# xxlong0/NeuralUDF

Hardware: AMD Instinct MI355X
Metric: ray-samples/sec (train step) (higher is better)
Workload: dtype f32 emulated on the 16-bit matrix pipe, f32 accumulate, f32 state / epilogues / optimizer.  Forward-order sweeps (UDF value, input gradient, colour / NeRF forward): f16x2 (x = hi + 2^-11 lo in fp16, 3 fp16 MFMA products, correction terms in their own accumulator).  Backward sweeps (tangent, adjoint

## Files before the change

include/nudf.h:

```cpp
#ifndef NUDF_H
#define NUDF_H
#include <stdint.h>

#ifdef __cplusplus
extern "C" {
#endif

#define NUDF_ABI_VERSION 111
int nudf_version(void);
#define NUDF_ABI_STRUCTS(X) \
  X(NudfGemmNN) X(NudfGemmTN) X(NudfGemmTNProblem) X(NudfGemmTNGroup) X(NudfComposite) X(NudfCompositeGrad) \
  X(NudfUpsample) X(NudfPixelBlend) X(NudfPixelComposite) X(NudfPatchBlend) X(NudfPatchWarp) X(NudfBlendLoss) \
  X(NudfAdamTensor) X(NudfAdamGroup) X(NudfAdam) X(NudfChainStep) X(NudfChain) X(NudfPackFrag) X(NudfPackLayer) \
  X(NudfPackMulti) X(NudfUnpackLayer) X(NudfUnpackMulti) X(NudfRayBatch) X(NudfMeshUDF) X(NudfMeshUDFSparse) \
  X(NudfIsoSurface) X(NudfIsoSurfaceSparse) X(NudfPointCloud) X(NudfMeshTopo) X(NudfMeshOrient) X(NudfMeshRaster)
int nudf_abi_struct(int i, const char** name);
const char* nudf_last_error(void);

enum {
  NUDF_STATUS_NONFINITE_RENDER = 1,
  NUDF_STATUS_NONFINITE_SAMPLES = 2,
  NUDF_STATUS_NONFINITE_LOSS = 4
};
int nudf_set_status_flag(int32_t* device_word);
// ... 154 lines not shown
  const float* add_z; const float* add_udf;
  float* z_merged; float* udf_merged;
  int32_t merge_K;
} NudfUpsample;
#define NUDF_UP_DBG_ROWS 7
#define NUDF_UP_THEORICAL 256
#define NUDF_UP_SERIAL 512
#define NUDF_UP_NOCONTRACT 1024
#define NUDF_UP_SLEEF 2048
#define NUDF_UP_EXPCR 4096
int nudf_upsample(const NudfUpsample* args, void* stream);
int nudf_merge(const float* z, const float* udf, const float* z_new, const float* udf_new, int N, int M,
               int K, float* z_out, float* udf_out, void* stream);
int nudf_merge_points(const float* z, const float* z_new, int N, int M, int K, float* z_out, const float* rays_o,
                      const float* rays_d, const float* sample_dist, float* pts, float* xrows, int ldx, int xcols,
                      void* stream);

typedef struct NudfPixelBlend {
  const float* pts;
  const float* logits; int32_t nl;
  const float* proj;
  const float* imgs;
  int32_t P, V, H, W;
  float* pix;
  int32_t img_layout;
} NudfPixelBlend;
int nudf_pixel_blend_fwd(const NudfPixelBlend* a, void* stream);
int nudf_pixel_blend_bwd(const NudfPixelBlend* a, const float* d_pix, float* d_logits, void* stream);

typedef struct NudfPixelComposite {
  const float* w;
  const float* pix;
  const float* pts;
  const float* bg_in;
  const float* bg_tail;
  int32_t N, S, n_out;
  float* out;
} NudfPixelComposite;
int nudf_pixel_composite_fwd(const NudfPixelComposite* a, void* stream);
int nudf_pixel_composite_bwd(const NudfPixelComposite* a, const float* d_out, float* d_w, float* d_pix,
                             float* d_bg_in, float* d_bg_tail, void* stream);

typedef struct NudfPatchBlend {
  const float* pts;
  const float* grad;
  const float* rays_d;
  const float* uv;
  const float* logits; int32_t nl;
  const float* w; int32_t ldw;
  const float* ref_cam;
  const float* src_cam;
  const float* imgs;
  int32_t N, S, V, H, W, hps;
  float* patch_colors;
  float* patch_mask;
  int32_t img_layout;
} NudfPatchBlend;
int nudf_patch_blend_fwd(const NudfPatchBlend* a, void* stream);
int nudf_patch_blend_bwd(const NudfPatchBlend* a, const float* d_patch, float* d_logits, float* d_w, void* stream);

int nudf_pixel_warp(const NudfPixelBlend* a , float* colors ,
                    float* mask , void* stream);
typedef struct NudfPatchWarp {
  const float* pts;
  const float* normals;
  const float* uv;
  const float* ref_cam;
  const float* src_cam;
  const float* imgs;
  int32_t N, S, V, H, W, hps, img_layout;
  float* colors;
  float* mask;
} NudfPatchWarp;
int nudf_patch_warp(const NudfPatchWarp* a, void* stream);

int nudf_ssim_patch(const float* pred, const float* gt, const float* window, int N, int Npx, float* out,
                    const float* d_out, float* d_pred, void* stream);
int nudf_patch_metric(int type, const float* pred, const float* gt, const float* window, int N, int Npx, float* out,
                      const float* d_out, float* d_pred, void* stream);

typedef struct NudfBlendLoss {
  const float* cb; const float* c; const float* pix; const float* gt;
  const float* err;
  const float* patch_mask;
  const float* weight_sum;
  const float* err_sorted;
  const int64_t* order;
  float* m;
  float* err_masked;
  float* sums;
  const float* sums_ws;
  const float* w_dev;
  float* out;
  const float* d_total;
  float* d_cb; float* d_c; float* d_pix;
  float* d_err;
  float* d_sums;
  int32_t N, sums_nblk;
  float n_rays, trim_ratio;
} NudfBlendLoss;
int nudf_blend_loss_prepare(const NudfBlendLoss* args, void* stream);
int nudf_blend_loss_fwd(const NudfBlendLoss* args, void* stream);
int nudf_blend_loss_bwd(const NudfBlendLoss* args, void* stream);

int nudf_coarse_z(const float* near, const float* far, int nf_stride, const float* t_rand, int N, int S,
                  float* z, float* sample_dist, void* stream);
int nudf_coarse_start(const float* near, const float* far, int nf_stride, const float* t_rand, int center, int N, int S,
                      float* z, float* sample_dist, const float* rays_o, const float* rays_d, float* pts, void* stream);
int nudf_outside_z(const float* far, int f_stride, const float* lin, int N, int n_out, int n_samples,
                   float* z_out, void* stream);
int nudf_ray_points(const float* rays_o, const float* rays_d, const float* z, const float* sample_dist, int N,
                    int S, int mode, float* pts, void* stream);

int nudf_posenc(const float* x, int xld, int xdiv, const float* tangent, int D, int L, float in_scale, int P,
                float* dst1, int ld1, float scale1, float* dst2, int ld2, float scale2, void* stream);
int nudf_posenc_vjp(const float* x, int xld, int D, int L, float in_scale, int P, const float* src1, int ld1,
                    float scale1, const float* src2, int ld2, float scale2, float* g, void* stream);
int nudf_copy_cols(const float* src, int lds, int sdiv, float* dst, int ldd, int ncols, int P, float scale,
                   void* stream);

int nudf_udf_grad_seed(const float* sign, const float* w_row0, const float* h, int ldh, float hscale, int P, int C,
                       float inv_scale, float* out, int ldo, void* stream);
int nudf_udf_head_bwd(const float* sign, const float* dudf, const float* dfeat, int ldf, int P, int F,
                      float scale, float* out, int ldo, void* stream);
int nudf_signed_colsum(const float* sign, const float* R, int ldr, int P, int C, float scale, float* out,
                       void* stream);
int nudf_sigmoid_head_bwd(const float* y, const float* dy, const float* dy_extra, int ldx, int nsig,
                          const float* draw, int ldr, int nraw, int P, float* out, int ldo, void* stream);

int nudf_weightnorm_pack(const float* v, const float* g, int out, int in, const int* perm, float* W, int ldw,
                         float* Wt, int ldwt, float* inv_norm, void* stream);
int nudf_weightnorm_unpack_grad(const float* dW, int ldw, const float* v, const float* g, const float* inv_norm,
                                int out, int in, const int* perm, float* dv, float* dg, void* stream);

#define NUDF_ADAM_MAX_TENSORS 64
#define NUDF_ADAM_MAX_GROUPS 4
typedef struct NudfAdamTensor {
  float* p; const float* g; float* m; float* v;
  int32_t n;
  int32_t group;
  float neg_step_size;
  float bc2_sqrt;
} NudfAdamTensor;
typedef struct NudfAdamGroup {
  float one_minus_beta1, beta2, one_minus_beta2, eps;
} NudfAdamGroup;
typedef struct NudfAdam {
  int32_t n_tensors; int32_t pad_;
  NudfAdamTensor t[NUDF_ADAM_MAX_TENSORS];
  int32_t block_start[NUDF_ADAM_MAX_TENSORS + 1];
  int32_t pad2_;
  NudfAdamGroup group[NUDF_ADAM_MAX_GROUPS];
  const float* dyn;
} NudfAdam;
int nudf_adam_step(const NudfAdam* args, void* stream);
int nudf_adam_chunk(void);

enum {
  NUDF_CH_NONE = 0,
  NUDF_CH_SOFTPLUS = 1,
  NUDF_CH_MULSP = 2,
  NUDF_CH_TANGENT = 3,
  NUDF_CH_BWD = 4,
  NUDF_CH_UDFHEAD = 5,
  NUDF_CH_RELU = 6,
  NUDF_CH_SIGMOIDN = 7,
  NUDF_CH_MULMASK = 8,
  NUDF_CH_ADDMASK = 9,
  NUDF_CH_RELUADD = 10,
  NUDF_CH_SEED = 11
};
enum {
  NUDF_CH_INIT_LOAD = 0,
  NUDF_CH_INIT_POSENC = 1,
  NUDF_CH_INIT_SEED = 2
};
#define NUDF_CH_MAX_STEPS 20
typedef struct NudfChainStep {
  const float* Bp;
  const float* bias;
  const float* X1; const float* X2;
  float* C1; float* C2;
  const float* r1_row;
  const float* r1_col;
  int32_t K, N;
  int32_t epi;
  int32_t iparam;
  int32_t ldx1, ldx2, ldc1, ldc2;
  int32_t ldr1;
  int32_t prec;
  int32_t act_write;
  int32_t act_col0;
  int32_t pe_tail_col;
  int32_t ld_pe;
  float* pe_dst;
  float pe_tail_scale;
  float scale, xscale;
  int32_t layout;
  const float* row_w;
  float* row_sums;
  const float* X3;
  int32_t ldx3;
} NudfChainStep;
#define NUDF_CH_BLK_X1 1
#define NUDF_CH_BLK_X2 2
#define NUDF_CH_BLK_C1 4
#define NUDF_CH_BLK_C2 8
#define NUDF_CH_BLK_PE 16
#define NUDF_CH_STATE16 32
#define NUDF_CH_P4_X1 64
#define NUDF_CH_P4_C1 128
typedef struct NudfChain {
  int32_t P, n_steps;
  int32_t init;
  int32_t k0;
  int32_t x_div;
  int32_t tile_rows;
  int32_t lda0, ldg0;
  int32_t pe_L, pe_jvp;
  int32_t init_state16;
  float pe_in_scale;
  float seed_scale, seed_xscale;
  const float* A0;
  float* G0;
  const float* x;
  const float* v;
  const float* seed_sign;
  const float* seed_wrow;
  unsigned long long* dbg;
  float* absmax_out;
  const float* tile_amax_in;
  float* tile_amax_out;
  int32_t tile_scale;
  int32_t reserved0;
  NudfChainStep step[NUDF_CH_MAX_STEPS];
} NudfChain;
#define NUDF_CH_TILE_TQ 66
#define NUDF_CH_TILE_ROWS 128
#if defined(__cplusplus)
static_assert(sizeof(NudfChain) <= 4096, "NudfChain travels by value: the kernel-argument segment holds 4 KB");
#endif
int nudf_mlp_chain(const NudfChain* args, void* stream);
int nudf_mlp_chain_plan(const NudfChain* args, char* name, int capacity, int32_t* out);
int nudf_set_chain_t16(int on);
int nudf_pack_frag(const float* B, int ldb, int K, int N, float* out, void* stream);

#define NUDF_PACK_MAX_LAYERS 16
#define NUDF_PACK_MAX_FRAGS 4
typedef struct NudfPackFrag {
  float* dst;
  int32_t transpose;
  int32_t o0, i0;
  int32_t K, N;
  int32_t dtype;
} NudfPackFrag;
typedef struct NudfPackLayer {
  const float* v; const float* g;
  const int32_t* perm;
  float* W; float* Wt;
  float* inv_norm;
  int32_t out, in, ldw, ldwt;
  int32_t nfrag, row_start;
  NudfPackFrag frag[NUDF_PACK_MAX_FRAGS];
} NudfPackLayer;
typedef struct NudfPackMulti {
  int32_t n_layers, total_rows;
  NudfPackLayer layer[NUDF_PACK_MAX_LAYERS];
} NudfPackMulti;
int nudf_weightnorm_pack_multi(const NudfPackMulti* args, void* stream);

typedef struct NudfUnpackLayer {
  const float* dW;
  const float* v; const float* g; const float* inv_norm;
  const int32_t* perm;
  float* dv; float* dg;
  const float* db_in; float* db_out;
  int32_t out, in, ldw, row_start;
} NudfUnpackLayer;
typedef struct NudfUnpackMulti {
  int32_t n_layers, total_rows;
  NudfUnpackLayer layer[NUDF_PACK_MAX_LAYERS];
} NudfUnpackMulti;
int nudf_weightnorm_unpack_grad_multi(const NudfUnpackMulti* args, void* stream);

int nudf_scalars_fwd(const float* variance, const float* beta, const float* gamma, float beta_hi, float* scal,
                     float* recip, void* stream);
int nudf_scalars_bwd(const float* variance, const float* beta, const float* gamma, float beta_hi, const float* d_scal,
                     float* d_param, void* stream);

int nudf_l1_sum_fwd(const float* pred, const float* gt, int n, float* out, void* stream);
int nudf_l1_sum_bwd(const float* pred, const float* gt, int n, const float* d_out, float* d_pred, void* stream);

int nudf_sums_errors_fwd(const float* sums, float n_rays, float* err, void* stream);
int nudf_sums_errors_bwd(const float* sums, float n_rays, const float* d_err, float* d_sums, void* stream);

enum { NUDF_LW_COLOR_BASE = 0, NUDF_LW_COLOR = 1, NUDF_LW_COLOR_PIXEL = 2, NUDF_LW_COLOR_PATCH = 3, NUDF_LW_IGR = 4,
       NUDF_LW_IGR_NS = 5, NUDF_LW_SPARSE = 6, NUDF_LW_MASK = 7,
       NUDF_LW_COLOR_SUM = 8,
       NUDF_LW_COUNT = 16 };

int nudf_color_loss_fwd(const float* cb, const float* c, const float* gt, int n, const float* mask, int n_mask,
                        float w_b, float w_c, float w_px, const float* w_dev, float* out, float* den_out, void* stream);
int nudf_color_loss_bwd(const float* cb, const float* c, const float* gt, int n, const float* den, float w_b, float w_c,
                        float w_px, const float* w_dev, const float* d_out, float* d_cb, float* d_c, void* stream);
int nudf_color_loss_sums(const float* cb, const float* c, const float* gt, int n, const float* mask, int n_mask,
                         float* sums, void* stream);
int nudf_color_loss_finish(const float* sums, int has_mask, float w_b, float w_c, float w_px, const float* w_dev,
                           float* out, float* den_out, void* stream);
// ... 414 lines not shown
```

neuraludf_amd/_lib.py:

```python
from __future__ import annotations

import ctypes as C
import os

import torch

_HERE = os.path.dirname(os.path.abspath(__file__))
LIB_PATH = os.environ.get("NUDF_LIB") or os.path.join(_HERE, "libnudf.so")
ABI_VERSION = 111

c_fp = C.c_void_p
i32 = C.c_int32
f32 = C.c_float


class NudfError(RuntimeError):
    pass


class GemmNN(C.Structure):
    _fields_ = [("A", c_fp), ("lda", i32), ("B", c_fp), ("ldb", i32), ("bias", c_fp),
                ("C1", c_fp), ("ldc1", i32), ("C2", c_fp), ("ldc2", i32), ("C3", c_fp), ("ldc3", i32),
                ("X1", c_fp), ("ldx1", i32), ("X2", c_fp), ("ldx2", i32),
                ("M", i32), ("N", i32), ("K", i32), ("epi", i32), ("iparam", i32), ("scale", f32), ("xscale", f32)]


class GemmTN(C.Structure):
    _fields_ = [("A1", c_fp), ("lda1", i32), ("na1", i32), ("B1", c_fp), ("ldb1", i32),
                ("A2", c_fp), ("lda2", i32), ("na2", i32), ("B2", c_fp), ("ldb2", i32),
                ("C", c_fp), ("ldc", i32), ("dbias", c_fp), ("M", i32), ("NA", i32), ("NB", i32),
                ("rows_per_block", i32), ("prec", i32)]


TN_MAX_PROBLEMS = 12


class GemmTNProblem(C.Structure):
    _fields_ = [("A1", c_fp), ("B1", c_fp), ("C", c_fp), ("dbias", c_fp), ("lda1", i32), ("ldb1", i32), ("ldc", i32),
                ("NA", i32), ("NB", i32), ("tile_start", i32), ("flags", i32)]


class GemmTNGroup(C.Structure):
    _fields_ = [("n_problems", i32), ("M", i32), ("rows_per_block", i32), ("total_tiles", i32), ("prec", i32),
                ("prob", GemmTNProblem * TN_MAX_PROBLEMS), ("workspace", c_fp), ("workspace_floats", C.c_int64),
                ("assign", i32), ("amax_a", c_fp), ("amax_b", c_fp)]


class BlendLoss(C.Structure):
    _fields_ = [("cb", c_fp), ("c", c_fp), ("pix", c_fp), ("gt", c_fp), ("err", c_fp), ("patch_mask", c_fp),
                ("weight_sum", c_fp), ("err_sorted", c_fp), ("order", c_fp), ("m", c_fp), ("err_masked", c_fp), ("sums", c_fp),
                ("sums_ws", c_fp), ("w_dev", c_fp), ("out", c_fp), ("d_total", c_fp), ("d_cb", c_fp), ("d_c", c_fp),
                ("d_pix", c_fp), ("d_err", c_fp), ("d_sums", c_fp), ("N", i32), ("sums_nblk", i32), ("n_rays", f32),
                ("trim_ratio", f32)]


class RayBatch(C.Structure):
    _fields_ = [("image", c_fp), ("mask", c_fp), ("intrinsics_inv", c_fp), ("pose", c_fp), ("pixels_x", c_fp),
                ("pixels_y", c_fp), ("N", i32), ("H", i32), ("W", i32), ("h_patch_size", i32), ("rays", c_fp),
                ("ndc_uv", c_fp), ("xyz_cam", c_fp), ("near", c_fp), ("far", c_fp), ("patch_color", c_fp),
                ("patch_mask", c_fp)]


class Composite(C.Structure):
    _fields_ = [("rays_o", c_fp), ("rays_d", c_fp), ("z", c_fp), ("udf", c_fp), ("grad", c_fp),
                ("color", c_fp), ("color_base", c_fp), ("bg_z", c_fp), ("bg_sigma", c_fp), ("bg_color", c_fp),
                ("scal", c_fp), ("sample_dist", c_fp), ("background_rgb", c_fp),
                ("N", i32), ("S", i32), ("n_out", i32), ("s_nominal", i32),
                ("has_anneal", i32), ("cos_anneal", f32), ("flip_saturation", f32),
                ("use_norm_grad", i32), ("sparse_scale", f32), ("alpha_type", i32),
                ("weights", c_fp), ("out_color", c_fp), ("out_color_base", c_fp), ("out_depth", c_fp),
                ("out_normals", c_fp), ("out_wsum", c_fp), ("out_wsum_all", c_fp), ("sums", c_fp), ("ws", c_fp),
                ("o_alpha", c_fp), ("o_alpha_plus", c_fp), ("o_alpha_minus", c_fp), ("o_vis_prob", c_fp),
                ("o_alpha_occ", c_fp), ("o_raw_occ", c_fp), ("o_true_cos", c_fp), ("o_grad_mag", c_fp),
                ("o_mid_z", c_fp), ("o_dists", c_fp), ("o_inside", c_fp), ("o_flip", c_fp), ("sched", c_fp),
                ("p_variance", c_fp), ("p_beta", c_fp), ("p_gamma", c_fp), ("beta_hi", f32), ("defer_sums", i32),
                ("scal_out", c_fp), ("recip_out", c_fp)]


class CompositeGrad(C.Structure):
    _fields_ = [("d_color", c_fp), ("d_color_base", c_fp), ("d_weights", c_fp), ("d_depth", c_fp),
                ("d_normals", c_fp), ("d_wsum", c_fp), ("d_wsum_all", c_fp), ("d_sums", c_fp),
                ("o_d_udf", c_fp), ("o_d_grad", c_fp), ("o_d_color", c_fp), ("o_d_color_base", c_fp),
                ("o_d_bg_sigma", c_fp), ("o_d_bg_color", c_fp), ("o_d_scal", c_fp), ("ws", c_fp), ("o_d_param", c_fp)]


class Upsample(C.Structure):
    _fields_ = [("rays_o", c_fp), ("rays_d", c_fp), ("z", c_fp), ("udf", c_fp), ("u", c_fp),
                ("sample_dist", c_fp), ("gamma_dev", c_fp),
                ("N", i32), ("M", i32), ("K", i32), ("mode", i32),
                ("inv_s", f32), ("beta", f32), ("gamma", f32),
                ("z_new", c_fp), ("pts_new", c_fp), ("dbg", c_fp),
                ("prev_z", c_fp), ("prev_udf", c_fp), ("add_z", c_fp), ("add_udf", c_fp),
                ("z_merged", c_fp), ("udf_merged", c_fp), ("merge_K", i32)]


class PixelBlend(C.Structure):
    _fields_ = [("pts", c_fp), ("logits", c_fp), ("nl", i32), ("proj", c_fp), ("imgs", c_fp),
                ("P", i32), ("V", i32), ("H", i32), ("W", i32), ("pix", c_fp), ("img_layout", i32)]


class PixelComposite(C.Structure):
    _fields_ = [("w", c_fp), ("pix", c_fp), ("pts", c_fp), ("bg_in", c_fp), ("bg_tail", c_fp),
                ("N", i32), ("S", i32), ("n_out", i32), ("out", c_fp)]


class PatchBlend(C.Structure):
    _fields_ = [("pts", c_fp), ("grad", c_fp), ("rays_d", c_fp), ("uv", c_fp), ("logits", c_fp), ("nl", i32),
                ("w", c_fp), ("ldw", i32), ("ref_cam", c_fp), ("src_cam", c_fp), ("imgs", c_fp),
                ("N", i32), ("S", i32), ("V", i32), ("H", i32), ("W", i32), ("hps", i32),
                ("patch_colors", c_fp), ("patch_mask", c_fp), ("img_layout", i32)]


class PatchWarp(C.Structure):
    _fields_ = [("pts", c_fp), ("normals", c_fp), ("uv", c_fp), ("ref_cam", c_fp), ("src_cam", c_fp), ("imgs", c_fp),
                ("N", i32), ("S", i32), ("V", i32), ("H", i32), ("W", i32), ("hps", i32), ("img_layout", i32),
                ("colors", c_fp), ("mask", c_fp)]


ADAM_MAX_TENSORS = 64
ADAM_MAX_GROUPS = 4


class AdamTensor(C.Structure):
    _fields_ = [("p", c_fp), ("g", c_fp), ("m", c_fp), ("v", c_fp), ("n", i32), ("group", i32), ("neg_step_size", f32), ("bc2_sqrt", f32)]


class AdamGroup(C.Structure):
    _fields_ = [("one_minus_beta1", f32), ("beta2", f32), ("one_minus_beta2", f32), ("eps", f32)]


class Adam(C.Structure):
    _fields_ = [("n_tensors", i32), ("pad_", i32), ("t", AdamTensor * ADAM_MAX_TENSORS),
                ("block_start", i32 * (ADAM_MAX_TENSORS + 1)), ("pad2_", i32), ("group", AdamGroup * ADAM_MAX_GROUPS),
                ("dyn", c_fp)]


CH_MAX_STEPS = 20
CH_STATE16 = 32
CH_P4_X1, CH_P4_C1 = 64, 128
CH = dict(NONE=0, SOFTPLUS=1, MULSP=2, TANGENT=3, BWD=4, UDFHEAD=5, RELU=6, SIGMOIDN=7, MULMASK=8, ADDMASK=9, RELUADD=10,
          SEED=11)
CH_INIT = dict(LOAD=0, POSENC=1, SEED=2)


class ChainStep(C.Structure):
    _fields_ = [("Bp", c_fp), ("bias", c_fp), ("X1", c_fp), ("X2", c_fp), ("C1", c_fp), ("C2", c_fp),
                ("r1_row", c_fp), ("r1_col", c_fp), ("K", i32), ("N", i32), ("epi", i32), ("iparam", i32),
                ("ldx1", i32), ("ldx2", i32), ("ldc1", i32), ("ldc2", i32), ("ldr1", i32), ("prec", i32), ("act_write", i32),
                ("act_col0", i32), ("pe_tail_col", i32), ("ld_pe", i32), ("pe_dst", c_fp), ("pe_tail_scale", f32),
                ("scale", f32), ("xscale", f32), ("layout", i32), ("row_w", c_fp), ("row_sums", c_fp), ("X3", c_fp),
                ("ldx3", i32)]


class Chain(C.Structure):
    _fields_ = [("P", i32), ("n_steps", i32), ("init", i32), ("k0", i32), ("x_div", i32), ("tile_rows", i32), ("lda0", i32),
                ("ldg0", i32), ("pe_L", i32), ("pe_jvp", i32), ("init_state16", i32), ("pe_in_scale", f32), ("seed_scale", f32),
                ("seed_xscale", f32), ("A0", c_fp), ("G0", c_fp), ("x", c_fp), ("v", c_fp), ("seed_sign", c_fp),
                ("seed_wrow", c_fp), ("dbg", c_fp), ("absmax_out", c_fp), ("tile_amax_in", c_fp),
                ("tile_amax_out", c_fp), ("tile_scale", C.c_int32), ("reserved0", C.c_int32), ("step", ChainStep * CH_MAX_STEPS)]


PACK_MAX_LAYERS = 16
PACK_MAX_FRAGS = 4


class PackFrag(C.Structure):
    _fields_ = [("dst", c_fp), ("transpose", i32), ("o0", i32), ("i0", i32), ("K", i32), ("N", i32), ("dtype", i32)]


class PackLayer(C.Structure):
    _fields_ = [("v", c_fp), ("g", c_fp), ("perm", c_fp), ("W", c_fp), ("Wt", c_fp), ("inv_norm", c_fp),
                ("out", i32), ("in_", i32), ("ldw", i32), ("ldwt", i32), ("nfrag", i32), ("row_start", i32),
                ("frag", PackFrag * PACK_MAX_FRAGS)]


class PackMulti(C.Structure):
    _fields_ = [("n_layers", i32), ("total_rows", i32), ("layer", PackLayer * PACK_MAX_LAYERS)]


class UnpackLayer(C.Structure):
    _fields_ = [("dW", c_fp), ("v", c_fp), ("g", c_fp), ("inv_norm", c_fp), ("perm", c_fp), ("dv", c_fp),
                ("dg", c_fp), ("db_in", c_fp), ("db_out", c_fp), ("out", i32), ("in_", i32), ("ldw", i32), ("row_start", i32)]


class UnpackMulti(C.Structure):
    _fields_ = [("n_layers", i32), ("total_rows", i32), ("layer", UnpackLayer * PACK_MAX_LAYERS)]


class MeshUDF(C.Structure):
    _fields_ = [("U", c_fp), ("G", c_fp), ("axes", c_fp), ("cell_case", c_fp), ("cell_ntri", c_fp), ("edge_flag", c_fp),
                ("cells", c_fp), ("face_off", c_fp), ("edge_scan", c_fp), ("faces", c_fp), ("edges", c_fp), ("verts", c_fp),
                ("n_cells", C.c_int64), ("n_edges", C.c_int64), ("n_faces", C.c_int64), ("N", i32), ("mean_thr", f32),
                ("max_thr", f32), ("pad_", i32)]


class MeshUDFSparse(C.Structure):
    _fields_ = [("U", c_fp), ("G", c_fp), ("axes", c_fp), ("blocks", c_fp), ("block_slot", c_fp), ("cell_case", c_fp),
                ("cell_ntri", c_fp), ("cells", c_fp), ("face_off", c_fp), ("edge_keys", c_fp), ("edges", c_fp),
                ("faces", c_fp), ("verts", c_fp), ("n_blocks", C.c_int64), ("n_cells", C.c_int64), ("n_edges", C.c_int64),
                ("n_faces", C.c_int64), ("N", i32), ("B", i32), ("nb", i32), ("mean_thr", f32), ("max_thr", f32),
                ("pad_", i32)]


class IsoSurface(C.Structure):
    _fields_ = [("F", c_fp), ("axes", c_fp), ("cell_case", c_fp), ("cell_ntri", c_fp), ("edge_flag", c_fp), ("cells", c_fp),
                ("face_off", c_fp), ("edge_scan", c_fp), ("faces", c_fp), ("edges", c_fp), ("verts", c_fp),
                ("n_cells", C.c_int64), ("n_edges", C.c_int64), ("n_faces", C.c_int64), ("N", i32), ("level", f32)]


class IsoSurfaceSparse(C.Structure):
    _fields_ = [("F", c_fp), ("axes", c_fp), ("blocks", c_fp), ("block_slot", c_fp), ("cell_case", c_fp), ("cell_ntri", c_fp),
                ("cells", c_fp), ("face_off", c_fp), ("edge_keys", c_fp), ("edges", c_fp), ("faces", c_fp), ("verts", c_fp),
                ("n_blocks", C.c_int64), ("n_cells", C.c_int64), ("n_edges", C.c_int64), ("n_faces", C.c_int64), ("N", i32),
                ("B", i32), ("nb", i32), ("level", f32)]


class PointCloud(C.Structure):
    _fields_ = [("verts", c_fp), ("faces", c_fp), ("tri_n", c_fp), ("tri_off", c_fp), ("out", c_fp),
                ("n_verts", C.c_int64), ("n_faces", C.c_int64), ("n_out", C.c_int64), ("out_base", C.c_int64),
                ("cap", C.c_int64), ("density", C.c_double),
                ("pts", c_fp), ("n", C.c_int64), ("origin", C.c_double * 3), ("cell", C.c_double), ("grid", i32 * 3),
                ("pad_", i32), ("keys", c_fp), ("cell_key", c_fp), ("cell_start", c_fp), ("cell_count", c_fp),
                ("n_cells", C.c_int64), ("hash_key", c_fp), ("hash_row", c_fp), ("hash_cap", C.c_int64),
                ("rank", c_fp), ("state", c_fp), ("undecided", c_fp), ("r2", C.c_double),
                ("query", c_fp), ("query_idx", c_fp), ("n_query", C.c_int64), ("bound", C.c_double),
                ("box_bound2", C.c_double), ("box_lo", C.c_double * 3), ("box_hi", C.c_double * 3),
                ("dist", c_fp), ("idx", c_fp),
                ("md_ref_n", c_fp), ("md_ref_off", c_fp), ("md_ref_key", c_fp), ("md_ref_face", c_fp),
                ("md_n_refs", C.c_int64), ("md_cell_face", c_fp), ("md_point", c_fp), ("md_bary", c_fp),
                ("md_ray_o", c_fp), ("md_ray_d", c_fp), ("md_t_min", C.c_double), ("md_t_max", C.c_double),
                ("md_ray_window", c_fp), ("md_mode", i32), ("md_pad_", i32), ("md_count", c_fp)]


class MeshTopo(C.Structure):
    _fields_ = [("faces", c_fp), ("he_key", c_fp), ("he_id", c_fp), ("edge_start", c_fp), ("edges", c_fp), ("he_edge", c_fp),
                ("edge_key", c_fp), ("nbr_off", c_fp), ("nbr", c_fp), ("bverts", c_fp), ("new_count", c_fp), ("new_off", c_fp),
                ("new_faces", c_fp), ("pos", c_fp), ("pos_out", c_fp), ("labels", c_fp), ("changed", c_fp), ("proj", c_fp),
                ("masks", c_fp), ("vis_count", c_fp), ("n_faces", C.c_int64), ("n_verts", C.c_int64), ("n_edges", C.c_int64),
                ("n_bverts", C.c_int64), ("n_new", C.c_int64), ("lam", C.c_double), ("max_loop", i32), ("n_views", i32),
                ("H", i32), ("W", i32), ("border", i32), ("pad_", i32),
                ("sp_key", c_fp), ("sp_cluster_key", c_fp), ("sp_vcluster", c_fp), ("sp_member_off", c_fp),
                ("sp_member", c_fp), ("sp_corner_off", c_fp), ("sp_corner", c_fp), ("sp_attr", c_fp), ("sp_rep", c_fp),
                ("sp_accepted", c_fp), ("sp_quadric", c_fp), ("sp_attr_out", c_fp), ("sp_faces", c_fp),
                ("sp_triple", c_fp), ("sp_degenerate", c_fp), ("n_clusters", C.c_int64), ("sp_grid", C.c_int64 * 3),
                ("sp_origin", C.c_double * 3), ("sp_cell", C.c_double), ("sp_lambda", C.c_double),
                ("sp_boundary_weight", C.c_double), ("sp_attr_width", i32), ("sp_placement", i32),
                ("sp_sd_mark", c_fp), ("sp_sd_edge_vertex", c_fp), ("sp_sd_marked", c_fp), ("sp_sd_ring_off", c_fp),
                ("sp_sd_ring", c_fp), ("sp_sd_vclass", c_fp), ("sp_sd_pos_out", c_fp), ("sp_sd_attr_out", c_fp),
                ("sp_sd_fcount", c_fp), ("sp_sd_foff", c_fp), ("sp_sd_faces_out", c_fp), ("sp_sd_parent", c_fp),
                ("sp_sd_n_ring", C.c_int64), ("sp_sd_n_border", C.c_int64), ("sp_sd_n_marked", C.c_int64),
                ("sp_sd_n_out", C.c_int64), ("sp_sd_max_edge", C.c_double), ("sp_sd_scheme", i32),
                ("sp_sd_mark_all", i32),
                ("sp_sd_hf_bedge", c_fp), ("sp_sd_hf_brank", c_fp), ("sp_sd_hf_link", c_fp), ("sp_sd_hf_rank_in", c_fp),
                ("sp_sd_hf_rank_out", c_fp), ("sp_sd_hf_loop_off", c_fp), ("sp_sd_hf_loop_vertex", c_fp),
                ("sp_sd_hf_loop_edge", c_fp), ("sp_sd_hf_closed", c_fp), ("sp_sd_hf_perimeter", c_fp),
                ("sp_sd_hf_status", c_fp), ("sp_sd_hf_n_border", C.c_int64), ("sp_sd_hf_n_loops", C.c_int64),
                ("sp_sd_hf_n_items", C.c_int64), ("sp_sd_hf_max_perimeter", C.c_double), ("sp_sd_hf_round", i32),
                ("sp_sd_hf_pad_", i32)]


class MeshOrient(C.Structure):
    _fields_ = [("faces", c_fp), ("me_a", c_fp), ("me_b", c_fp), ("word", c_fp), ("changed", c_fp), ("nonorient", c_fp),
                ("comp_off", c_fp), ("comp_face", c_fp), ("comp_sum", c_fp), ("pos", c_fp), ("corner_off", c_fp),
                ("corner", c_fp), ("normals", c_fp), ("origin", C.c_double * 3), ("n_faces", C.c_int64),
                ("n_verts", C.c_int64), ("n_medges", C.c_int64), ("n_comps", C.c_int64),
                ("sm_nbr_off", c_fp), ("sm_nbr", c_fp), ("sm_fixed", c_fp), ("sm_pos_out", c_fp), ("sm_fnormal", c_fp),
                ("sm_fnormal_out", c_fp), ("sm_farea", c_fp), ("sm_fcentre", c_fp), ("sm_n_nbr", C.c_int64),
                ("sm_step", C.c_double), ("sm_inv2sc", C.c_double), ("sm_inv2ss", C.c_double), ("sm_weights", i32),
                ("sm_pad_", i32)]


class MeshRaster(C.Structure):
    _fields_ = [("pos", c_fp), ("faces", c_fp), ("proj", c_fp), ("scr", c_fp), ("npix", c_fp), ("entries", c_fp),
                ("zbuf", c_fp), ("depth", c_fp), ("face", c_fp), ("bary", c_fp), ("vis", c_fp), ("images", c_fp),
                ("normals", c_fp), ("cam_pos", c_fp), ("colors", c_fp), ("n_seen", c_fp), ("n_faces", C.c_int64),
                ("n_verts", C.c_int64), ("n_entries", C.c_int64), ("power", C.c_double), ("fill", f32 * 3),
                ("min_gap", f32), ("n_views", i32), ("H", i32), ("W", i32), ("image_f32", i32)]


LW = dict(color_base=0, color=1, color_pixel=2, color_patch=3, igr=4, igr_ns=5, sparse=6, mask=7, color_sum=8)
LW_COUNT = 16

EPI = dict(NONE=0, SOFTPLUS=1, RELU=2, MUL=3, MULMASK=4, TANGENT=5, BWD=6, SIGMOID=7, UDFHEAD=8,
           SKIPSPLIT=9, RELU_DUAL=10, ADDMASK=11, MULSP=12)

HOLE = dict(FILLED=0, OPEN_CHAIN=1, TOO_MANY_EDGES=2, PERIMETER=3, NONFINITE=4, DUPLICATE=5, REPEATED_VERTEX=6)
HOLE_MAX_EDGES = 64
HOLE_FAN_CAP = 4096

MIRRORS = {"Nudf" + c.__name__: c for c in C.Structure.__subclasses__() if c.__module__ == __name__}

_P, _I, _F = C.c_void_p, C.c_int, C.c_float
SIGNATURES = {
    "nudf_version": (_I, []),
    "nudf_abi_struct": (_I, [_I, C.POINTER(C.c_char_p)]),
    "nudf_last_error": (C.c_char_p, []),
    "nudf_set_status_flag": (_I, [_P]),
    "nudf_status_flag": (_P, []),
    "nudf_gemm_nn": (_I, [C.POINTER(GemmNN), _P]),
    "nudf_gemm_tn": (_I, [C.POINTER(GemmTN), _P]),
    "nudf_gemm_tn_grouped": (_I, [C.POINTER(GemmTNGroup), _P]),
    "nudf_gemm_tn_grouped_workspace": (C.c_int64, [C.POINTER(GemmTNGroup)]),
    "nudf_gemm_tn_grouped_plan": (_I, [C.POINTER(GemmTNGroup), C.POINTER(C.c_int32), i32]),
    "nudf_gemm_tn_grouped_kernel": (_I, [C.POINTER(GemmTNGroup), C.c_char_p, i32, C.POINTER(C.c_int32)]),
    "nudf_set_tn_flags": (_I, [i32]),
    "nudf_set_tn_debug": (_I, [_P]),
    "nudf_composite_fwd": (_I, [C.POINTER(Composite), _P]),
    "nudf_composite_bwd": (_I, [C.POINTER(Composite), C.POINTER(CompositeGrad), _P]),
    "nudf_partial_sums": (_I, [_P, _I, _I, _P, _P]),
    "nudf_composite_colour_finish": (_I, [_P, _P, _I, _I, _P, _P, _P, _P, _P]),
    "nudf_upsample": (_I, [C.POINTER(Upsample), _P]),
    "nudf_merge": (_I, [_P, _P, _P, _P, _I, _I, _I, _P, _P, _P]),
    "nudf_coarse_z": (_I, [_P, _P, _I, _P, _I, _I, _P, _P, _P]),
    "nudf_coarse_start": (_I, [_P, _P, _I, _P, _I, _I, _I, _P, _P, _P, _P, _P, _P]),
    "nudf_merge_points": (_I, [_P, _P, _I, _I, _I, _P, _P, _P, _P, _P, _P, _I, _I, _P]),
    "nudf_outside_z": (_I, [_P, _I, _P, _I, _I, _I, _P, _P]),
    "nudf_ray_points": (_I, [_P, _P, _P, _P, _I, _I, _I, _P, _P]),
    "nudf_posenc": (_I, [_P, _I, _I, _P, _I, _I, _F, _I, _P, _I, _F, _P, _I, _F, _P]),
    "nudf_posenc_vjp": (_I, [_P, _I, _I, _I, _F, _I, _P, _I, _F, _P, _I, _F, _P, _P]),
    "nudf_copy_cols": (_I, [_P, _I, _I, _P, _I, _I, _I, _F, _P]),
    "nudf_udf_grad_seed": (_I, [_P, _P, _P, _I, _F, _I, _I, _F, _P, _I, _P]),
    "nudf_udf_head_bwd": (_I, [_P, _P, _P, _I, _I, _I, _F, _P, _I, _P]),
    "nudf_signed_colsum": (_I, [_P, _P, _I, _I, _I, _F, _P, _P]),
    "nudf_sigmoid_head_bwd": (_I, [_P, _P, _P, _I, _I, _P, _I, _I, _I, _P, _I, _P]),
    "nudf_weightnorm_pack": (_I, [_P, _P, _I, _I, _P, _P, _I, _P, _I, _P, _P]),
    "nudf_weightnorm_unpack_grad": (_I, [_P, _I, _P, _P, _P, _I, _I, _P, _P, _P, _P]),
    "nudf_pixel_blend_fwd": (_I, [C.POINTER(PixelBlend), _P]),
    "nudf_pixel_blend_bwd": (_I, [C.POINTER(PixelBlend), _P, _P, _P]),
    "nudf_pixel_composite_fwd": (_I, [C.POINTER(PixelComposite), _P]),
    "nudf_pixel_composite_bwd": (_I, [C.POINTER(PixelComposite), _P, _P, _P, _P, _P, _P]),
    "nudf_patch_blend_fwd": (_I, [C.POINTER(PatchBlend), _P]),
    "nudf_patch_blend_bwd": (_I, [C.POINTER(PatchBlend), _P, _P, _P, _P]),
    "nudf_pixel_warp": (_I, [C.POINTER(PixelBlend), _P, _P, _P]),
    "nudf_patch_warp": (_I, [C.POINTER(PatchWarp), _P]),
    "nudf_ssim_patch": (_I, [_P, _P, _P, _I, _I, _P, _P, _P, _P]),
    "nudf_patch_metric": (_I, [_I] + [_P, _P, _P, _I, _I, _P, _P, _P, _P]),
    "nudf_adam_step": (_I, [C.POINTER(Adam), _P]),
    "nudf_adam_chunk": (_I, []),
    "nudf_mlp_chain": (_I, [C.POINTER(Chain), _P]),
    "nudf_mlp_chain_plan": (_I, [C.POINTER(Chain), C.c_char_p, i32, C.POINTER(C.c_int32)]),
    "nudf_set_chain_t16": (_I, [_I]),
    "nudf_pack_frag": (_I, [_P, _I, _I, _I, _P, _P]),
    "nudf_weightnorm_pack_multi": (_I, [C.POINTER(PackMulti), _P]),
    "nudf_weightnorm_unpack_grad_multi": (_I, [C.POINTER(UnpackMulti), _P]),
    "nudf_scalars_fwd": (_I, [_P, _P, _P, _F, _P, _P, _P]),
    "nudf_scalars_bwd": (_I, [_P, _P, _P, _F, _P, _P, _P]),
    "nudf_l1_sum_fwd": (_I, [_P, _P, _I, _P, _P]),
    "nudf_l1_sum_bwd": (_I, [_P, _P, _I, _P, _P, _P]),
    "nudf_sums_errors_fwd": (_I, [_P, _F, _P, _P]),
    "nudf_sums_errors_bwd": (_I, [_P, _F, _P, _P, _P]),
    "nudf_color_loss_fwd": (_I, [_P, _P, _P, _I, _P, _I, _F, _F, _F, _P, _P, _P, _P]),
    "nudf_color_loss_bwd": (_I, [_P, _P, _P, _I, _P, _F, _F, _F, _P, _P, _P, _P, _P]),
    "nudf_gen_ray_batch": (_I, [C.POINTER(RayBatch), _P]),
    "nudf_color_loss_sums": (_I, [_P, _P, _P, _I, _P, _I, _P, _P]),
    "nudf_color_loss_finish": (_I, [_P, _I, _F, _F, _F, _P, _P, _P, _P]),
    "nudf_step_loss_fwd": (_I, [_P, _P, _P, _I, _P, _I, _P, _F, _F, _F, _F, _F, _F, _F, _P, _P, _P, _P, _I, _P]),
    "nudf_step_loss_bwd": (_I, [_P, _P, _P, _I, _P, _P, _F, _F, _F, _F, _F, _F, _F, _P, _P, _P, _P, _P, _P, _P]),
    "nudf_col0_seed4": (_I, [_P, _P, _F, _I, _I, _P, _P, _P]),
    **{"nudf_" + n: (_I, [C.POINTER(st), _P]) for st, names in (
        (BlendLoss, ("blend_loss_prepare", "blend_loss_fwd", "blend_loss_bwd")),
        (MeshUDF, ("meshudf_classify", "meshudf_emit", "meshudf_vertices")),
        (MeshUDFSparse, ("meshudf_sparse_classify", "meshudf_sparse_edges", "meshudf_sparse_emit",
                         "meshudf_sparse_vertices")),
        (IsoSurface, ("isosurface_classify", "isosurface_emit", "isosurface_vertices")),
        (IsoSurfaceSparse, ("isosurface_sparse_classify", "isosurface_sparse_edges", "isosurface_sparse_emit",
                            "isosurface_sparse_vertices")),
        (PointCloud, ("pc_tri_count", "pc_tri_emit", "pc_keys", "pc_cells", "pc_thin_round", "pc_nearest",
                      "pc_tribin_count", "pc_tribin_emit", "pc_closest", "pc_raycast")),
        (MeshTopo, ("meshtopo_edges", "meshtopo_fill_count", "meshtopo_fill_emit", "meshtopo_smooth", "meshtopo_cc_hook",
                    "meshtopo_cc_jump", "meshtopo_views", "meshsimplify_keys", "meshsimplify_place",
                    "meshsimplify_faces", "meshsubdiv_mark", "meshsubdiv_odd", "meshsubdiv_even", "meshsubdiv_count",
                    "meshsubdiv_emit", "meshhole_link", "meshhole_rank", "meshhole_count", "meshhole_triangulate")),
        (MeshOrient, ("meshorient_hook", "meshorient_jump", "meshorient_check", "meshorient_outward", "meshorient_normals",
                      "meshsmooth_laplace", "meshsmooth_frames", "meshsmooth_normals", "meshsmooth_update")),
        (MeshRaster, ("meshraster_project", "meshraster_bounds", "meshraster_draw_small", "meshraster_draw_large",
                      "meshraster_resolve", "meshraster_visible", "meshraster_colour")),
    ) for n in names},
}
SYMBOLS = list(SIGNATURES)

_lib = None


def _abi_mismatch(version, table):
    if version != ABI_VERSION:
        return f"is ABI version {version}, this package binds {ABI_VERSION}"
    for name, size in table.items():
        if name not in MIRRORS:
            return f"has an argument struct {name} that this package does not bind"
        if size != C.sizeof(MIRRORS[name]):
            return f"has a {name} of {size} bytes, this package binds {C.sizeof(MIRRORS[name])}"
    missing = [name for name in MIRRORS if name not in table]
    if missing:
        return f"does not report {', '.join(missing)}, which this package binds"
    return None


def _abi_report(l):
    version, table, name, i = int(l.nudf_version()), {}, C.c_char_p(), 0
    if version == ABI_VERSION:
        while (size := l.nudf_abi_struct(i, C.byref(name))) >= 0:
            table[name.value.decode()], i = size, i + 1
    return version, table


def lib():
    global _lib
    if _lib is None:
        if not os.path.exists(LIB_PATH):
            raise NudfError(
                f"{LIB_PATH} not found: build it with `python -m neuraludf_amd.build` "
                "(the NeuralUDF hot path has no CPU/PyTorch fallback)")
        try:
            l = C.CDLL(LIB_PATH)
        except OSError as e:
            raise NudfError(f"cannot load {LIB_PATH}: {e}") from e
        try:
            why = _abi_mismatch(*_abi_report(l))
            if why is None:
                for name, (restype, argtypes) in SIGNATURES.items():
                    fn = getattr(l, name)
                    fn.restype, fn.argtypes = restype, argtypes
        except AttributeError as e:
            why = f"does not export every symbol of include/nudf.h ({e})"
        if why is not None:
            raise NudfError(f"{LIB_PATH} {why}: rebuild with `python -m neuraludf_amd.build --force`")
        _lib = l
    return _lib


STATUS_NONFINITE_RENDER, STATUS_NONFINITE_SAMPLES, STATUS_NONFINITE_LOSS = 1, 2, 4
_STATUS_WORDS = {}
_STATUS_BOUND = None


def bind_status(dev):
    global _STATUS_BOUND
    if dev.type != "cuda":
        raise NudfError("libnudf kernels need device tensors (got a CPU tensor): run on an MI355X")
    idx = dev.index if dev.index is not None else torch.cuda.current_device()
    if _STATUS_BOUND == idx:
        return _STATUS_WORDS[idx]
    w = _STATUS_WORDS.get(idx)
    if w is None:
        w = torch.zeros(1, dtype=torch.int32, device=torch.device("cuda", idx))
        _STATUS_WORDS[idx] = w
    check(lib().nudf_set_status_flag(C.c_void_p(w.data_ptr())), "nudf_set_status_flag")
    _STATUS_BOUND = idx
    return w


def read_status(dev, clear=False):
    w = bind_status(dev)
    v = int(w.item())
    if clear and v:
        w.zero_()
    return v


def status_text(bits):
    names = [(STATUS_NONFINITE_SAMPLES, "non-finite new samples in the hierarchical re-sampling (nudf_upsample)"),
             (STATUS_NONFINITE_RENDER, "non-finite composited ray outputs or renderer scalars (nudf_composite_fwd)"),
             (STATUS_NONFINITE_LOSS, "non-finite loss (nudf_step_loss_fwd)")]
    return "; ".join(t for b, t in names if bits & b) or "finite"


def ptr(t):
    if t is None:
        return None
    if not t.is_cuda:
        raise NudfError("libnudf kernels need device tensors (got a CPU tensor): run on an MI355X")
    if not t.is_contiguous():
        raise NudfError("libnudf kernels need contiguous tensors")
    return t.data_ptr()


HOST_FAST = os.environ.get("NUDF_HOST_FAST", "1") != "0"
_raw_stream = getattr(torch._C, "_cuda_getCurrentRawStream", None)
_raw_device = getattr(torch._C, "_cuda_getDevice", None)


def stream():
    if HOST_FAST and _raw_stream is not None and _raw_device is not None:
        return C.c_void_p(_raw_stream(_raw_device()))
    return C.c_void_p(torch.cuda.current_stream().cuda_stream)


def check(rc, what=""):
    if rc != 0:
        msg = lib().nudf_last_error()
        raise NudfError(f"{what} failed (hipError {rc}): {msg.decode() if msg else ''}")
# ... 19 lines not shown
```

neuraludf_amd/csrc/optim.hip:

```cpp
#include "nudf_common.h"
#include "../../include/nudf.h"

#define ADAM_BLOCK 256
#define ADAM_PER_THREAD 4
#define ADAM_CHUNK (ADAM_BLOCK * ADAM_PER_THREAD)

__global__ __launch_bounds__(ADAM_BLOCK) void adam_kernel(NudfAdam a) {
  int lo = 0, hi = a.n_tensors;
  const int b = blockIdx.x;
  while (hi - lo > 1) {
    const int mid = (lo + hi) >> 1;
    if (a.block_start[mid] <= b) lo = mid; else hi = mid;
  }
  NudfAdamTensor t = a.t[lo];
  const NudfAdamGroup g = a.group[t.group];
  if (a.dyn) {
    t.neg_step_size = a.dyn[2 * lo];
    t.bc2_sqrt = a.dyn[2 * lo + 1];
  }
  const int base = (b - a.block_start[lo]) * ADAM_CHUNK;
#pragma unroll
  for (int k = 0; k < ADAM_PER_THREAD; ++k) {
    const int i = base + k * ADAM_BLOCK + threadIdx.x;
    if (i < t.n) {
      const float gr = t.g[i];
      float m = t.m[i], v = t.v[i];
      m = m + (gr - m) * g.one_minus_beta1;
      v = v * g.beta2 + g.one_minus_beta2 * gr * gr;
      const float denom = sqrtf(v) / t.bc2_sqrt + g.eps;
      t.p[i] = t.p[i] + t.neg_step_size * (m / denom);
      t.m[i] = m;
      t.v[i] = v;
    }
  }
}

extern "C" int nudf_adam_step(const NudfAdam* args, void* stream) {
  const NudfAdam& a = *args;
  if (a.n_tensors <= 0) return 0;
  if (a.n_tensors > NUDF_ADAM_MAX_TENSORS) {
    nudf_set_error("nudf_adam_step: too many tensors in one call", hipErrorInvalidValue);
    return (int)hipErrorInvalidValue;
  }
  const int nblk = a.block_start[a.n_tensors];
  if (nblk <= 0) return 0;
  hipLaunchKernelGGL(adam_kernel, dim3(nblk), dim3(ADAM_BLOCK), 0, (hipStream_t)stream, a);
  NUDF_CHECK_LAUNCH("nudf_adam_step");
  return 0;
}

extern "C" int nudf_adam_chunk(void) { return ADAM_CHUNK; }
```

neuraludf_amd/csrc/rays_embed.hip:

```cpp
#include "nudf_common.h"
#include "../../include/nudf.h"

static inline int nblocks(long long n, int bs) { return (int)((n + bs - 1) / bs); }

__global__ void coarse_z_kernel(const float* near, const float* far, int nf_stride, const float* t_rand,
                                int N, int S, float* z) {
  int idx = blockIdx.x * blockDim.x + threadIdx.x;
  if (idx >= N * S) return;
  int r = idx / S, s = idx - r * S;
  float nr = near[r * nf_stride], fr = far[r * nf_stride];
  float step = 1.0f / (float)(S - 1);
  float t = (s < S / 2) ? s * step : 1.0f - (S - 1 - s) * step;
  float v = nr + (fr - nr) * t;
  if (t_rand) v = v + t_rand[r] * 2.0f / (float)S;
  z[idx] = v;
}

__global__ void sample_dist_kernel(const float* near, const float* far, int n, int S, float* out) {
  __shared__ float red[256];
  float acc = 0.f;
  for (int i = threadIdx.x; i < n; i += blockDim.x) acc += (far[i] - near[i]) / (float)S;
  red[threadIdx.x] = acc;
  __syncthreads();
  for (int s = 128; s > 0; s >>= 1) {
    if (threadIdx.x < s) red[threadIdx.x] += red[threadIdx.x + s];
    __syncthreads();
  }
  if (threadIdx.x == 0) out[0] = red[0] / (float)n;
}

extern "C" int nudf_coarse_z(const float* near, const float* far, int nf_stride, const float* t_rand, int N, int S,
                             float* z, float* sample_dist, void* stream) {
  hipStream_t st = (hipStream_t)stream;
  hipLaunchKernelGGL(coarse_z_kernel, dim3(nblocks((long long)N * S, 256)), dim3(256), 0, st, near, far, nf_stride,
                     t_rand, N, S, z);
  if (sample_dist)
    hipLaunchKernelGGL(sample_dist_kernel, dim3(1), dim3(256), 0, st, near, far, nf_stride ? N : 1, S, sample_dist);
  NUDF_CHECK_LAUNCH("nudf_coarse_z");
  return 0;
}

__global__ __launch_bounds__(256) void coarse_start_kernel(const float* near, const float* far, int nf_stride,
                                                           const float* t_rand, int center, int N, int S, float* z,
                                                           float* sample_dist, const float* __restrict__ o,
                                                           const float* __restrict__ d, float* __restrict__ pts) {
  const int idx = blockIdx.x * blockDim.x + threadIdx.x;
  if (idx < N * S) {
    const int r = idx / S, s = idx - r * S;
    const float nr = near[r * nf_stride], fr = far[r * nf_stride];
    const float step = 1.0f / (float)(S - 1);
    const float t = (s < S / 2) ? s * step : 1.0f - (S - 1 - s) * step;
    float v = nr + (fr - nr) * t;
    if (t_rand) {
      const float tr = center ? __fsub_rn(t_rand[r], 0.5f) : t_rand[r];
      v = v + tr * 2.0f / (float)S;
    }
    z[idx] = v;
    if (pts) {
      pts[(size_t)idx * 3 + 0] = o[r * 3 + 0] + d[r * 3 + 0] * v;
      pts[(size_t)idx * 3 + 1] = o[r * 3 + 1] + d[r * 3 + 1] * v;
      pts[(size_t)idx * 3 + 2] = o[r * 3 + 2] + d[r * 3 + 2] * v;
    }
  }
  if (blockIdx.x == 0 && sample_dist) {
    __shared__ float red[256];
    const int n = nf_stride ? N : 1;
    float acc = 0.f;
    for (int i = threadIdx.x; i < n; i += 256) acc += (far[i] - near[i]) / (float)S;
    red[threadIdx.x] = acc;
    __syncthreads();
    for (int s = 128; s > 0; s >>= 1) {
      if (threadIdx.x < s) red[threadIdx.x] += red[threadIdx.x + s];
      __syncthreads();
    }
    if (threadIdx.x == 0) sample_dist[0] = red[0] / (float)n;
  }
}
extern "C" int nudf_coarse_start(const float* near, const float* far, int nf_stride, const float* t_rand, int center, int N,
                                 int S, float* z, float* sample_dist, const float* rays_o, const float* rays_d, float* pts,
                                 void* stream) {
  if (N <= 0 || S < 2) {
    nudf_set_error("nudf_coarse_start: N >= 1 and S >= 2 required", hipErrorInvalidValue);
    return (int)hipErrorInvalidValue;
  }
  hipLaunchKernelGGL(coarse_start_kernel, dim3(nblocks((long long)N * S, 256)), dim3(256), 0, (hipStream_t)stream, near, far,
                     nf_stride, t_rand, center, N, S, z, sample_dist, rays_o, rays_d, pts);
  NUDF_CHECK_LAUNCH("nudf_coarse_start");
  return 0;
}

__global__ void outside_z_kernel(const float* far, int f_stride, const float* lin, int N, int n_out, float inv_ns,
                                 float* z_out) {
  int idx = blockIdx.x * blockDim.x + threadIdx.x;
  if (idx >= N * n_out) return;
  int r = idx / n_out, j = idx - r * n_out;
  z_out[idx] = far[r * f_stride] / lin[n_out - 1 - j] + inv_ns;
}
extern "C" int nudf_outside_z(const float* far, int f_stride, const float* lin, int N, int n_out, int n_samples,
                              float* z_out, void* stream) {
  hipLaunchKernelGGL(outside_z_kernel, dim3(nblocks((long long)N * n_out, 256)), dim3(256), 0, (hipStream_t)stream,
                     far, f_stride, lin, N, n_out, 1.0f / (float)n_samples, z_out);
  NUDF_CHECK_LAUNCH("nudf_outside_z");
  return 0;
}

__global__ void ray_points_kernel(const float* __restrict__ o, const float* __restrict__ d, const float* __restrict__ z,
                                  const float* sample_dist, int N, int S, int mode, float* __restrict__ pts) {
  int idx = blockIdx.x * blockDim.x + threadIdx.x;
  if (idx >= N * S) return;
  int r = idx / S, s = idx - r * S;
  float t = z[idx];
  if (mode >= 1) {
    float dist = (s < S - 1) ? (z[idx + 1] - t) : sample_dist[0];
    t = t + dist * 0.5f;
  }
  float px = o[r * 3 + 0] + d[r * 3 + 0] * t;
  float py = o[r * 3 + 1] + d[r * 3 + 1] * t;
  float pz = o[r * 3 + 2] + d[r * 3 + 2] * t;
  if (mode == 2) {
    float rr = sqrtf(px * px + py * py + pz * pz);
    rr = fminf(fmaxf(rr, 1.0f), 1e10f);
    pts[(size_t)idx * 4 + 0] = px / rr;
    pts[(size_t)idx * 4 + 1] = py / rr;
    pts[(size_t)idx * 4 + 2] = pz / rr;
    pts[(size_t)idx * 4 + 3] = 1.0f / rr;
  } else {
    pts[(size_t)idx * 3 + 0] = px;
    pts[(size_t)idx * 3 + 1] = py;
    pts[(size_t)idx * 3 + 2] = pz;
  }
}
extern "C" int nudf_ray_points(const float* rays_o, const float* rays_d, const float* z, const float* sample_dist, int N,
                               int S, int mode, float* pts, void* stream) {
  if (N * S == 0) return 0;
  hipLaunchKernelGGL(ray_points_kernel, dim3(nblocks((long long)N * S, 256)), dim3(256), 0, (hipStream_t)stream, rays_o,
                     rays_d, z, sample_dist, N, S, mode, pts);
  NUDF_CHECK_LAUNCH("nudf_ray_points");
  return 0;
}

__global__ void posenc_kernel(const float* __restrict__ x, int xld, int xdiv, const float* __restrict__ v, int D, int L,
                              float in_scale, int P, float* d1, int ld1, float s1, float* d2, int ld2, float s2,
                              int mode) {
  const int E = D * (2 * L + 1);
  long long idx = (long long)blockIdx.x * blockDim.x + threadIdx.x;
  if (idx >= (long long)P * E) return;
  int p = (int)(idx / E), e = (int)(idx - (long long)p * E);
  int blk = e / D, j = e - blk * D;
  float xv = x[(size_t)(p / xdiv) * xld + j] * in_scale;
  float val;
  if (blk == 0) {
    val = (mode == 0) ? xv : v[(size_t)p * D + j] * in_scale;
  } else {
    int k = (blk - 1) >> 1;
// ... 168 lines not shown
  out[idx] = v;
}
extern "C" int nudf_sigmoid_head_bwd(const float* y, const float* dy, const float* dy_extra, int ldx, int nsig,
                                     const float* draw, int ldr, int nraw, int P, float* out, int ldo, void* stream) {
  if (P == 0) return 0;
  hipLaunchKernelGGL(sigmoid_head_bwd_kernel, dim3(nblocks((long long)P * ldo, 256)), dim3(256), 0,
                     (hipStream_t)stream, y, dy, dy_extra, ldx, nsig, draw, ldr, nraw, P, out, ldo);
  NUDF_CHECK_LAUNCH("nudf_sigmoid_head_bwd");
  return 0;
}

__global__ void wn_pack_kernel(const float* __restrict__ v, const float* __restrict__ g, int out, int in,
                               const int* __restrict__ perm, float* __restrict__ W, int ldw, float* __restrict__ Wt,
                               int ldwt, float* __restrict__ inv_norm) {
  const int row = blockIdx.x * (blockDim.x >> 6) + (threadIdx.x >> 6);
  if (row >= out) return;
  const int l = threadIdx.x & 63;
  float sc = 1.0f;
  if (g) {
    float ss = 0.f;
    for (int i = l; i < in; i += 64) {
      float t = v[(size_t)row * in + i];
      ss += t * t;
    }
    ss = wave_sum(ss);
    float inv = 1.0f / sqrtf(ss);
    if (l == 0 && inv_norm) inv_norm[row] = inv;
    sc = g[row] * inv;
  }
  for (int i = l; i < in; i += 64) {
    int c = perm ? perm[i] : i;
    float w = v[(size_t)row * in + i] * sc;
    if (W) W[(size_t)row * ldw + c] = w;
    if (Wt) Wt[(size_t)c * ldwt + row] = w;
  }
}
extern "C" int nudf_weightnorm_pack(const float* v, const float* g, int out, int in, const int* perm, float* W, int ldw,
                                    float* Wt, int ldwt, float* inv_norm, void* stream) {
  hipLaunchKernelGGL(wn_pack_kernel, dim3((out + 3) / 4), dim3(256), 0, (hipStream_t)stream, v, g, out, in, perm, W, ldw,
                     Wt, ldwt, inv_norm);
  NUDF_CHECK_LAUNCH("nudf_weightnorm_pack");
  return 0;
}

__global__ void wn_unpack_grad_kernel(const float* __restrict__ dW, int ldw, const float* __restrict__ v,
                                      const float* __restrict__ g, const float* __restrict__ inv_norm, int out, int in,
                                      const int* __restrict__ perm, float* __restrict__ dv, float* __restrict__ dg) {
  const int row = blockIdx.x * (blockDim.x >> 6) + (threadIdx.x >> 6);
  if (row >= out) return;
  const int l = threadIdx.x & 63;
  if (!g) {
    for (int i = l; i < in; i += 64) dv[(size_t)row * in + i] = dW[(size_t)row * ldw + (perm ? perm[i] : i)];
    return;
  }
  float dot = 0.f;
  for (int i = l; i < in; i += 64) dot += dW[(size_t)row * ldw + (perm ? perm[i] : i)] * v[(size_t)row * in + i];
  dot = wave_sum(dot);
  const float inv = inv_norm[row];
  const float gg = g[row];
  if (l == 0) dg[row] = dot * inv;
  const float c1 = gg * inv, c2 = gg * inv * inv * inv * dot;
  for (int i = l; i < in; i += 64)
    dv[(size_t)row * in + i] = c1 * dW[(size_t)row * ldw + (perm ? perm[i] : i)] - c2 * v[(size_t)row * in + i];
}
extern "C" int nudf_weightnorm_unpack_grad(const float* dW, int ldw, const float* v, const float* g,
                                           const float* inv_norm, int out, int in, const int* perm, float* dv, float* dg,
                                           void* stream) {
  hipLaunchKernelGGL(wn_unpack_grad_kernel, dim3((out + 3) / 4), dim3(256), 0, (hipStream_t)stream, dW, ldw, v, g,
                     inv_norm, out, in, perm, dv, dg);
  NUDF_CHECK_LAUNCH("nudf_weightnorm_unpack_grad");
  return 0;
}

__device__ __forceinline__ void frag_store(const NudfPackFrag& f, int o, int c, float w) {
  const int k = f.transpose ? (c - f.i0) : (o - f.o0);
  const int n = f.transpose ? (o - f.o0) : (c - f.i0);
  if (k < 0 || n < 0 || k >= f.K || n >= f.N) return;
  const int NT = (f.N + 31) >> 5;
  if (f.dtype == 0) {
    const int g = k >> 3, r = k & 7;
    const int lane = 32 * (r >> 2) + (n & 31);
    f.dst[((size_t)(g * NT + (n >> 5)) * 64 + lane) * 4 + (r & 3)] = w;
  } else if (f.dtype == 3) {
    const int g = k >> 4, r = k & 15;
    const int lane = 32 * (r >> 3) + (n & 31);
    const __bf16 hi = (__bf16)w;
    const float r1 = w - (float)hi;
    const __bf16 mid = (__bf16)r1;
    const __bf16 lo = (__bf16)(r1 - (float)mid);
    unsigned short* d16 = reinterpret_cast<unsigned short*>(f.dst) + ((size_t)(g * NT + (n >> 5)) * 3 * 64 + lane) * 8 + (r & 7);
    d16[0] = __builtin_bit_cast(unsigned short, hi);
    d16[512] = __builtin_bit_cast(unsigned short, mid);
    d16[1024] = __builtin_bit_cast(unsigned short, lo);
  } else if (f.dtype == 4) {
    const int g = k >> 4, r = k & 15;
    const int lane = 32 * (r >> 3) + (n & 31);
    const _Float16 hi = (_Float16)w;
    const _Float16 lo = (_Float16)((w - (float)hi) * 2048.0f);
    unsigned short* d16 = reinterpret_cast<unsigned short*>(f.dst) + ((size_t)(g * NT + (n >> 5)) * 2 * 64 + lane) * 8 + (r & 7);
    d16[0] = __builtin_bit_cast(unsigned short, hi);
    d16[512] = __builtin_bit_cast(unsigned short, lo);
  } else {
    const int g = k >> 4, r = k & 15;
    const int lane = 32 * (r >> 3) + (n & 31);
    unsigned short bits;
    if (f.dtype == 1) {
      const _Float16 hv = (_Float16)w;
      bits = __builtin_bit_cast(unsigned short, hv);
    } else {
      const __bf16 bv = (__bf16)w;
      bits = __builtin_bit_cast(unsigned short, bv);
    }
    reinterpret_cast<unsigned short*>(f.dst)[((size_t)(g * NT + (n >> 5)) * 64 + lane) * 8 + (r & 7)] = bits;
  }
}

#define WNP_ROWS 32
#define WNP_THREADS 1024
__device__ __forceinline__ void wnp_split8(const float (&w)[8], uint4& hi, uint4& mid, uint4& lo) {
  unsigned short h[8], m[8], q[8];
#pragma unroll
  for (int j = 0; j < 8; ++j) {
    const __bf16 a = (__bf16)w[j];
    const float r1 = w[j] - (float)a;
    const __bf16 b = (__bf16)r1;
    const __bf16 c = (__bf16)(r1 - (float)b);
    h[j] = __builtin_bit_cast(unsigned short, a);
    m[j] = __builtin_bit_cast(unsigned short, b);
    q[j] = __builtin_bit_cast(unsigned short, c);
  }
  hi = uint4{(unsigned)h[0] | ((unsigned)h[1] << 16), (unsigned)h[2] | ((unsigned)h[3] << 16),
             (unsigned)h[4] | ((unsigned)h[5] << 16), (unsigned)h[6] | ((unsigned)h[7] << 16)};
  mid = uint4{(unsigned)m[0] | ((unsigned)m[1] << 16), (unsigned)m[2] | ((unsigned)m[3] << 16),
              (unsigned)m[4] | ((unsigned)m[5] << 16), (unsigned)m[6] | ((unsigned)m[7] << 16)};
  lo = uint4{(unsigned)q[0] | ((unsigned)q[1] << 16), (unsigned)q[2] | ((unsigned)q[3] << 16),
             (unsigned)q[4] | ((unsigned)q[5] << 16), (unsigned)q[6] | ((unsigned)q[7] << 16)};
}

__device__ __forceinline__ void wnp_split8_f16(const float (&w)[8], uint4& hi, uint4& lo) {
  unsigned short h[8], q[8];
#pragma unroll
  for (int j = 0; j < 8; ++j) {
    const _Float16 a = (_Float16)w[j];
    const _Float16 b = (_Float16)((w[j] - (float)a) * 2048.0f);
    h[j] = __builtin_bit_cast(unsigned short, a);
    q[j] = __builtin_bit_cast(unsigned short, b);
  }
  hi = uint4{(unsigned)h[0] | ((unsigned)h[1] << 16), (unsigned)h[2] | ((unsigned)h[3] << 16),
             (unsigned)h[4] | ((unsigned)h[5] << 16), (unsigned)h[6] | ((unsigned)h[7] << 16)};
  lo = uint4{(unsigned)q[0] | ((unsigned)q[1] << 16), (unsigned)q[2] | ((unsigned)q[3] << 16),
             (unsigned)q[4] | ((unsigned)q[5] << 16), (unsigned)q[6] | ((unsigned)q[7] << 16)};
}

__global__ __launch_bounds__(WNP_THREADS) void wn_pack_multi_kernel(NudfPackMulti a, int pw) {
  extern __shared__ float panel[];
  int li = 0, b = blockIdx.x;
  for (; li < a.n_layers; ++li) {
    const int nb = (a.layer[li].out + WNP_ROWS - 1) / WNP_ROWS;
    if (b < nb) break;
    b -= nb;
  }
  if (li >= a.n_layers) return;
  const NudfPackLayer& L = a.layer[li];
  const int row0 = b * WNP_ROWS;
  const int wave = threadIdx.x >> 6, l = threadIdx.x & 63, tid = threadIdx.x;
  for (int e = tid; e < WNP_ROWS * pw; e += WNP_THREADS) panel[e] = 0.0f;
  __syncthreads();
  for (int r = wave; r < WNP_ROWS; r += WNP_THREADS / 64) {
    const int row = row0 + r;
    if (row >= L.out) break;
    float sc = 1.0f;
    if (L.g) {
      float ss = 0.f;
      for (int i = l; i < L.in; i += 64) {
        const float t = L.v[(size_t)row * L.in + i];
        ss += t * t;
      }
      ss = wave_sum(ss);
      const float inv = 1.0f / sqrtf(ss);
      if (l == 0 && L.inv_norm) L.inv_norm[row] = inv;
      sc = L.g[row] * inv;
    }
    for (int i = l; i < L.in; i += 64) {
      const int c = L.perm ? L.perm[i] : i;
      const float w = L.v[(size_t)row * L.in + i] * sc;
      if (L.W) L.W[(size_t)row * L.ldw + c] = w;
      panel[r * pw + c] = w;
    }
  }
  __syncthreads();
  const int nrows = min(WNP_ROWS, L.out - row0);
  if (L.Wt) {
    for (int e = tid; e < L.in * WNP_ROWS; e += WNP_THREADS) {
      const int c = e >> 5, r = e & 31;
      if (r < nrows) L.Wt[(size_t)c * L.ldwt + row0 + r] = panel[r * pw + c];
    }
  }
  for (int fi = 0; fi < L.nfrag; ++fi) {
    const NudfPackFrag& f = L.frag[fi];
    const int NT = (f.N + 31) >> 5;
    uint4* d4 = reinterpret_cast<uint4*>(f.dst);
    const bool split16 = f.dtype == 3 || f.dtype == 4;
    const int np = (f.dtype == 3) ? 3 : 2;
    if (split16 && f.transpose) {
      const int Q = (f.K + 7) >> 3;
      for (int e = tid; e < WNP_ROWS * Q; e += WNP_THREADS) {
        const int r = e & 31, q = e >> 5;
        const int n = row0 + r - f.o0;
        if (r >= nrows || n < 0 || n >= f.N) continue;
        float w[8];
#pragma unroll
        for (int j = 0; j < 8; ++j) {
          const int k = 8 * q + j;
          w[j] = (k < f.K) ? panel[r * pw + f.i0 + k] : 0.0f;
        }
        uint4 hi, mid, lo;
        const size_t slot = ((size_t)((q >> 1) * NT + (n >> 5)) * np) * 64 + 32 * (q & 1) + (n & 31);
        if (np == 3) {
          wnp_split8(w, hi, mid, lo);
          d4[slot] = hi; d4[slot + 64] = mid; d4[slot + 128] = lo;
        } else {
          wnp_split8_f16(w, hi, lo);
          d4[slot] = hi; d4[slot + 64] = lo;
        }
      }
    } else if (split16 && (f.o0 & 7) == 0) {
      for (int e = tid; e < 4 * f.N; e += WNP_THREADS) {
        const int t = e / f.N, n = e - t * f.N;
        const int k0 = row0 - f.o0 + 8 * t;
        if (k0 < 0 || k0 >= f.K) continue;
        float w[8];
#pragma unroll
        for (int j = 0; j < 8; ++j) w[j] = (k0 + j < f.K) ? panel[(8 * t + j) * pw + f.i0 + n] : 0.0f;
        uint4 hi, mid, lo;
        const size_t slot = ((size_t)((k0 >> 4) * NT + (n >> 5)) * np) * 64 + 32 * ((k0 >> 3) & 1) + (n & 31);
        if (np == 3) {
          wnp_split8(w, hi, mid, lo);
          d4[slot] = hi; d4[slot + 64] = mid; d4[slot + 128] = lo;
        } else {
          wnp_split8_f16(w, hi, lo);
          d4[slot] = hi; d4[slot + 64] = lo;
        }
      }
    } else {
      for (int e = tid; e < nrows * L.in; e += WNP_THREADS) {
        const int r = e / L.in, c = e - r * L.in;
        frag_store(f, row0 + r, c, panel[r * pw + c]);
      }
    }
  }
}
extern "C" int nudf_weightnorm_pack_multi(const NudfPackMulti* args, void* stream) {
  if (args->n_layers <= 0 || args->total_rows <= 0) return 0;
  if (args->n_layers > NUDF_PACK_MAX_LAYERS) {
    nudf_set_error("nudf_weightnorm_pack_multi: too many layers", hipErrorInvalidValue);
    return (int)hipErrorInvalidValue;
  }
  int blocks = 0, in_max = 0;
  for (int i = 0; i < args->n_layers; ++i) {
    blocks += (args->layer[i].out + WNP_ROWS - 1) / WNP_ROWS;
    in_max = max(in_max, args->layer[i].in);
    for (int f = 0; f < args->layer[i].nfrag; ++f)
      if ((args->layer[i].frag[f].dtype == 3 || args->layer[i].frag[f].dtype == 4) && (((uintptr_t)args->layer[i].frag[f].dst) & 15)) {
        nudf_set_error("nudf_weightnorm_pack_multi: split (bf16x3 / f16x2) fragment buffers must be 16-byte aligned", hipErrorInvalidValue);
        return (int)hipErrorInvalidValue;
      }
  }
  const int pw = (in_max + 31) / 32 * 32 + 4;
  const size_t lds = (size_t)WNP_ROWS * pw * sizeof(float);
  if (lds > 64 * 1024) {
    nudf_set_error("nudf_weightnorm_pack_multi: layer wider than 508 inputs", hipErrorInvalidValue);
    return (int)hipErrorInvalidValue;
  }
  hipLaunchKernelGGL(wn_pack_multi_kernel, dim3(blocks), dim3(WNP_THREADS), lds, (hipStream_t)stream, *args, pw);
  NUDF_CHECK_LAUNCH("nudf_weightnorm_pack_multi");
  return 0;
}

__global__ __launch_bounds__(256) void wn_unpack_multi_kernel(NudfUnpackMulti a) {
  const int grow = blockIdx.x * 4 + (threadIdx.x >> 6);
  if (grow >= a.total_rows) return;
  int li = 0;
  while (li + 1 < a.n_layers && a.layer[li + 1].row_start <= grow) ++li;
  const NudfUnpackLayer& L = a.layer[li];
  const int row = grow - L.row_start;
  const int l = threadIdx.x & 63;
  if (l == 0 && L.db_out) L.db_out[row] = L.db_in[row];
  if (!L.g) {
    for (int i = l; i < L.in; i += 64)
      L.dv[(size_t)row * L.in + i] = L.dW[(size_t)row * L.ldw + (L.perm ? L.perm[i] : i)];
    return;
  }
  float dot = 0.f;
  for (int i = l; i < L.in; i += 64)
    dot += L.dW[(size_t)row * L.ldw + (L.perm ? L.perm[i] : i)] * L.v[(size_t)row * L.in + i];
  dot = wave_sum(dot);
  const float inv = L.inv_norm[row];
  const float gg = L.g[row];
  if (l == 0) L.dg[row] = dot * inv;
  const float c1 = gg * inv, c2 = gg * inv * inv * inv * dot;
  for (int i = l; i < L.in; i += 64)
    L.dv[(size_t)row * L.in + i] =
        c1 * L.dW[(size_t)row * L.ldw + (L.perm ? L.perm[i] : i)] - c2 * L.v[(size_t)row * L.in + i];
}
extern "C" int nudf_weightnorm_unpack_grad_multi(const NudfUnpackMulti* args, void* stream) {
  if (args->n_layers <= 0 || args->total_rows <= 0) return 0;
  if (args->n_layers > NUDF_PACK_MAX_LAYERS) {
    nudf_set_error("nudf_weightnorm_unpack_grad_multi: too many layers", hipErrorInvalidValue);
    return (int)hipErrorInvalidValue;
  }
  hipLaunchKernelGGL(wn_unpack_multi_kernel, dim3((args->total_rows + 3) / 4), dim3(256), 0, (hipStream_t)stream, *args);
  NUDF_CHECK_LAUNCH("nudf_weightnorm_unpack_grad_multi");
  return 0;
}

__global__ void scalars_fwd_kernel(const float* variance, const float* beta, const float* gamma, float beta_hi,
                                   float* scal, float* recip) {
  if (threadIdx.x != 0) return;
  const float s = fminf(fmaxf(expf(10.0f * variance[0]), 1e-6f), 1e6f);
  const float b = fminf(fmaxf(fminf(fmaxf(expf(10.0f * beta[0]), 0.0f), beta_hi), 1e-6f), 1e6f);
  const float g = fminf(fmaxf(expf(10.0f * gamma[0]), 1e-6f), 1e6f);
  scal[0] = s; scal[1] = b; scal[2] = g;
  if (recip) { recip[0] = 1.0f / s; recip[1] = 1.0f / b; }
}
extern "C" int nudf_scalars_fwd(const float* variance, const float* beta, const float* gamma, float beta_hi,
                                float* scal, float* recip, void* stream) {
  hipLaunchKernelGGL(scalars_fwd_kernel, dim3(1), dim3(64), 0, (hipStream_t)stream, variance, beta, gamma, beta_hi,
                     scal, recip);
  NUDF_CHECK_LAUNCH("nudf_scalars_fwd");
  return 0;
}
__global__ void scalars_bwd_kernel(const float* variance, const float* beta, const float* gamma, float beta_hi,
                                   const float* d_scal, float* d_param) {
  if (threadIdx.x != 0) return;
  const float s = expf(10.0f * variance[0]);
  d_param[0] = (s >= 1e-6f && s <= 1e6f) ? d_scal[0] * 10.0f * s : 0.0f;
  const float b = expf(10.0f * beta[0]);
  const float b1 = fminf(fmaxf(b, 0.0f), beta_hi);
  d_param[1] = (b >= 0.0f && b <= beta_hi && b1 >= 1e-6f && b1 <= 1e6f) ? d_scal[1] * 10.0f * b : 0.0f;
  const float g = expf(10.0f * gamma[0]);
  d_param[2] = (g >= 1e-6f && g <= 1e6f) ? d_scal[2] * 10.0f * g : 0.0f;
}
extern "C" int nudf_scalars_bwd(const float* variance, const float* beta, const float* gamma, float beta_hi,
                                const float* d_scal, float* d_param, void* stream) {
  hipLaunchKernelGGL(scalars_bwd_kernel, dim3(1), dim3(64), 0, (hipStream_t)stream, variance, beta, gamma, beta_hi,
                     d_scal, d_param);
  NUDF_CHECK_LAUNCH("nudf_scalars_bwd");
  return 0;
}

__global__ __launch_bounds__(1024) void l1_sum_fwd_kernel(const float* __restrict__ pred, const float* __restrict__ gt,
                                                          int n, float* out) {
  __shared__ float red[16];
  float acc = 0.f;
  for (int i = threadIdx.x; i < n; i += 1024) acc += fabsf(pred[i] - gt[i]);
  acc = wave_sum(acc);
  if ((threadIdx.x & 63) == 0) red[threadIdx.x >> 6] = acc;
  __syncthreads();
  if (threadIdx.x == 0) {
    float t = 0.f;
    for (int w = 0; w < 16; ++w) t += red[w];
    out[0] = t;
  }
}
extern "C" int nudf_l1_sum_fwd(const float* pred, const float* gt, int n, float* out, void* stream) {
  if (n <= 0) return 0;
  hipLaunchKernelGGL(l1_sum_fwd_kernel, dim3(1), dim3(1024), 0, (hipStream_t)stream, pred, gt, n, out);
  NUDF_CHECK_LAUNCH("nudf_l1_sum_fwd");
  return 0;
}
__global__ void l1_sum_bwd_kernel(const float* __restrict__ pred, const float* __restrict__ gt, int n,
                                  const float* d_out, float* __restrict__ d_pred) {
  const int i = blockIdx.x * blockDim.x + threadIdx.x;
  if (i >= n) return;
  const float d = pred[i] - gt[i];
  d_pred[i] = d_out[0] * ((d > 0.0f) ? 1.0f : ((d < 0.0f) ? -1.0f : 0.0f));
}
extern "C" int nudf_l1_sum_bwd(const float* pred, const float* gt, int n, const float* d_out, float* d_pred,
                               void* stream) {
  if (n <= 0) return 0;
  hipLaunchKernelGGL(l1_sum_bwd_kernel, dim3(nblocks(n, 256)), dim3(256), 0, (hipStream_t)stream, pred, gt, n, d_out,
                     d_pred);
  NUDF_CHECK_LAUNCH("nudf_l1_sum_bwd");
  return 0;
}

__global__ void sums_errors_fwd_kernel(const float* sums, float n_rays, float* err) {
  if (threadIdx.x != 0) return;
  err[0] = sums[0] / (sums[1] + 1e-5f);
  err[1] = sums[2] / (sums[3] + 1e-5f);
  err[2] = sums[4] / n_rays;
}
extern "C" int nudf_sums_errors_fwd(const float* sums, float n_rays, float* err, void* stream) {
  hipLaunchKernelGGL(sums_errors_fwd_kernel, dim3(1), dim3(64), 0, (hipStream_t)stream, sums, n_rays, err);
  NUDF_CHECK_LAUNCH("nudf_sums_errors_fwd");
  return 0;
}
__global__ void sums_errors_bwd_kernel(const float* sums, float n_rays, const float* d_err, float* d_sums) {
  if (threadIdx.x != 0) return;
  const float a = sums[1] + 1e-5f, b = sums[3] + 1e-5f;
  d_sums[0] = d_err[0] / a;
  d_sums[1] = -d_err[0] * sums[0] / (a * a);
  d_sums[2] = d_err[1] / b;
  d_sums[3] = -d_err[1] * sums[2] / (b * b);
// ... 402 lines not shown
```

neuraludf_amd/mlp.py:

```python
from __future__ import annotations

import math
from typing import List, Optional

import ctypes as C

import torch

from . import _lib
import os

from ._lib import CH, CH_INIT, CH_MAX_STEPS, EPI, Chain, GemmNN, GemmTN, call, ptr


def pad32(n: int) -> int:
    return (n + 31) // 32 * 32


def pad_rows(P: int) -> int:
    return (P + 63) // 64 * 64


def _buf(P, width, dev, zero=None, dtype=torch.float32, blocked=False):
    if blocked:
        assert zero is False and dtype == torch.float32
        t = torch.empty((pad_rows(P), pad32(width)), device=dev, dtype=dtype)
        t._nudf_blk = True
        return t
    ld = pad32(width)
    if dtype == torch.bfloat16:
        t = (torch.zeros if zero else torch.empty)((pad_rows(P), ld), device=dev, dtype=dtype)
        if zero is None and ld != width:
            t.view(pad_rows(P) // 4, ld, 4)[:, width:, :].zero_()
        t._nudf_p4 = True
        return t
    if zero is None:
        t = torch.empty((pad_rows(P), ld), device=dev, dtype=dtype)
        if ld != width:
            t[:, width:].zero_()
        return t
    return (torch.zeros if zero else torch.empty)((pad_rows(P), ld), device=dev, dtype=dtype)


def _is16(t):
    return t is not None and t.dtype == torch.bfloat16


def _isblk(t):
    return t is not None and getattr(t, "_nudf_blk", False)


def _isp4(t):
    return t is not None and getattr(t, "_nudf_p4", False)


def pack16(t):
    R, ld = t.shape
    assert R % 4 == 0
    b = t.to(torch.bfloat16).reshape(R // 4, 4, ld).permute(0, 2, 1).reshape(R, ld).contiguous()
    b._nudf_p4 = True
    return b


def unpack16(t):
    R, ld = t.shape
    assert _isp4(t) and R % 4 == 0
    return t.reshape(R // 4, ld, 4).permute(0, 2, 1).reshape(R, ld).float()


def block(t):
    R, ld = t.shape
    assert R % 32 == 0 and ld % 4 == 0 and t.dtype == torch.float32
    b = t.reshape(R // 32, 32, ld // 4, 4).permute(0, 2, 1, 3).reshape(R, ld).contiguous()
    b._nudf_blk = True
    return b


def unblock(t):
    if not _isblk(t):
        return t
    R, ld = t.shape
    return t.reshape(R // 32, ld // 4, 32, 4).permute(0, 2, 1, 3).reshape(R, ld).contiguous()


def _zero_cols(t, c0):
    if c0 < t.shape[1]:
        t[:, c0:].zero_()
    return t


def alloc_grads(layers, zero=True):
    sizes = [(pl.out_pad * pl.in_pad, pl.out_pad) for pl in layers]
    flat = (torch.zeros if zero else torch.empty)(sum(a + b for a, b in sizes), device=layers[0].W.device)
    out, off = [], 0
    for pl, (a, b) in zip(layers, sizes):
        dW = flat[off:off + a].view(pl.out_pad, pl.in_pad)
        db = flat[off + a:off + a + pl.out]
        out.append((dW, db))
        off += a + b
    return out


def gemm_nn(A, B, M, N, K, epi, C1=None, ldc1=0, C2=None, ldc2=0, C3=None, ldc3=0, X1=None, ldx1=0, X2=None, ldx2=0,
            bias=None, lda=None, ldb=None, iparam=0, scale=1.0, xscale=1.0, c1_off=0, c2_off=0, x1_off=0, x2_off=0):
    a = GemmNN()
    a.A, a.lda = ptr(A), (lda if lda is not None else A.shape[1])
    a.B, a.ldb = ptr(B), (ldb if ldb is not None else B.shape[1])
    a.bias = ptr(bias)
    a.C1 = (ptr(C1) + 4 * c1_off) if C1 is not None else None
    a.ldc1 = ldc1 or (C1.shape[1] if (C1 is not None and C1.dim() == 2) else 0)
    a.C2 = (ptr(C2) + 4 * c2_off) if C2 is not None else None
    a.ldc2 = ldc2 or (C2.shape[1] if (C2 is not None and C2.dim() == 2) else 0)
    a.C3 = ptr(C3)
    a.ldc3 = ldc3 or (C3.shape[1] if (C3 is not None and C3.dim() == 2) else 0)
    a.X1 = (ptr(X1) + 4 * x1_off) if X1 is not None else None
    a.ldx1 = ldx1 or (X1.shape[1] if (X1 is not None and X1.dim() == 2) else 0)
    a.X2 = (ptr(X2) + 4 * x2_off) if X2 is not None else None
    a.ldx2 = ldx2 or (X2.shape[1] if (X2 is not None and X2.dim() == 2) else 0)
    a.M, a.N, a.K, a.epi, a.iparam, a.scale, a.xscale = M, N, K, EPI[epi], iparam, scale, xscale
    if PROFILE is not None:
        _timed("gemm_nn", 2.0 * M * N * getattr(B, "k_true", K), lambda: call("nudf_gemm_nn", a))
        return
    call("nudf_gemm_nn", a)


MFMA_PRODUCTS = {0: 1, 1: 1, 2: 1, 3: 6, 4: 3}

PROFILE = None


def _timed(name, flops, fn, detail=None, nbytes=0.0, xflops=None):
    s = torch.cuda.Event(enable_timing=True)
    e = torch.cuda.Event(enable_timing=True)
    s.record()
    fn()
    e.record()
    PROFILE.append((name, flops, s, e, detail or name, nbytes, xflops))


def call_timed(cls, detail, nbytes, name, *args, units=0.0):
    if PROFILE is None:
        call(name, *args)
    else:
        _timed(cls, -float(units), lambda: call(name, *args), detail, float(nbytes))


def gemm_tn(A1, na1, B1, C, NA, NB, M, dbias=None, A2=None, na2=0, B2=None):
    for t in (A1, B1, A2, B2):
        if t is not None and (_is16(t) or _isblk(t)):
            raise _lib.NudfError("gemm_tn: bf16-stored / blocked-layout operands need gemm_tn_grouped (per-problem "
                                 "NUDF_TN_A16 / _B16 / _A_BLK / _B_BLK flags): the per-layer path (USE_CHAIN = False) "
                                 "stores row-major fp32 state")
    a = GemmTN()
    a.A1, a.lda1, a.na1 = ptr(A1), A1.shape[1], na1
    a.B1, a.ldb1 = ptr(B1), B1.shape[1]
    if A2 is not None:
        a.A2, a.lda2, a.na2 = ptr(A2), A2.shape[1], na2
        a.B2, a.ldb2 = ptr(B2), B2.shape[1]
# ... 273 lines not shown

TN_DETERMINISTIC = True
_TN_WS = {}


def _tn_workspace(g, dev):
    need = int(_lib.lib().nudf_gemm_tn_grouped_workspace(C.byref(g)))
    if need <= 0:
        return None, 0
    ws = _TN_WS.get(dev)
    if ws is None or ws.numel() < need:
        ws = _TN_WS[dev] = torch.empty(need, device=dev)
    return ws, ws.numel()


TN_ASSIGN = os.environ.get("NUDF_TN_ASSIGN", "1") == "1"
_TN_ATOMIC = bool(int(os.environ.get("NUDF_TN_FLAGS", "0")) & 8)


def tn_can_assign():
    return TN_ASSIGN and TN_DETERMINISTIC and not _TN_ATOMIC


def gemm_tn_grouped(jobs, M, assign=False, rows_per_block=0, f16x2=False, amax_a=None, amax_b=None):
    for base in range(0, len(jobs), _lib.TN_MAX_PROBLEMS):
        chunk = jobs[base:base + _lib.TN_MAX_PROBLEMS]
        g = _lib.GemmTNGroup()
        g.n_problems, g.M, g.rows_per_block = len(chunk), M, rows_per_block
        g.prec = _tn_prec()
        if f16x2 and g.prec == 3 and not any(_is16(t) or _isblk(t) for j in chunk for t in (j[0], j[2])):
            g.prec = 4
            g.amax_a, g.amax_b = ptr(amax_a), ptr(amax_b)
        flops = nbytes = 0.0
        for i, (A1, NA, B1, NB, Cm, db) in enumerate(chunk):
            q = g.prob[i]
            q.A1, q.B1, q.C, q.dbias = ptr(A1), ptr(B1), ptr(Cm), ptr(db)
            q.flags = ((1 if _is16(A1) else 0) | (2 if _is16(B1) else 0) | (4 if _isblk(A1) else 0) | (8 if _isblk(B1) else 0) |
                       (16 if _isp4(A1) else 0) | (32 if _isp4(B1) else 0))
            q.lda1, q.ldb1, q.ldc, q.NA, q.NB = A1.shape[1], B1.shape[1], Cm.shape[1], NA, NB
            flops += 2.0 * M * NA * NB
            nbytes += float(M) * (NA * A1.element_size() + NB * B1.element_size())
        if TN_DETERMINISTIC:
            ws, n = _tn_workspace(g, chunk[0][0].device)
            g.workspace, g.workspace_floats = ptr(ws), n
        g.assign = 1 if assign else 0
        if PROFILE is not None:
            _timed("gemm_tn", flops, lambda: call("nudf_gemm_tn_grouped", g),
                   "%s %d problems M=%d (%.1f GFLOP)" % (_lib.kernel_of("nudf_gemm_tn_grouped_kernel", g)[0], len(chunk), M, flops / 1e9),
                   nbytes, flops * MFMA_PRODUCTS.get(int(g.prec), 1))
        else:
            call("nudf_gemm_tn_grouped", g)


class PackedLinear:

    def __init__(self, lin: torch.nn.Module, perm: Optional[List[int]] = None):
        self.lin = lin
        self.weight_norm = hasattr(lin, "weight_v")
        v = lin.weight_v if self.weight_norm else lin.weight
        self.out, self.inp = v.shape
        self.out_pad, self.in_pad = pad32(self.out), pad32(self.inp)
        self._perm_list = perm
        self.perm = None
        self.W = self.Wt = self.inv_norm = None
        self._ver = None
        self._frags = {}
        self._plist = None

    def params(self):
        reg = self.lin._parameters
        pl = self._plist
        if self.weight_norm:
            if pl is None or reg.get("weight_v") is not pl[0] or reg.get("weight_g") is not pl[1] or reg.get("bias") is not pl[2]:
                pl = self._plist = [self.lin.weight_v, self.lin.weight_g, self.lin.bias]
        elif pl is None or reg.get("weight") is not pl[0] or reg.get("bias") is not pl[1]:
            pl = self._plist = [self.lin.weight, self.lin.bias]
        return list(pl)

    def _ensure_buffers(self, dev):
        if self.W is None or self.W.device != dev:
            self.W = torch.zeros(self.out_pad, self.in_pad, device=dev)
            self.Wt = torch.zeros(self.in_pad, self.out_pad, device=dev)
            self.inv_norm = torch.empty(self.out, device=dev)
            self.Wt.k_true, self.W.k_true = self.inp, self.out
            self._frags = {}
            if self._perm_list is not None:
                self.perm = torch.tensor(self._perm_list, dtype=torch.int32, device=dev)

    def invalidate(self):
        self._ver = None
        self._frags = {}

    def frag(self, kind):
        f = self._frags.get(kind)
        if f is None:
            if "@" in kind:
                raise _lib.NudfError("16-bit fragment %r was not packed (pack_group packs them)" % kind)
            if kind == "fwd":
                f = pack_frag(self.Wt, self.out_pad, self.inp, self.out)
            elif kind == "bwd":
                f = pack_frag(self.W, self.in_pad, self.out, self.inp)
            elif kind == "fwd_head0":
                f = pack_frag(self.Wt, self.out_pad, self.inp, 1)
            elif kind == "fwd_feat":
                f = pack_frag(self.Wt, self.out_pad, self.inp, self.out - 1, off=1)
            elif kind == "bwd_feat":
                f = pack_frag(self.W, self.in_pad, self.out - 1, self.inp, off=self.in_pad)
            elif kind.startswith("bwd_hid:"):
                f = pack_frag(self.W, self.in_pad, self.out, int(kind.split(":")[1]))
            elif kind.startswith("fwd_in:"):
                _, i0, K = kind.split(":")
                f = pack_frag(self.Wt, self.out_pad, int(K), self.out, off=int(i0) * self.out_pad)
            else:
                raise KeyError(kind)
            self._frags[kind] = f
        return f

    @property
    def bias(self):
        return self.lin.bias.detach()

    def new_grad_buffers(self):
        dev = self.W.device
        return torch.zeros(self.out_pad, self.in_pad, device=dev), torch.zeros(self.out, device=dev)


PRECISION = os.environ.get("NUDF_PRECISION", "bf16x3")
_PREC = {"f32": 0, "f16": 1, "bf16": 2, "bf16x3": 3, "f16x2": 4}
FWD_F16X2 = os.environ.get("NUDF_FWD_F16X2", "1")
BWD_F16X2 = os.environ.get("NUDF_BWD_F16X2", "1") != "0"
EX_FLY = os.environ.get("NUDF_EX_FLY", "1") != "0"
TN_F16X2 = True
TN_SPLIT = True
BLOCKED_STATE = True


FUSE_SWEEPS = os.environ.get("NUDF_FUSE_SWEEPS", "1") != "0"


def set_fuse_sweeps(on):
    global FUSE_SWEEPS
    old, FUSE_SWEEPS = FUSE_SWEEPS, bool(on)
    return old


def _shared_split(state=None, mixed16=False):
    return (PRECISION != "fp32" if mixed16 else PRECISION == "bf16x3") and CHAIN_TILE in (0, 32, 64) and not _isblk(state)


def _fuse():
    return FUSE_SWEEPS and _shared_split()


def _tn_prec():
    if PRECISION == "fp32":
        return 0
    return 3 if PRECISION == "bf16x3" else 2


HEAD16 = os.environ.get("NUDF_HEAD16", "1") != "0"


def _head_kind():
    return "fwd_head0@f16" if (PRECISION == "mixed16" and HEAD16) else "fwd_head0"


def _state_blocked(P):
    return PRECISION == "fp32" and USE_CHAIN and CHAIN_TILE in (0, 66) and P > 256 * 64


def _state_dtype():
    return torch.bfloat16 if PRECISION == "mixed16" else torch.float32


def set_precision(name):
    global PRECISION
    if name not in ("fp32", "mixed16", "bf16x3"):
        raise ValueError("precision must be 'fp32', 'bf16x3' or 'mixed16'")
    PRECISION = name


def set_fwd_split(name):
    global FWD_F16X2
    if str(name) not in ("0", "1", "grad"):
        raise ValueError("forward split must be '0', '1' or 'grad'")
    old, FWD_F16X2 = FWD_F16X2, str(name)
    return old


def _sweep_dtype(sweep):
    if PRECISION == "fp32":
        return "f32"
    if PRECISION == "bf16x3":
        if FWD_F16X2 != "0" and (sweep == "fwd" or (sweep == "grad" and FWD_F16X2 != "grad")):
            return "f16x2"
        if sweep == "bwd" and BWD_F16X2 and FWD_F16X2 != "0":
            return "f16x2"
        return "bf16x3"
    return "f16" if sweep in ("fwd", "grad") else "bf16"


def _kind(base, sweep):
    dt = _sweep_dtype(sweep)
    return base if dt == "f32" else base + "@" + dt


def _frag_spec(pl, kind):
    dtype = 0
    if "@" in kind:
        kind, dt = kind.split("@")
        dtype = _PREC[dt]
    return _frag_spec32(pl, kind) + (dtype,)


def _frag_spec32(pl, kind):
    if kind == "fwd":
        return (1, 0, 0, pl.inp, pl.out)
    if kind == "bwd":
        return (0, 0, 0, pl.out, pl.inp)
    if kind == "fwd_head0":
        return (1, 0, 0, pl.inp, 1)
    if kind == "fwd_feat":
        return (1, 1, 0, pl.inp, pl.out - 1)
    if kind == "bwd_feat":
        return (0, 1, 0, pl.out - 1, pl.inp)
    if kind.startswith("bwd_hid:"):
        return (0, 0, 0, pl.out, int(kind.split(":")[1]))
    if kind.startswith("fwd_in:"):
        _, i0, K = kind.split(":")
        return (1, 0, int(i0), int(K), pl.out)
    raise KeyError(kind)


def _mode_key():
    return (PRECISION, FWD_F16X2, BWD_F16X2, HEAD16)


def pack_group(layers, kinds=None):
    memo_key = (len(layers), tuple(kinds) if kinds is not None else None)
    memos = getattr(layers[0], "_group_memo", None) if _lib.HOST_FAST else None
    m = memos.get(memo_key) if memos is not None else None
    if m is not None:
        fresh = True
        for pl, ver_obj, p0, v0, d0, p1, v1, d1 in m:
            if (pl._ver is not ver_obj or p0._version != v0 or p0.data_ptr() != d0
                    or (p1 is not None and (p1._version != v1 or p1.data_ptr() != d1))):
                fresh = False
                break
        if fresh:
            return
    kinds = kinds or [()] * len(layers)
    dev = layers[0].params()[0].device
    stale = False
    kinds = [tuple(dict.fromkeys(ks)) for ks in kinds]
    for pl, ks in zip(layers, kinds):
        ps = pl.params()
        ver = tuple((p.data_ptr(), p._version) for p in ps[:-1])
        if ver != pl._ver or pl.W is None or pl.W.device != dev or any(k not in pl._frags for k in ks):
            stale = True
        pl._new_ver = ver
    if not stale:
        _remember_group(layers, memo_key)
        return
    psig = _pack_ptr_signature(layers, kinds, dev)
    if m is not None and psig is not None and getattr(layers[0], "_pack_descs", {}).get(memo_key, (None,))[0] == psig:
        for a in layers[0]._pack_descs[memo_key][1]:
            call("nudf_weightnorm_pack_multi", a)
        for pl in layers:
            pl._ver = pl._new_ver
        _remember_group(layers, memo_key)
        return
    descs = []
    for base in range(0, len(layers), _lib.PACK_MAX_LAYERS):
        chunk = layers[base:base + _lib.PACK_MAX_LAYERS]
        a = _lib.PackMulti()
        rows = 0
        keep = []
        for li, pl in enumerate(chunk):
            ks = kinds[base + li]
            if len(ks) > _lib.PACK_MAX_FRAGS:
                raise _lib.NudfError("too many fragment copies for one layer")
            pl._ensure_buffers(dev)
            ps = pl.params()
            v = ps[0].detach().contiguous()
            g = ps[1].detach().contiguous() if pl.weight_norm else None
            keep += [v, g]
            L = a.layer[li]
            L.v, L.g, L.perm = ptr(v), ptr(g), ptr(pl.perm)
            L.W, L.Wt, L.inv_norm = ptr(pl.W), ptr(pl.Wt), ptr(pl.inv_norm)
            L.out, L.in_, L.ldw, L.ldwt = pl.out, pl.inp, pl.in_pad, pl.out_pad
            L.nfrag, L.row_start = len(ks), rows
            for fi, kind in enumerate(ks):
                tr, o0, i0, K, N, dtype = _frag_spec(pl, kind)
                f = pl._frags.get(kind)
                if f is None:
                    nfl = k8(K) // 8 * ((N + 31) // 32) * 256
                    f = torch.zeros({0: nfl, 3: 3 * (nfl // 2), 4: nfl}.get(dtype, nfl // 2), device=dev, dtype=torch.float32)
                    f.k_true, f.n_true, f.prec = K, N, dtype
                    pl._frags[kind] = f
                F = L.frag[fi]
                F.dst, F.transpose, F.o0, F.i0, F.K, F.N, F.dtype = ptr(f), tr, o0, i0, K, N, dtype
            rows += pl.out
        a.n_layers, a.total_rows = len(chunk), rows
        call("nudf_weightnorm_pack_multi", a)
        descs.append(a)
        del keep
    for pl in layers:
        pl._ver = pl._new_ver
    _remember_group(layers, memo_key)
    psig = _pack_ptr_signature(layers, kinds, dev)
    if psig is not None:
        layers[0].__dict__.setdefault("_pack_descs", {})[memo_key] = (psig, descs)


def _pack_ptr_signature(layers, kinds, dev):
    sig = []
    for pl, ks in zip(layers, kinds):
        if pl.W is None or pl.W.device != dev:
            return None
        for p in pl.params()[:-1]:
            if not p.is_contiguous():
                return None
            sig.append(p.data_ptr())
        sig += [pl.W.data_ptr(), pl.Wt.data_ptr(), pl.inv_norm.data_ptr(), pl.perm.data_ptr() if pl.perm is not None else 0]
        for k in ks:
            f = pl._frags.get(k)
            if f is None:
                return None
            sig.append(f.data_ptr())
    return sig


def _remember_group(layers, memo_key):
    m = []
    for pl in layers:
        ps = pl.params()[:-1]
        p0 = ps[0]
        p1 = ps[1] if len(ps) > 1 else None
        m.append((pl, pl._ver, p0, p0._version, p0.data_ptr(), p1, p1._version if p1 is not None else 0,
                  p1.data_ptr() if p1 is not None else 0))
    memos = getattr(layers[0], "_group_memo", None)
    if memos is None or len(memos) > 8:
        memos = layers[0]._group_memo = {}
    memos[memo_key] = m


def claim_grad_slot(engine, layers):
    slot = getattr(engine, "grad_slot", None)
    if slot is None or getattr(engine, "_slot_inflight", False):
        return None
    lo, hi = slot.data_ptr(), slot.data_ptr() + 4 * slot.numel()
    for pl in layers:
        for p in pl.params():
            g = p.grad
            if g is not None and lo <= g.data_ptr() < hi:
                return None
    try:
        torch.autograd.Variable._execution_engine.queue_callback(lambda: setattr(engine, "_slot_inflight", False))
        engine._slot_inflight = True
    except RuntimeError:
        pass
    return slot


def unpack_group(layers, grads, slot=None):
    out_per_layer = []
    off = 0
    if slot is not None:
        need = sum(p.numel() for pl in layers for p in pl.params())
        if slot.numel() != need or slot.dtype != torch.float32 or not slot.is_contiguous():
            raise _lib.NudfError("gradient slot has %d elements, the layers need %d" % (slot.numel(), need))

    def take(shape_like):
        nonlocal off
        if slot is None:
            return torch.empty_like(shape_like)
        n = shape_like.numel()
        v = slot[off:off + n].view(shape_like.shape)
        off += n
        return v
    for base in range(0, len(layers), _lib.PACK_MAX_LAYERS):
        chunk = layers[base:base + _lib.PACK_MAX_LAYERS]
        a = _lib.UnpackMulti()
        rows = 0
        keep = []
        for li, pl in enumerate(chunk):
            dW, db = grads[base + li]
            ps = pl.params()
            v = ps[0].detach().contiguous()
            dv = take(v)
            L = a.layer[li]
            L.dW, L.v, L.perm, L.dv = ptr(dW), ptr(v), ptr(pl.perm), ptr(dv)
            L.out, L.in_, L.ldw, L.row_start = pl.out, pl.inp, pl.in_pad, rows
            dg = None
            if pl.weight_norm:
                g = ps[1].detach().contiguous()
                dg = take(g)
                L.g, L.inv_norm, L.dg = ptr(g), ptr(pl.inv_norm), ptr(dg)
                keep += [v, g]
            else:
                keep += [v]
            dbo = take(ps[-1].detach())
            L.db_in, L.db_out = ptr(db), ptr(dbo)
            keep.append(db)
            out_per_layer.append([dv, dg, dbo] if pl.weight_norm else [dv, dbo])
            rows += pl.out
        a.n_layers, a.total_rows = len(chunk), rows
        call("nudf_weightnorm_unpack_grad_multi", a)
        del keep
    return [t for lay in out_per_layer for t in lay]


def _tn_jobs(specs, layers, grads, bias=True):
    jobs = []
    for D, X, i, *rows in specs:
        pl, (dW, db) = layers[i], grads[i]
        r0, r1 = rows or (0, pl.out)
        if rows:
            dW, db = dW[r0:r1], db[r0:r1]
        jobs.append((D, r1 - r0, X, pl.in_pad, dW, db if bias else None))
    return jobs


class Engine:

    def __init__(self, net):
        self.net = net
        self._kinds_cache = {}
        self._site_token = object()

    def _all(self):
        return self.layers

    def params(self):
        out = []
        for pl in self._all():
            out += pl.params()
        return out

    def invalidate(self):
        for pl in self._all():
            pl.invalidate()

    def mark_stale(self):
        for pl in self._all():
            pl._ver = None

    def _frag_kinds(self):
        k = self._kinds_cache.get(_mode_key())
        if k is None:
            k = self._kinds_cache[_mode_key()] = tuple(tuple(dict.fromkeys(ks)) for ks in self._frag_kinds_build())
        return k

    def _site(self, name):
        return (name, self._site_token)

    def backward(self, st, *adjoints):
        return (self._backward_chain if "chain" in st else self._backward_layers)(st, *adjoints)

    def _weight_grads(self, P, first, second=(), f16x2=False, amax_a=None, amax_b=None):
        layers = self._all()
        assign = tn_can_assign()
        grads = alloc_grads(layers, zero=not assign)
        gemm_tn_grouped(_tn_jobs(first, layers, grads), P, assign=assign, f16x2=f16x2, amax_a=amax_a)
        if second:
            gemm_tn_grouped(_tn_jobs(second, layers, grads, bias=False), P, f16x2=f16x2, amax_b=amax_b)
        return unpack_group(layers, grads, claim_grad_slot(self, layers))


class UDFEngine(Engine):
    def __init__(self, net):
        super().__init__(net)
        self.L = net.num_layers - 2
        self.E = net.embed_dim
        self.layers = [PackedLinear(getattr(net, f"lin{l}")) for l in range(self.L + 1)]
        self.skip = set(net.skip_in)
        self.inv_sqrt2 = 1.0 / math.sqrt(2.0)
        self.head_type = {"abs": 0, "square": 1, "sdf": 2}[getattr(net, "udf_type", "abs")]

    def _embed(self, x, P, X, tangent=None):
        net = self.net
        skip_dst = [X[s] for s in sorted(self.skip)]
        d2 = skip_dst[0] if skip_dst else None
        off2 = (self.layers[sorted(self.skip)[0]].inp - self.E) if skip_dst else 0
        call("nudf_posenc", ptr(x), 3, 1, ptr(tangent), net.d_in, net.multires, float(net.scale), P,
             ptr(X[0]), X[0].shape[1], 1.0,
             (ptr(d2) + 4 * off2) if d2 is not None else None, d2.shape[1] if d2 is not None else 0, self.inv_sqrt2)
        for s, dst in zip(sorted(self.skip)[1:], skip_dst[1:]):
            off = self.layers[s].inp - self.E
            call("nudf_posenc", ptr(x), 3, 1, ptr(tangent), net.d_in, net.multires, float(net.scale), P,
                 ptr(dst) + 4 * off, dst.shape[1], self.inv_sqrt2, None, 0, 0.0)

    def _chain_ok(self):
        net = self.net
        widths_ok = all(pl.out <= 256 and pl.inp <= 256 for pl in self.layers[:-1]) and self.layers[-1].inp <= 256 \
            and self.layers[-1].out - 1 <= 256
        skip_ok = len(self.skip) <= 1 and all(0 < s < self.L for s in self.skip)
        return USE_CHAIN and net.multires > 0 and net.d_in == 3 and widths_ok and skip_ok and self.L + 2 <= CH_MAX_STEPS

    def forward(self, x, need_grad_state, feat_ld=0, udf_only=False, feat_buf=None):
        if self._chain_ok():
            return self._forward_chain(x, need_grad_state, feat_ld, udf_only, feat_buf)
        return self._forward_layers(x, need_grad_state, feat_ld, udf_only)

    def _gradient_guard(self):
        if len(self.skip) > 1:
            raise NotImplementedError("more than one skip layer")
        if self.E > PV_MAXE:
            raise _lib.NudfError("nudf_posenc_vjp: encoding wider than %d (multires %d gives %d columns)"
                                 % (PV_MAXE, self.net.multires, self.E))

    def gradient(self, x, st):
        self._gradient_guard()
        if self._chain_ok():
            return self._gradient_chain(x, st)
        return self._gradient_layers(x, st)

    def forward_gradient(self, x, feat_ld=0, feat_buf=None):
        self._gradient_guard()
        if self._chain_ok() and _fuse() and 2 * self.L + 3 <= CH_MAX_STEPS:
            st = self._forward_chain(x, True, feat_ld, False, feat_buf, with_grad=True)
            g, DA = st.pop("g"), st.pop("DA")
            return st, g, DA
        st = self.forward(x, need_grad_state=True, feat_ld=feat_ld, feat_buf=feat_buf)
        g, DA = self.gradient(x, st)
        return st, g, DA

    def backward(self, x, st, DA, d_udf, d_feat, d_feat_ld, d_g):
        if self._chain_ok():
            return self._backward_chain(x, st, DA, d_udf, d_feat, d_feat_ld, d_g)
        return self._backward_layers(x, st, DA, d_udf, d_feat, d_feat_ld, d_g)

    def _frag_kinds_build(self):
        kinds = []
        for l, pl in enumerate(self.layers):
            if l == self.L:
                ks = [_head_kind(), _kind("fwd_feat", "fwd"), _kind("bwd_feat", "bwd")]
            elif l in self.skip:
                ks = [_kind("fwd", "fwd"), _kind("bwd", "grad"), _kind("bwd_hid:%d" % self.layers[l - 1].out, "bwd")]
                if PRECISION != "fp32":
                    ks.append(_kind("fwd", "bwd"))
            else:
                ks = [_kind("fwd", "fwd"), _kind("bwd", "grad")]
                if PRECISION != "fp32":
                    ks += [_kind("fwd", "bwd"), _kind("bwd", "bwd")]
            kinds.append(tuple(ks))
        return kinds

    def _blocked(self, P):
        return _state_blocked(P) and k8(self.layers[self.L].inp) == self.layers[self.L].inp

    def _skip_col(self, l):
        return self.layers[l].inp - self.E

    def _forward_chain(self, x, need_grad_state, feat_ld=0, udf_only=False, feat_buf=None, with_grad=False):
        P, dev, L = x.shape[0], x.device, self.L
        net = self.net
        pack_group(self.layers, self._frag_kinds())
        sd = _state_dtype()
        blk = self._blocked(P)
        X = ([_buf(P, self.layers[0].inp, dev, zero=False)] +
             [_buf(P, pl.inp, dev, zero=False, dtype=sd, blocked=blk) for pl in self.layers[1:]]) if need_grad_state else None
        if need_grad_state and k8(self.layers[L].inp) != self.layers[L].inp:
            X[L] = _buf(P, self.layers[L].inp, dev, dtype=sd)
        cb = ChainBuilder(P, "POSENC", k8(self.E), site=self._site("udf_fwd_grad" if with_grad else "udf_fwd"))
        cb.posenc(x, net.multires, float(net.scale))
        if need_grad_state:
            cb.init_store(X[0])
        for l in range(L):
            pl = self.layers[l]
            nxt_skip = (l + 1) in self.skip
            cb.step("SOFTPLUS", pl.frag(_kind("fwd", "fwd")), k8(pl.inp), pl.out, bias=pl.bias,
                    C1=X[l + 1] if need_grad_state else None,
                    scale=self.inv_sqrt2 if nxt_skip else 1.0,
                    pe_tail_col=self._skip_col(l + 1) if nxt_skip else -1, pe_tail_scale=self.inv_sqrt2,
                    pe_dst=X[l + 1] if (need_grad_state and nxt_skip) else None)
        pl = self.layers[L]
        Pp = pad_rows(P)
        udf = torch.empty(Pp, device=dev)
        sign = torch.empty(Pp, device=dev) if need_grad_state else None
        F = pl.out - 1
        feat = None
        if not udf_only:
            ld = max(feat_ld, F)
            if feat_buf is not None and tuple(feat_buf.shape) == (Pp, ld) and ld >= F + 3 and feat_buf.is_contiguous():
                feat = feat_buf
            else:
                feat = torch.empty((Pp, ld), device=dev)
                if ld >= F + 3:
                    call("nudf_copy_cols", ptr(x), 3, 1, ptr(feat) + 4 * F, ld, 3, P, 1.0)
                    _zero_cols(feat, F + 3)
                else:
                    _zero_cols(feat, F)
            cb.step("NONE", pl.frag(_kind("fwd_feat", "fwd")), k8(pl.inp), F, bias=pl.bias, bias_off=1, C1=feat,
                    act_write=0)
        cb.step("UDFHEAD", pl.frag(_head_kind()), k8(pl.inp), 1, bias=pl.bias, C1=sign, C2=udf, ldc1=1, ldc2=1,
                act_write=0, scale=1.0 / float(net.scale), iparam=self.head_type)
        st = dict(udf=udf[:P], sign=(sign[:P] if sign is not None else None),
                  feat=(feat[:P] if feat is not None else None), X=X, P=P)
        if with_grad:
            DA = self._gradient_buffers(P, X, dev)
            n_top = self.layers[L - 1].out
            cb.step("SEED", None, k8(n_top), n_top, r1_col=pl.W, C1=DA[L - 1], scale=1.0 / float(net.scale),
                    xscale=self._xs(L - 1))
            demb0, demb_skip = self._gradient_steps(cb, P, X, DA, dev)
            cb.launch()
            st["g"], st["DA"] = self._gradient_finish(x, P, demb0, demb_skip), DA
            return st
        cb.launch()
        return st

    def _gradient_buffers(self, P, X, dev):
        L = self.L
        return [_buf(P, self.layers[l].out, dev, zero=False, dtype=X[L].dtype, blocked=_isblk(X[L])) for l in range(L)]

    def _gradient_steps(self, cb, P, X, DA, dev):
        Epad = pad32(self.E)
        demb_skip = None
        for l in range(self.L - 1, 0, -1):
            pl = self.layers[l]
            if l in self.skip:
                demb_skip = torch.empty(pad_rows(P), Epad, device=dev)
                cb.step("MULSP", pl.frag(_kind("bwd", "grad")), k8(pl.out), pl.inp, X1=X[l], C1=DA[l - 1], C2=demb_skip,
                        iparam=self.layers[l - 1].out, scale=self.inv_sqrt2, xscale=self._xs(l - 1))
            else:
                cb.step("MULSP", pl.frag(_kind("bwd", "grad")), k8(pl.out), pl.inp, X1=X[l], C1=DA[l - 1],
                        xscale=self._xs(l - 1))
        demb0 = torch.empty(pad_rows(P), Epad, device=dev)
        pl0 = self.layers[0]
        cb.step("NONE", pl0.frag(_kind("bwd", "grad")), k8(pl0.out), pl0.inp, C1=demb0, act_write=0)
        return demb0, demb_skip

    def _gradient_finish(self, x, P, demb0, demb_skip):
        net, Epad = self.net, pad32(self.E)
        g = torch.empty(P, 3, device=x.device)
        call("nudf_posenc_vjp", ptr(x), 3, net.d_in, net.multires, float(net.scale), P,
             ptr(demb0), Epad, 1.0, ptr(demb_skip), Epad, 1.0, ptr(g))
        return g

    def _gradient_chain(self, x, st):
        P, L, dev = st["P"], self.L, x.device
        X = st["X"]
        net = self.net
        DA = self._gradient_buffers(P, X, dev)
        plL = self.layers[L]
        cb = ChainBuilder(P, "SEED", k8(self.layers[L - 1].out), site=self._site("udf_grad"))
        cb.init_seed(X[L], X[L].shape[1], st["sign"], plL.W, 1.0 / float(net.scale), self._xs(L - 1))
        cb.init_store(DA[L - 1])
        demb0, demb_skip = self._gradient_steps(cb, P, X, DA, dev)
        cb.launch()
        return self._gradient_finish(x, P, demb0, demb_skip), DA

    def _backward_chain(self, x, st, DA, d_udf, d_feat, d_feat_ld, d_g):
        P, L, dev = st["P"], self.L, x.device
        X, sign = st["X"], st["sign"]
        layers = self.layers
        net = self.net
        second = d_g is not None and DA is not None
        R = EX = None
        ex_fly = second and EX_FLY and _shared_split(X[L], mixed16=True)
        tn2 = _shared_split(X[L]) and not _is16(X[L])
        amax = torch.zeros(2, device=dev) if tn2 else None
        bsc = _sweep_dtype("bwd") == "f16x2"
        TA = torch.empty(pad_rows(P) // 32, device=dev) if (bsc and second) else None
        if second:
            sd, blk = X[L].dtype, _isblk(X[L])
            R = ([_buf(P, layers[0].inp, dev, zero=False)] +
                 [_buf(P, pl.inp, dev, zero=False, dtype=sd, blocked=blk) for pl in layers[1:]])
            EX = None if ex_fly else [_buf(P, layers[l].out, dev, zero=False, dtype=sd, blocked=blk) for l in range(L)]
            cb = ChainBuilder(P, "POSENC", k8(self.E), site=self._site("udf_tangent"))
            cb.posenc(x, net.multires, float(net.scale), tangent=d_g.contiguous())
            cb.init_store(R[0])
            if tn2:
                cb.absmax(amax[1:2])
            if bsc:
                cb.tile_scale(amax_out=TA)
            for l in range(L):
                pl = layers[l]
                nxt_skip = (l + 1) in self.skip
                if ex_fly:
                    cb.step("MULSP", pl.frag(_kind("fwd", "bwd")), k8(pl.inp), pl.out, X1=X[l + 1], C1=R[l + 1],
                            scale=self.inv_sqrt2 if nxt_skip else 1.0, xscale=self._xs(l),
                            pe_tail_col=self._skip_col(l + 1) if nxt_skip else -1, pe_tail_scale=self.inv_sqrt2,
                            pe_dst=R[l + 1] if nxt_skip else None)
                else:
                    cb.step("TANGENT", pl.frag(_kind("fwd", "bwd")), k8(pl.inp), pl.out, X1=X[l + 1], X2=DA[l], C1=R[l + 1],
                            C2=EX[l],
                            scale=self.inv_sqrt2 if nxt_skip else 1.0, xscale=self._xs(l),
                            pe_tail_col=self._skip_col(l + 1) if nxt_skip else -1, pe_tail_scale=self.inv_sqrt2,
                            pe_dst=R[l + 1] if nxt_skip else None)
            cb.launch()
        inv_scale = 1.0 / float(net.scale)
        plL = layers[L]
        F = plL.out - 1
        head4 = torch.empty(pad_rows(P), 4, device=dev)
        sg4 = torch.empty(pad_rows(P), 4, device=dev) if second else None
        if d_udf is not None:
            call("nudf_col0_seed4", ptr(sign), ptr(d_udf.reshape(-1).contiguous()), float(inv_scale), P, pad_rows(P),
                 ptr(head4), ptr(sg4))
        else:
            head4.zero_()
            if second:
                call("nudf_col0_seed4", ptr(sign), None, float(inv_scale), P, pad_rows(P), ptr(sg4), None)
        ABAR = [_buf(P, layers[l].out, dev, zero=False, dtype=X[L].dtype, blocked=_isblk(X[L])) for l in range(L)]
        cb = ChainBuilder(P, "LOAD", k8(F), site=self._site("udf_adjoint"))
        if d_feat is None:
            d_feat, d_feat_ld = torch.zeros(P, k8(F), device=dev), k8(F)
        elif d_feat_ld < k8(F) or d_feat_ld % 4:
            padded = torch.zeros(P, pad32(F), device=dev)
            padded[:, :F] = d_feat[:, :F]
            d_feat, d_feat_ld = padded, pad32(F)
        cb.init_load(d_feat, d_feat_ld)
        if tn2:
            cb.absmax(amax[0:1])
        if bsc:
            cb.tile_scale(amax_in=TA)
        for l in range(L, 0, -1):
            pl = layers[l]
            sc = self.inv_sqrt2 if l in self.skip else 1.0
            x2 = (R[l] if ex_fly else EX[l - 1]) if second else None
            x3 = DA[l - 1] if ex_fly else None
            if l == L:
                cb.step("BWD", pl.frag(_kind("bwd_feat", "bwd")), k8(F), layers[l - 1].out, X1=X[l], X2=x2, X3=x3,
                        C1=ABAR[l - 1], r1_row=head4, ldr1=4, r1_col=pl.W, scale=sc,
                        xscale=self._xs(l - 1))
            else:
                n_hid = layers[l - 1].out
                cb.step("BWD", pl.frag(_kind("bwd" if n_hid == pl.inp else "bwd_hid:%d" % n_hid, "bwd")), k8(pl.out),
                        n_hid, X1=X[l], X2=x2, X3=x3, C1=ABAR[l - 1], scale=sc, xscale=self._xs(l - 1))
        cb.launch()
        assert d_feat.shape[1] == d_feat_ld and d_feat.is_contiguous()
        first = [(ABAR[l], X[l], l) for l in range(L)] + [(d_feat, X[L], L, 1, plL.out), (head4, X[L], L, 0, 1)]
        sec = [(DA[l], R[l], l) for l in range(L)] + [(sg4, R[L], L, 0, 1)] if second else ()
        return self._weight_grads(P, first, sec, f16x2=tn2, amax_a=amax[0:1] if tn2 else None,
                                  amax_b=amax[1:2] if tn2 else None)

    def _forward_layers(self, x, need_grad_state, feat_ld=0, udf_only=False):
        P = x.shape[0]
        dev = x.device
        L = self.L
        pack_group(self.layers)
        X = [_buf(P, pl.inp, dev) for pl in self.layers]
        self._embed(x, P, X)
        for l in range(L):
            pl = self.layers[l]
            sc = self.inv_sqrt2 if (l + 1) in self.skip else 1.0
            gemm_nn(X[l], pl.Wt, P, pl.out, pl.in_pad, "SOFTPLUS", C1=X[l + 1], bias=pl.bias, scale=sc)
        pl = self.layers[L]
        udf = torch.empty(P, device=dev)
        sign = torch.empty(P, device=dev) if need_grad_state else None
        F = pl.out - 1
        feat = None
        if not udf_only:
            ld = max(feat_ld, F)
            feat = (torch.zeros if ld > F else torch.empty)((P, ld), device=dev)
            if ld >= F + 3:
                call("nudf_copy_cols", ptr(x), 3, 1, ptr(feat) + 4 * F, ld, 3, P, 1.0)
        gemm_nn(X[L], pl.Wt, P, 1 if udf_only else pl.out, pl.in_pad, "UDFHEAD", C1=feat, C2=udf, ldc2=1, C3=sign,
                ldc3=1, bias=pl.bias, scale=1.0 / float(self.net.scale), iparam=self.head_type)
        return dict(udf=udf, sign=sign, feat=feat, X=X, P=P)

    def _xs(self, j):
        return math.sqrt(2.0) if (j + 1) in self.skip else 1.0

    def _gradient_layers(self, x, st):
        P, L, dev = st["P"], self.L, x.device
        X = st["X"]
        DA = [_buf(P, self.layers[l].out, dev) for l in range(L)]
        plL = self.layers[L]
        call("nudf_udf_grad_seed", ptr(st["sign"]), ptr(plL.W), ptr(X[L]), X[L].shape[1], self._xs(L - 1), P,
             self.layers[L - 1].out, 1.0 / float(self.net.scale), ptr(DA[L - 1]), DA[L - 1].shape[1])
        Epad = pad32(self.E)
        demb_skip = None
        for l in range(L - 1, 0, -1):
            pl = self.layers[l]
            if l in self.skip:
                if demb_skip is not None:
                    raise NotImplementedError("more than one skip layer")
                demb_skip = torch.zeros(P, Epad, device=dev)
                gemm_nn(DA[l], pl.W, P, pl.inp, pl.out_pad, "SKIPSPLIT", C1=DA[l - 1], C2=demb_skip, X1=X[l],
                        iparam=self.layers[l - 1].out, scale=self.inv_sqrt2, xscale=self._xs(l - 1))
            else:
                gemm_nn(DA[l], pl.W, P, pl.inp, pl.out_pad, "MULSP", C1=DA[l - 1], X1=X[l], xscale=self._xs(l - 1))
        demb0 = torch.zeros(P, Epad, device=dev)
        pl0 = self.layers[0]
        gemm_nn(DA[0], pl0.W, P, pl0.inp, pl0.out_pad, "NONE", C1=demb0)
        g = torch.empty(P, 3, device=dev)
        call("nudf_posenc_vjp", ptr(x), 3, self.net.d_in, self.net.multires, float(self.net.scale), P,
             ptr(demb0), Epad, 1.0, ptr(demb_skip), Epad, 1.0, ptr(g))
        return g, DA

    def _backward_layers(self, x, st, DA, d_udf, d_feat, d_feat_ld, d_g):
        P, L, dev = st["P"], self.L, x.device
        X, sign = st["X"], st["sign"]
        layers = self.layers
        grads = [pl.new_grad_buffers() for pl in layers]
        second = d_g is not None and DA is not None
        R = EX = None
        if second:
            R = [_buf(P, pl.inp, dev) for pl in layers]
            EX = [_buf(P, layers[l].out, dev) for l in range(L)]
            self._embed(x, P, R, tangent=d_g.contiguous())
            for l in range(L):
                pl = layers[l]
                sc = self.inv_sqrt2 if (l + 1) in self.skip else 1.0
                gemm_nn(R[l], pl.Wt, P, pl.out, pl.in_pad, "TANGENT", C1=R[l + 1], C2=EX[l], X1=X[l + 1], X2=DA[l],
                        scale=sc, xscale=self._xs(l))
            call("nudf_signed_colsum", ptr(sign), ptr(R[L]), R[L].shape[1], P, layers[L].inp,
                 1.0 / float(self.net.scale), ptr(grads[L][0]))
        plL = layers[L]
        ABAR = [None] * (L + 1)
        ABAR[L] = _buf(P, plL.out, dev)
        call("nudf_udf_head_bwd", ptr(sign), ptr(d_udf), ptr(d_feat), d_feat_ld, P, plL.out - 1,
             1.0 / float(self.net.scale), ptr(ABAR[L]), ABAR[L].shape[1])
        for l in range(L, 0, -1):
            pl = layers[l]
            ABAR[l - 1] = _buf(P, layers[l - 1].out, dev)
            sc = self.inv_sqrt2 if l in self.skip else 1.0
            gemm_nn(ABAR[l], pl.W, P, layers[l - 1].out, pl.out_pad, "BWD", C1=ABAR[l - 1], X1=X[l],
                    X2=EX[l - 1] if second else None, scale=sc, xscale=self._xs(l - 1))
        for l, pl in enumerate(layers):
            dW, db = grads[l]
            if second and l < L:
                gemm_tn(ABAR[l], pl.out, X[l], dW, pl.out, pl.in_pad, P, dbias=db, A2=DA[l], na2=pl.out, B2=R[l])
            else:
                gemm_tn(ABAR[l], pl.out, X[l], dW, pl.out, pl.in_pad, P, dbias=db)
        return unpack_group(layers, grads)


def relu_chain_bwd(layers, inputs, outs, D_last, P, first_needs_input_grad, add_at=None):
    n = len(layers)
    grads = alloc_grads(layers)
    D = D_last
    d_in0 = None
    tn_jobs = []
    for i in range(n - 1, -1, -1):
        pl = layers[i]
        tn_jobs.append((D, pl.out, inputs[i], pl.in_pad, grads[i][0], grads[i][1]))
        if i > 0:
            prev = layers[i - 1]
            Dn = _buf(P, prev.out, D.device)
            extra = add_at.get(i - 1) if add_at else None
            if extra is not None:
                gemm_nn(D, pl.W, P, prev.out, pl.out_pad, "ADDMASK", C1=Dn, X1=outs[i - 1], ldx1=outs[i - 1].shape[1],
                        X2=extra[0], ldx2=extra[1], x2_off=extra[2])
            else:
                gemm_nn(D, pl.W, P, prev.out, pl.out_pad, "MULMASK", C1=Dn, X1=outs[i - 1], ldx1=outs[i - 1].shape[1])
            D = Dn
        elif first_needs_input_grad:
            d_in0 = _buf(P, pl.inp, D.device, zero=False)
            gemm_nn(D, pl.W, P, pl.inp, pl.out_pad, "NONE", C1=d_in0)
    gemm_tn_grouped(tn_jobs, P)
    return grads, d_in0


class ColorEngine(Engine):

    def __init__(self, net):
        super().__init__(net)
        n = net.num_layers - 1
        self.n = n
        F, H, dout = net.d_feature, net.d_hidden, net.d_out
        self.F, self.H, self.dout = F, H, dout
        self.npe = net.view_dim
        self.nrm = 0 if net.mode == "no_normal" else 6
        perm_b0 = [F + i for i in range(3 + self.nrm)] + list(range(F))
        perm_v0 = [H + i for i in range(self.npe)] + [H + self.npe + j for j in range(dout)] + list(range(H))
        self.base = [PackedLinear(getattr(net, f"lin_base{l}"), perm_b0 if l == 0 else None) for l in range(n)]
        self.view = [PackedLinear(getattr(net, f"lin{l}"), perm_v0 if l == 0 else None) for l in range(n)]

    def _all(self):
        return self.view + self.base

    @property
    def cin_ld(self):
        return pad32(self.F + 3 + self.nrm)

    def _chain_ok(self):
        n = self.n
        ok = USE_CHAIN and n >= 2 and 2 * n <= CH_MAX_STEPS and self.H <= 256 and self.net.embedview_fn is not None
        ok = ok and k8(self.base[0].inp) <= 288 and k8(self.H + self.npe + self.dout) <= 288 and self.F % 4 == 0
        ok = ok and self.view[n - 1].out <= 32 and self.dout <= 32
        ok = ok and self.H + self.npe + pad32(self.dout) <= 288
        return ok

    def _frag_kinds_build(self):
        fw, bw = _kind("fwd", "fwd"), _kind("bwd", "bwd")
        kinds = [(fw, _kind("bwd_hid:%d" % self.F, "bwd"))]
        kinds += [(fw, bw)] * (self.n - 1)
        kinds += [(fw, bw)] * self.n
        return kinds

    def forward(self, CIN, rays_d, S, P, keep_state=True, row_w=None):
        if self._chain_ok():
            return self._forward_chain(CIN, rays_d, S, P, keep_state, row_w)
        if row_w is not None:
            raise _lib.NudfError("the compositing sum inside the colour heads needs the fused chain launch")
        return self._forward_layers(CIN, rays_d, S, P, keep_state)

    def _forward_chain(self, CIN, rays_d, S, P, keep_state=True, row_w=None):
        dev, n = CIN.device, self.n
        fused = row_w is not None
        assert not (fused and keep_state)
        H, npe, dout = self.H, self.npe, self.dout
        pack_group(self.base + self.view, self._frag_kinds())
        Pp = pad_rows(P)
        VIN = torch.empty(Pp, pad32(H + npe + dout), device=dev) if keep_state else None
        sd = _state_dtype()
        HB = [CIN] + [_buf(P, H, dev, zero=False, dtype=sd) for _ in range(n - 1)] if keep_state else None
        HV = [VIN] + [_buf(P, H, dev, zero=False, dtype=sd) for _ in range(n - 1)] if keep_state else None
        cb = ChainBuilder(P, "LOAD", k8(self.base[0].inp), site=self._site("col_fwd"))
        cb.init_load(CIN, CIN.shape[1])
        cb.posenc(rays_d, self.net.multires_view, 1.0, x_div=S)
        for l in range(n - 1):
            pl = self.base[l]
            tap = (l == n - 2)
            cb.step("RELU", pl.frag(_kind("fwd", "fwd")), k8(pl.inp), pl.out, bias=pl.bias, C1=HB[l + 1] if keep_state else None,
                    C2=VIN if (tap and keep_state) else None, pe_tail_col=H if tap else -1, pe_tail_scale=1.0,
                    pe_dst=VIN if (tap and keep_state) else None)
        color_base = None if fused else torch.empty(Pp, dout, device=dev)
        sums_b = torch.empty(Pp // 32, 4, device=dev) if fused else None
        sums_c = torch.empty(Pp // 32, 4, device=dev) if fused else None
        pl = self.base[n - 1]
        cb.step("SIGMOIDN", pl.frag(_kind("fwd", "fwd")), k8(pl.inp), pl.out, bias=pl.bias, C1=color_base, C2=VIN if keep_state else None,
                c2_off=H + npe, iparam=dout, act_write=1, act_col0=H + npe, row_w=row_w, row_sums=sums_b)
        for l in range(n - 1):
            pl = self.view[l]
            cb.step("RELU", pl.frag(_kind("fwd", "fwd")), k8(pl.inp), pl.out, bias=pl.bias, C1=HV[l + 1] if keep_state else None)
        pl = self.view[n - 1]
        nb = pl.out - dout
        color = None if fused else torch.empty(Pp, dout, device=dev)
        logits = torch.empty(Pp, max(nb, 1), device=dev)
        cb.step("SIGMOIDN", pl.frag(_kind("fwd", "fwd")), k8(pl.inp), pl.out, bias=pl.bias, C1=color, C2=logits if nb > 0 else None,
                iparam=dout, act_write=0, row_w=row_w, row_sums=sums_c)
        cb.launch()
        if fused:
            return sums_b, sums_c, (logits[:P] if nb > 0 else None), None
        st = dict(HB=HB, HV=HV, P=P, chain=True) if keep_state else None
        return color_base[:P], color[:P], (logits[:P] if nb > 0 else None), st

    def _backward_chain(self, st, color_base, color, d_cb, d_color, d_logits):
        P, n = st["P"], self.n
        HB, HV = st["HB"], st["HV"]
        dev = color.device
        H, npe, dout = self.H, self.npe, self.dout
        plv = self.view[n - 1]
        nb = plv.out - dout
        sd = HV[1].dtype
        Dv = [_buf(P, H, dev, zero=False, dtype=sd) for _ in range(n - 1)] + [_buf(P, plv.out, dev, zero=False)]
        call("nudf_sigmoid_head_bwd", ptr(color), ptr(d_color), None, 0, dout, ptr(d_logits), max(nb, 1), nb, P,
             ptr(Dv[n - 1]), Dv[n - 1].shape[1])
        dVIN = _buf(P, self.view[0].inp, dev, zero=False)
        tn2 = PRECISION == "bf16x3" and not _is16(HV[1])
        amax = torch.zeros(1, device=dev) if tn2 else None
        cb = ChainBuilder(P, "LOAD", k8(plv.out), site=self._site("col_bwd_view"))
        cb.init_load(Dv[n - 1], Dv[n - 1].shape[1])
        if tn2:
            cb.absmax(amax)
        bsc = _sweep_dtype("bwd") == "f16x2"
        TV = torch.empty(pad_rows(P) // 32, device=dev) if bsc else None
        if bsc:
            cb.tile_scale(amax_out=TV)
        for i in range(n - 1, 0, -1):
            pl = self.view[i]
            cb.step("MULMASK", pl.frag(_kind("bwd", "bwd")), k8(pl.out), pl.inp, X1=HV[i], C1=Dv[i - 1])
        pl0 = self.view[0]
        cb.step("NONE", pl0.frag(_kind("bwd", "bwd")), k8(pl0.out), pl0.inp, C1=dVIN, act_write=0)
        cb.launch()
        plb = self.base[n - 1]
        Db = [_buf(P, H, dev, zero=False, dtype=sd) for _ in range(n - 1)] + [_buf(P, plb.out, dev, zero=False)]
        call("nudf_sigmoid_head_bwd", ptr(color_base), ptr(d_cb), ptr(dVIN) + 4 * (H + npe), dVIN.shape[1],
             dout, None, 0, 0, P, ptr(Db[n - 1]), Db[n - 1].shape[1])
        dCIN = torch.empty(pad_rows(P), self.cin_ld, device=dev)
        if k8(self.F) != self.F:
            _zero_cols(dCIN, self.F)
        cb = ChainBuilder(P, "LOAD", k8(plb.out), site=self._site("col_bwd_base"))
        cb.init_load(Db[n - 1], Db[n - 1].shape[1])
        if tn2:
            cb.absmax(amax)
        if bsc:
            cb.tile_scale(amax_in=TV)
        for i in range(n - 1, 0, -1):
            pl = self.base[i]
            if i == n - 1:
                cb.step("ADDMASK", pl.frag(_kind("bwd", "bwd")), k8(pl.out), pl.inp, X1=HB[i], X2=dVIN, C1=Db[i - 1])
            else:
                cb.step("MULMASK", pl.frag(_kind("bwd", "bwd")), k8(pl.out), pl.inp, X1=HB[i], C1=Db[i - 1])
        pb0 = self.base[0]
        cb.step("NONE", pb0.frag(_kind("bwd_hid:%d" % self.F, "bwd")), k8(pb0.out), self.F, C1=dCIN, act_write=0)
        cb.launch()
        jobs = [(Dv[i], HV[i], i) for i in range(n)] + [(Db[i], HB[i], n + i) for i in range(n)]
        return self._weight_grads(P, jobs, f16x2=tn2, amax_a=amax), dCIN[:P]

    def _forward_layers(self, CIN, rays_d, S, P, keep_state=True):
        dev = CIN.device
        n = self.n
        pack_group(self.base + self.view)
        VIN = _zero_cols(torch.empty(P, pad32(self.H + self.npe + self.dout), device=dev), self.H + self.npe + self.dout)
        call("nudf_posenc", ptr(rays_d), 3, S, None, 3, self.net.multires_view, 1.0, P,
             ptr(VIN) + 4 * self.H, VIN.shape[1], 1.0, None, 0, 0.0)
        HB = [CIN]
        for l in range(n - 1):
            pl = self.base[l]
            h = _buf(P, pl.out, dev)
            if l == n - 2:
                gemm_nn(HB[l], pl.Wt, P, pl.out, pl.in_pad, "RELU_DUAL", C1=h, C2=VIN, bias=pl.bias)
            else:
                gemm_nn(HB[l], pl.Wt, P, pl.out, pl.in_pad, "RELU", C1=h, bias=pl.bias)
            HB.append(h)
        color_base = torch.empty(P, self.dout, device=dev)
        pl = self.base[n - 1]
        gemm_nn(HB[n - 1], pl.Wt, P, pl.out, pl.in_pad, "SIGMOID", C1=color_base, C2=VIN, c2_off=self.H + self.npe,
                bias=pl.bias, iparam=self.dout)
        HV = [VIN]
        for l in range(n - 1):
            pl = self.view[l]
            h = _buf(P, pl.out, dev)
            gemm_nn(HV[l], pl.Wt, P, pl.out, pl.in_pad, "RELU", C1=h, bias=pl.bias)
            HV.append(h)
        pl = self.view[n - 1]
        color = torch.empty(P, self.dout, device=dev)
        nb = pl.out - self.dout
        logits = torch.empty(P, max(nb, 1), device=dev)
        gemm_nn(HV[n - 1], pl.Wt, P, pl.out, pl.in_pad, "SIGMOID", C1=color, C3=logits, bias=pl.bias,
                iparam=self.dout)
        st = dict(HB=HB, HV=HV, P=P) if keep_state else None
        return color_base, color, (logits if nb > 0 else None), st

    def _backward_layers(self, st, color_base, color, d_cb, d_color, d_logits):
        P, n = st["P"], self.n
        HB, HV = st["HB"], st["HV"]
        dev = color.device
        plv = self.view[n - 1]
        nb = plv.out - self.dout
        D = _buf(P, plv.out, dev, zero=False)
        call("nudf_sigmoid_head_bwd", ptr(color), ptr(d_color), None, 0, self.dout, ptr(d_logits), max(nb, 1), nb, P,
             ptr(D), D.shape[1])
        gv, dVIN = relu_chain_bwd(self.view, HV, HV[1:], D, P, True)
        Db = _buf(P, self.dout, dev, zero=False)
        call("nudf_sigmoid_head_bwd", ptr(color_base), ptr(d_cb), ptr(dVIN) + 4 * (self.H + self.npe), dVIN.shape[1],
             self.dout, None, 0, 0, P, ptr(Db), Db.shape[1])
        gb, dCIN = relu_chain_bwd(self.base, HB, HB[1:], Db, P, True, add_at={n - 2: (dVIN, dVIN.shape[1], 0)})
        return unpack_group(self.view + self.base, gv + gb), dCIN[:P]


class PlainColorEngine(Engine):

    def __init__(self, net):
        super().__init__(net)
        self.layers = [PackedLinear(getattr(net, f"lin{l}")) for l in range(net.num_layers - 1)]
        self.dout = net.d_out

    def forward(self, Xin, P, keep_state=True):
        dev, n = Xin.device, len(self.layers)
        pack_group(self.layers)
        X = _buf(P, self.layers[0].inp, dev)
        X[:P, :Xin.shape[1]] = Xin
        H = [X]
        for l in range(n - 1):
            pl = self.layers[l]
            h = _buf(P, pl.out, dev)
            gemm_nn(H[l], pl.Wt, P, pl.out, pl.in_pad, "RELU", C1=h, bias=pl.bias)
            H.append(h)
        pl = self.layers[n - 1]
        nb = pl.out - self.dout
        color = torch.empty(P, self.dout, device=dev)
        logits = torch.empty(P, max(nb, 1), device=dev)
        if self.net.squeeze_out:
            gemm_nn(H[n - 1], pl.Wt, P, pl.out, pl.in_pad, "SIGMOID", C1=color, C3=logits, bias=pl.bias, iparam=self.dout)
        else:
            raw = _buf(P, pl.out, dev)
            gemm_nn(H[n - 1], pl.Wt, P, pl.out, pl.in_pad, "NONE", C1=raw, bias=pl.bias)
            color, logits = raw[:P, :self.dout].contiguous(), raw[:P, self.dout:pl.out].contiguous()
        st = dict(H=H, P=P) if keep_state else None
        return color, (logits if nb > 0 else None), st

    def backward(self, st, color, d_color, d_logits):
        P, H = st["P"], st["H"]
        dev = color.device
        pl = self.layers[-1]
        nb = pl.out - self.dout
        D = _buf(P, pl.out, dev, zero=True)
        if self.net.squeeze_out:
            if d_color is None:
                d_color = torch.zeros_like(color)
            if nb > 0 and d_logits is None:
                d_logits = torch.zeros(P, nb, device=dev)
            call("nudf_sigmoid_head_bwd", ptr(color), ptr(d_color.contiguous()), None, 0, self.dout,
                 ptr(d_logits.contiguous()) if nb > 0 else None, max(nb, 1), nb, P, ptr(D), D.shape[1])
        else:
            if d_color is not None:
                D[:P, :self.dout] = d_color
            if nb > 0 and d_logits is not None:
                D[:P, self.dout:pl.out] = d_logits
        grads, dX = relu_chain_bwd(self.layers, H, H[1:], D, P, True)
        return unpack_group(self.layers, grads), dX[:P, :self.layers[0].inp]


class NerfEngine(Engine):

    def __init__(self, net):
        super().__init__(net)
        assert net.use_viewdirs, "NeRF(use_viewdirs=False) has no forward in the reference (fields.py:629-630)"
        self.D, self.W = net.D, net.W
        self.e = net.input_ch
        self.ev = net.input_ch_view
        self.skips = set(net.skips)
        self.pts = []
        for i in range(self.D):
            lin = net.pts_linears[i]
            perm = None
            if (i - 1) in self.skips:
                perm = [self.W + j for j in range(self.e)] + list(range(self.W))
            self.pts.append(PackedLinear(lin, perm))
        self.alpha = PackedLinear(net.alpha_linear)
        self.feature = PackedLinear(net.feature_linear)
        self.views = PackedLinear(net.views_linears[0])
        self.rgb = PackedLinear(net.rgb_linear)
        if len(net.views_linears) != 1:
            raise NotImplementedError("NeRF with more than one views layer")

    def _all(self):
        return self.pts + [self.views, self.feature, self.alpha, self.rgb]

    def _skip_layer(self):
        sk = [i + 1 for i in sorted(self.skips) if i + 1 < self.D]
        return sk[0] if sk else -1

    def _chain_ok(self):
        net = self.net
        sk = [i for i in self.skips if 0 <= i < self.D]
        ok = USE_CHAIN and self.W <= 256 and self.W % 32 == 0 and self.D + 5 <= CH_MAX_STEPS and len(sk) <= 1
        ok = ok and (not sk or sk[0] < self.D - 1) and k8(self.e) <= 288 and k8(self.W + self.ev) <= 288
        ok = ok and net.d_in_view == 3 and self.ev == 3 * (2 * net.multires_view + 1) and self.views.out <= 256
        return ok

    def _frag_kinds_build(self):
        fw, bw = _kind("fwd", "fwd"), _kind("bwd", "bwd")
        W, e, j = self.W, self.e, self._skip_layer()
        kinds = []
        for i in range(self.D):
            if i == j:
                kinds.append((_kind("fwd_in:0:%d" % W, "fwd"), _kind("fwd_in:%d:%d" % (W, e), "fwd"),
                              _kind("bwd_hid:%d" % W, "bwd")))
            else:
                kinds.append((fw,) if i == 0 else (fw, bw))
        kinds += [(fw, _kind("bwd_hid:%d" % W, "bwd")), (fw, bw), (fw,), (fw, bw)]
        return kinds

    def forward(self, pts4, rays_d, S, P, keep_state=True):
        if self._chain_ok():
            return self._forward_chain(pts4, rays_d, S, P, keep_state)
        return self._forward_layers(pts4, rays_d, S, P, keep_state)

    def _forward_chain(self, pts4, rays_d, S, P, keep_state=True):
        dev, D, W, e, ev = pts4.device, self.D, self.W, self.e, self.ev
        net = self.net
        fw = _kind("fwd", "fwd")
        j = self._skip_layer()
        pack_group(self._all(), self._frag_kinds())
        Hin = [_buf(P, self.pts[0].inp, dev)]
        if keep_state:
            Hin += [_buf(P, pl.inp, dev) for pl in self.pts[1:]]
        d2 = Hin[j] if (j >= 0 and keep_state) else None
        call("nudf_posenc", ptr(pts4), net.d_in, 1, None, net.d_in, net.multires, 1.0, P,
             ptr(Hin[0]), Hin[0].shape[1], 1.0,
             (ptr(d2) + 4 * W) if d2 is not None else None, d2.shape[1] if d2 is not None else 0, 1.0)
        Pp = pad_rows(P)
        h_last = _buf(P, W, dev, zero=False) if keep_state else None
        VIN = _zero_cols(torch.empty(Pp, pad32(W + ev), device=dev), W + ev) if keep_state else None
        hv = _buf(P, self.views.out, dev, zero=False) if keep_state else None
        sigma = torch.empty(Pp, 1, device=dev)
        rgb = torch.empty(Pp, 3, device=dev)
        cb = ChainBuilder(P, "LOAD", k8(e), site=self._site("nerf_fwd"))
        cb.init_load(Hin[0], Hin[0].shape[1])
        cb.posenc(rays_d, net.multires_view, 1.0, x_div=S)
        SK = None
        if j >= 0:
            SK = _buf(P, W, dev, zero=False)
            cb.step("NONE", self.pts[j].frag(_kind("fwd_in:%d:%d" % (W, e), "fwd")), k8(e), W, C1=SK, act_write=0)
        for i in range(D):
            pl = self.pts[i]
            dst = None
            if keep_state:
                dst = Hin[i + 1] if i + 1 < D else h_last
            if i == j:
                cb.step("RELUADD", pl.frag(_kind("fwd_in:0:%d" % W, "fwd")), k8(W), W, bias=pl.bias, X2=SK, C1=dst)
            else:
                cb.step("RELU", pl.frag(fw), k8(pl.inp), pl.out, bias=pl.bias, C1=dst)
        cb.step("NONE", self.alpha.frag(fw), k8(W), 1, bias=self.alpha.bias, C1=sigma, act_write=0)
        cb.step("NONE", self.feature.frag(fw), k8(W), W, bias=self.feature.bias, C1=VIN, pe_tail_col=W, pe_tail_scale=1.0,
                pe_dst=VIN)
        cb.step("RELU", self.views.frag(fw), k8(W + ev), self.views.out, bias=self.views.bias, C1=hv)
        cb.step("NONE", self.rgb.frag(fw), k8(self.views.out), 3, bias=self.rgb.bias, C1=rgb, act_write=0)
        cb.launch()
        st = dict(Hin=Hin, h_last=h_last, VIN=VIN, hv=hv, P=P, chain=True) if keep_state else None
        return sigma[:P], rgb[:P], st

    def _backward_chain(self, st, d_sigma, d_rgb):
        P, D, W = st["P"], self.D, self.W
        Hin, h_last, VIN, hv = st["Hin"], st["h_last"], st["VIN"], st["hv"]
        dev = VIN.device
        bw = _kind("bwd", "bwd")
        j = self._skip_layer()
        Pp = pad_rows(P)
        Drgb = torch.zeros(Pp, 32, device=dev)
        call("nudf_copy_cols", ptr(d_rgb), 3, 1, ptr(Drgb), 32, 3, P, 1.0)
        Dsig = torch.zeros(Pp, 32, device=dev)
        call("nudf_copy_cols", ptr(d_sigma), 1, 1, ptr(Dsig), 32, 1, P, 1.0)
        Dv = _buf(P, self.views.out, dev, zero=False)
        dF = _buf(P, W, dev, zero=False)
        Dp = [_buf(P, W, dev, zero=False) for _ in range(D)]
        cb = ChainBuilder(P, "LOAD", k8(3), site=self._site("nerf_bwd"))
        cb.init_load(Drgb, Drgb.shape[1])
        if _sweep_dtype("bwd") == "f16x2":
            cb.tile_scale()
        cb.step("MULMASK", self.rgb.frag(bw), k8(3), self.views.out, X1=hv, C1=Dv)
        cb.step("NONE", self.views.frag(_kind("bwd_hid:%d" % W, "bwd")), k8(self.views.out), W, C1=dF)
        cb.step("MULMASK", self.feature.frag(bw), k8(W), W, X1=h_last, r1_row=Dsig, ldr1=Dsig.shape[1],
                r1_col=self.alpha.W, C1=Dp[D - 1])
        for i in range(D - 1, 0, -1):
            pl = self.pts[i]
            kind = _kind("bwd_hid:%d" % W, "bwd") if i == j else bw
            cb.step("MULMASK", pl.frag(kind), k8(pl.out), W, X1=Hin[i], C1=Dp[i - 1], act_write=1 if i > 1 else 0)
        cb.launch()
        jobs = [(Dp[i], Hin[i], i) for i in range(D)] + [(Dv, VIN, D), (dF, h_last, D + 1), (Dsig, h_last, D + 2), (Drgb, hv, D + 3)]
        return self._weight_grads(P, jobs)

    def _forward_layers(self, pts4, rays_d, S, P, keep_state=True):
        dev = pts4.device
        pack_group(self._all())
        Hin = [_buf(P, pl.inp, dev) for pl in self.pts]
        skip_layers = [i + 1 for i in sorted(self.skips) if i + 1 < self.D]
        d2 = Hin[skip_layers[0]] if skip_layers else None
        call("nudf_posenc", ptr(pts4), self.net.d_in, 1, None, self.net.d_in, self.net.multires, 1.0, P,
             ptr(Hin[0]), Hin[0].shape[1], 1.0,
             (ptr(d2) + 4 * self.W) if d2 is not None else None, d2.shape[1] if d2 is not None else 0, 1.0)
        if len(skip_layers) > 1:
            raise NotImplementedError("more than one NeRF skip")
        outs = []
        for i in range(self.D):
            pl = self.pts[i]
            dst = Hin[i + 1] if i + 1 < self.D else _buf(P, pl.out, dev)
            gemm_nn(Hin[i], pl.Wt, P, pl.out, pl.in_pad, "RELU", C1=dst, bias=pl.bias)
            outs.append(dst)
        h = outs[-1]
        if (self.D - 1) in self.skips:
            raise NotImplementedError("skip after the last NeRF layer")
        sigma = torch.empty(P, 1, device=dev)
        gemm_nn(h, self.alpha.Wt, P, 1, self.alpha.in_pad, "NONE", C1=sigma, bias=self.alpha.bias)
        VIN = torch.zeros(P, pad32(self.W + self.ev), device=dev)
        gemm_nn(h, self.feature.Wt, P, self.feature.out, self.feature.in_pad, "NONE", C1=VIN, bias=self.feature.bias)
        call("nudf_posenc", ptr(rays_d), 3, S, None, self.net.d_in_view, self.net.multires_view, 1.0, P,
             ptr(VIN) + 4 * self.W, VIN.shape[1], 1.0, None, 0, 0.0)
        hv = _buf(P, self.views.out, dev)
        gemm_nn(VIN, self.views.Wt, P, self.views.out, self.views.in_pad, "RELU", C1=hv, bias=self.views.bias)
        rgb = torch.empty(P, 3, device=dev)
        gemm_nn(hv, self.rgb.Wt, P, 3, self.rgb.in_pad, "NONE", C1=rgb, bias=self.rgb.bias)
        st = dict(Hin=Hin, outs=outs, VIN=VIN, hv=hv, P=P) if keep_state else None
        return sigma, rgb, st

    def _backward_layers(self, st, d_sigma, d_rgb):
        P = st["P"]
        Hin, outs, VIN, hv = st["Hin"], st["outs"], st["VIN"], st["hv"]
        dev = VIN.device
        Drgb = torch.zeros(P, 32, device=dev)
        call("nudf_copy_cols", ptr(d_rgb), 3, 1, ptr(Drgb), 32, 3, P, 1.0)
        g_rgb = self.rgb.new_grad_buffers()
        gemm_tn(Drgb, 3, hv, g_rgb[0], 3, self.rgb.in_pad, P, dbias=g_rgb[1])
        Dv = _buf(P, self.views.out, dev)
        gemm_nn(Drgb, self.rgb.W, P, self.views.out, self.rgb.out_pad, "MULMASK", C1=Dv, X1=hv)
        g_views = self.views.new_grad_buffers()
        gemm_tn(Dv, self.views.out, VIN, g_views[0], self.views.out, self.views.in_pad, P, dbias=g_views[1])
        dVIN = _buf(P, self.views.inp, dev)
        gemm_nn(Dv, self.views.W, P, self.views.inp, self.views.out_pad, "NONE", C1=dVIN)
        g_feat = self.feature.new_grad_buffers()
        gemm_tn(dVIN, self.feature.out, outs[-1], g_feat[0], self.feature.out, self.feature.in_pad, P, dbias=g_feat[1])
        Dsig = torch.zeros(P, 32, device=dev)
        call("nudf_copy_cols", ptr(d_sigma), 1, 1, ptr(Dsig), 32, 1, P, 1.0)
        g_alpha = self.alpha.new_grad_buffers()
        gemm_tn(Dsig, 1, outs[-1], g_alpha[0], 1, self.alpha.in_pad, P, dbias=g_alpha[1])
        T1 = _buf(P, self.W, dev)
        gemm_nn(Dsig, self.alpha.W, P, self.W, self.alpha.out_pad, "NONE", C1=T1)
        Dh = _buf(P, self.W, dev)
        gemm_nn(dVIN, self.feature.W, P, self.W, self.feature.out_pad, "ADDMASK", C1=Dh, X1=outs[-1],
                ldx1=outs[-1].shape[1], X2=T1)
        gp, _ = relu_chain_bwd(self.pts, Hin, outs, Dh, P, False)
        return unpack_group(self._all(), gp + [g_views, g_feat, g_alpha, g_rgb])
```

neuraludf_amd/optim.py:

```python
from __future__ import annotations

import math

import torch

from ._lib import ADAM_MAX_GROUPS, ADAM_MAX_TENSORS, Adam, call, lib, NudfError


class FusedAdam(torch.optim.Optimizer):
    def __init__(self, params, lr=1e-3, betas=(0.9, 0.999), eps=1e-8, weight_decay=0, amsgrad=False):
        if weight_decay != 0 or amsgrad:
            raise NotImplementedError("FusedAdam: weight_decay / amsgrad are not used by the reference runner")
        defaults = dict(lr=lr, betas=betas, eps=eps, weight_decay=0, amsgrad=False)
        super().__init__(params, defaults)
        if len(self.param_groups) > ADAM_MAX_GROUPS:
            raise NudfError("FusedAdam supports at most %d parameter groups" % ADAM_MAX_GROUPS)
        self._chunk = None
        self.dyn_base = None
        self._plan = None
        self.plan_hits = 0
        self._order = []
        self.state_epoch = 0

    def load_state_dict(self, state_dict):
        super().load_state_dict(state_dict)
        self.state_epoch += 1

    def dyn_values(self):
        vals = []
        for p, gi in self._order:
            group = self.param_groups[gi]
            step = float(self.state[p]["step"]) + 1.0
            b1, b2 = group["betas"]
            vals.append(-group["lr"] / (1.0 - b1 ** step))
            vals.append(math.sqrt(1.0 - b2 ** step))
        return vals

    def advance(self):
        for p, _ in self._order:
            self.state[p]["step"] += 1
            torch.autograd.graph.increment_version(p)

    @torch.no_grad()
    def step(self, closure=None):
        loss = None
        if closure is not None:
            with torch.enable_grad():
                loss = closure()
        if self._chunk is None:
            self._chunk = int(lib().nudf_adam_chunk())
        chunk = self._chunk
        plan = self._plan
        if plan is not None and plan["epoch"] == self.state_epoch and plan["dyn"] == self.dyn_base:
            ok = plan["n_with_grad"] == sum(1 for group in self.param_groups for q in group["params"] if q.grad is not None)
            if ok:
                memo = {}
                state = self.state
                for (pp, gi, t), pa, st_step in zip(plan["entries"], plan["addr"], plan["steps"]):
                    g = pp.grad
                    st = state[pp]
                    if (g is None or pp.data_ptr() != pa or not g.is_contiguous() or st["step"] is not st_step
                            or st["exp_avg"].data_ptr() != t.m or st["exp_avg_sq"].data_ptr() != t.v
                            or g.dtype != torch.float32 or not g.is_cuda):
                        ok = False
                        break
                    k = (gi, float(st_step))
                    v = memo.get(k)
                    if v is None:
                        group = self.param_groups[gi]
                        step = k[1] + 1.0
                        b1, b2 = group["betas"]
                        v = memo[k] = (-group["lr"] / (1.0 - b1 ** step), math.sqrt(1.0 - b2 ** step))
                    t.g = g.data_ptr()
                    t.neg_step_size, t.bc2_sqrt = v
            if ok:
                self.plan_hits += 1
                for a in plan["launches"]:
                    self._fill_groups(a)
                    call("nudf_adam_step", a)
                self._order = plan["order"]
                if torch.cuda.is_current_stream_capturing():
                    return loss
                torch._foreach_add_(plan["steps"], 1.0)
                torch.autograd.graph.increment_version(plan["params"])
                return loss
        a = Adam()
        launches, entries = [], []
        keep = []
        nt = 0
        blocks = 0

        order = []
        launched = 0

        def flush():
            nonlocal a, nt, blocks, launched
            if nt:
                a.n_tensors = nt
                a.block_start[nt] = blocks
                if self.dyn_base is not None:
                    a.dyn = self.dyn_base + 8 * launched
                call("nudf_adam_step", a)
                launches.append(a)
            launched += nt
            a = Adam()
            self._fill_groups(a)
            nt = 0
            blocks = 0

        self._fill_groups(a)
        for gi, group in enumerate(self.param_groups):
            for p in group["params"]:
                if p.grad is None:
                    continue
                if not p.is_cuda:
                    raise NudfError("FusedAdam needs device parameters (no CPU fallback)")
                st = self.state[p]
                if len(st) == 0:
                    st["step"] = torch.tensor(0.0)
                    st["exp_avg"] = torch.zeros_like(p, memory_format=torch.preserve_format)
                    st["exp_avg_sq"] = torch.zeros_like(p, memory_format=torch.preserve_format)
                g = p.grad
                if g.dtype != torch.float32 or not g.is_cuda or p.dtype != torch.float32:
                    raise NudfError("FusedAdam needs fp32 device parameters and gradients")
                if not g.is_contiguous():
                    g = g.contiguous()
                    keep.append(g)
                if not p.is_contiguous():
                    raise NudfError("FusedAdam needs contiguous parameters")
                if nt == ADAM_MAX_TENSORS:
                    flush()
                t = a.t[nt]
                t.p, t.g, t.m, t.v = p.data_ptr(), g.data_ptr(), st["exp_avg"].data_ptr(), st["exp_avg_sq"].data_ptr()
                t.n, t.group = p.numel(), gi
                step = float(st["step"]) + 1.0
                b1, b2 = group["betas"]
                t.neg_step_size = -group["lr"] / (1.0 - b1 ** step)
                t.bc2_sqrt = math.sqrt(1.0 - b2 ** step)
                a.block_start[nt] = blocks
                blocks += (p.numel() + chunk - 1) // chunk
                nt += 1
                order.append((p, gi))
                entries.append((p, gi, t))
        flush()
        self._order = order
        self._plan = None if keep else {
            "epoch": self.state_epoch, "dyn": self.dyn_base, "entries": entries, "launches": launches, "order": order,
            "addr": [q.data_ptr() for q, _, _ in entries], "params": [q for q, _ in order],
            "steps": [self.state[q]["step"] for q, _ in order],
            "n_with_grad": len(entries)}
        if torch.cuda.is_current_stream_capturing():
            return loss
        for p, _ in order:
            self.state[p]["step"] += 1
            torch.autograd.graph.increment_version(p)
        return loss

    def _fill_groups(self, a):
        for gi, group in enumerate(self.param_groups):
            b1, b2 = group["betas"]
            g = a.group[gi]
            g.one_minus_beta1 = 1.0 - b1
            g.beta2 = b2
            g.one_minus_beta2 = 1.0 - b2
            g.eps = group["eps"]
```

neuraludf_amd/train.py:

```python
from __future__ import annotations

import contextlib
import io

import os

import numpy as np
import torch

from . import dist as nudf_dist
from ._lib import LW, LW_COUNT
from .loss.loss import ColorLoss
from .models import fields
from .models.udf_renderer_blending import UDFRendererBlending

def other_scalars(var, beta):
    return list(var.parameters()) + list(beta.parameters())


DTU_MODEL_CONF = dict(
    nerf=dict(D=8, d_in=4, d_in_view=3, W=256, multires=10, multires_view=4, output_ch=4, skips=[4],
              use_viewdirs=True),
    udf_network=dict(d_out=257, d_in=3, d_hidden=256, n_layers=8, skip_in=[4], multires=6, bias=0.5, scale=1.0,
                     geometric_init=True, weight_norm=True, udf_type="abs"),
    variance_network=dict(init_val=0.3),
    rendering_network=dict(d_feature=256, mode="no_normal", d_in=6, d_out=3, d_hidden=128, n_layers=4,
                           weight_norm=True, multires_view=4, squeeze_out=True, blending_cand_views=10),
    beta_network=dict(init_var_beta=0.5, init_var_gamma=0.3, init_var_zeta=0.3, beta_min=0.00005,
                      requires_grad_beta=True, requires_grad_gamma=False, requires_grad_zeta=False),
)


class StepScalars:
    SCHED, LOSSW, ADAM = 0, 8, 8 + LW_COUNT

    def __init__(self, device, n_adam=96, slots=8):
        n = self.ADAM + 2 * n_adam
        self.n_adam = n_adam
        self.dev = torch.zeros(n, device=device)
        self.host = [torch.zeros(n).pin_memory() for _ in range(slots)]
        self.events = [None] * slots
        self.k = 0

    def upload(self, sched, lossw, adam):
        i = self.k % len(self.host)
        self.k += 1
        if self.events[i] is not None:
            self.events[i].synchronize()
        h = self.host[i].numpy()
        h[self.SCHED:self.SCHED + len(sched)] = sched
        h[self.LOSSW:self.LOSSW + len(lossw)] = lossw
        if len(adam) > 2 * self.n_adam:
            raise ValueError("too many optimizer tensors for the step-scalar buffer")
        h[self.ADAM:self.ADAM + len(adam)] = adam
        self.dev.copy_(self.host[i], non_blocking=True)
        ev = torch.cuda.Event()
        ev.record()
        self.events[i] = ev


SINGLE_THREAD_BACKWARD = os.environ.get("NUDF_HOST_FAST", "1") != "0"


class GraphedStep:

    def __init__(self, trainer, eager_steps=2, max_graphs=4, capture_collectives=False):
        from .optim import FusedAdam
        self.tr = trainer
        self.eager_steps = eager_steps
        self.max_graphs = max_graphs
        self.graphs = {}
        self.enabled = isinstance(trainer.optimizer, FusedAdam) and (capture_collectives or not trainer.data_parallel)
        self.scalars = None
        self.replays = 0
        self.captures = 0
        self._last = None
        self._epoch = getattr(trainer.optimizer, "state_epoch", 0)

    def invalidate(self):
        self.graphs.clear()
        self._last = None

    def _key(self, batch, blend, has_anneal, perturb_overwrite):
        tr = self.tr
        sig = lambda d: tuple(sorted((k, tuple(v.shape), str(v.dtype)) for k, v in d.items() if torch.is_tensor(v)))
        live = tuple(p.requires_grad for g in tr.param_groups for p in g)
        cw = tr.color_loss
        terms = (cw.color_pixel_weight > 0, cw.color_patch_weight > 0, tr.lc["color_pixel_weight"] > 0,
                 tr.lc["color_patch_weight"] > 0, tr.tc["mask_weight"] > 0)
        static = tuple(sorted((k, v) for k, v in tr.lc.items() if not k.endswith("_weight")))
        return (sig(batch), sig(blend) if blend is not None else None, bool(has_anneal), perturb_overwrite, terms, static,
                live)

    def __call__(self, batch, cos_anneal_ratio=1.0, flip_saturation=1.0, blend=None, perturb_overwrite=-1):
        tr = self.tr
        kw = dict(cos_anneal_ratio=cos_anneal_ratio, flip_saturation=flip_saturation, blend=blend,
                  perturb_overwrite=perturb_overwrite)
        if not self.enabled:
            return tr.step(batch, **kw)
        if getattr(tr.optimizer, "state_epoch", 0) != self._epoch:
            self._epoch = tr.optimizer.state_epoch
            self.invalidate()
        if (blend is not None and "ref_cam" not in blend and tr.lc["color_pixel_weight"] > 0
                and tr.lc["color_patch_weight"] > 0):
            from .models import blend as _blend
            blend = dict(blend)
            blend["ref_cam"], blend["src_cam"] = _blend.patch_cameras(blend["intrinsics"][0], blend["intrinsics"],
                                                                      blend["query_c2w"], torch.inverse(blend["w2cs"]))
            kw["blend"] = blend
        key = self._key(batch, blend, cos_anneal_ratio is not None, perturb_overwrite)
        ent = self.graphs.get(key)
        if ent is None:
            if len(self.graphs) >= self.max_graphs:
                self.graphs.pop(next(iter(self.graphs)))
            ent = self.graphs[key] = dict(calls=0, graph=None)
        ent["calls"] += 1
        self._last = ent
        if ent["graph"] is None:
            if ent["calls"] <= self.eager_steps or ent.get("failed"):
                return tr.step(batch, **kw)
            prev_stream = torch.cuda.current_stream()
            try:
                self._capture(ent, batch, blend, cos_anneal_ratio is not None, flip_saturation, perturb_overwrite)
            except Exception as e:
                import warnings
                ent["failed"], ent["graph"] = True, None
                torch.cuda.set_stream(prev_stream)
                torch.cuda.synchronize()
                warnings.warn("GraphedStep: capture failed (%s); this configuration keeps running eagerly" % (e,))
                return tr.step(batch, **kw)
        for k, v in ent["batch"].items():
            src = batch[k]
            if torch.is_tensor(v) and src is not v and src.data_ptr() != v.data_ptr():
                v.copy_(src)
        if blend is not None:
            for k, v in ent["blend"].items():
                src = blend[k]
                if torch.is_tensor(v) and src is not v and src.data_ptr() != v.data_ptr():
                    v.copy_(src)
        tr.optimizer._order = ent["order"]
        ent["scalars"].upload([0.0 if cos_anneal_ratio is None else float(cos_anneal_ratio), float(flip_saturation)],
                              tr.loss_weights().values(), tr.optimizer.dyn_values())
        ent["graph"].replay()
        tr.optimizer.advance()
        self.replays += 1
        return ent["loss"], ent["out"]

    def static_inputs(self):
        ent = self._last
        if ent is None or ent.get("graph") is None:
            return None
        return ent["batch"], ent["blend"]

    def _capture(self, ent, batch, blend, has_anneal, flip_saturation, perturb_overwrite):
        tr = self.tr
        dev = batch["rays_o"].device
        n_adam = sum(len(g) for g in tr.param_groups)
        if self.scalars is None or self.scalars.n_adam < n_adam:
            self.scalars = StepScalars(dev, n_adam=max(96, n_adam))
        ent["scalars"] = self.scalars
        ent["batch"] = {k: (v.clone() if torch.is_tensor(v) else v) for k, v in batch.items()}
        ent["blend"] = ({k: (v.clone() if torch.is_tensor(v) else v) for k, v in blend.items()}
                        if blend is not None else None)
        for m in tr.modules().values():
            e = getattr(m, "_engine", None)
            if e is not None and hasattr(e, "mark_stale"):
                e.mark_stale()
        sc = self.scalars
        tr.renderer.sched_scalars = sc.dev[sc.SCHED:sc.SCHED + 2]
        tr.optimizer.dyn_base = sc.dev.data_ptr() + 4 * sc.ADAM
        tr.loss_weights().bind(sc.dev[sc.LOSSW:sc.LOSSW + LW_COUNT])
        if blend is not None:
            tr.color_loss.prefill_constants(dev)
        g = torch.cuda.CUDAGraph()
        torch.cuda.synchronize()
        import gc
        gc_was_on = gc.isenabled()
        gc.disable()
        try:
            with torch.cuda.graph(g):
                loss, out = tr.step(ent["batch"], cos_anneal_ratio=(1.0 if has_anneal else None),
                                    flip_saturation=flip_saturation, blend=ent["blend"],
                                    perturb_overwrite=perturb_overwrite)
        finally:
            if gc_was_on:
                gc.enable()
            tr.renderer.sched_scalars = None
            tr.optimizer.dyn_base = None
            tr.loss_weights().unbind()
        ent["graph"], ent["loss"], ent["out"], ent["order"] = g, loss, out, list(tr.optimizer._order)
        self.captures += 1


class Trainer:
    def __init__(self, device, renderer_conf, color_loss_conf=None, train_conf=None, seed=0, data_parallel=False,
                 fields_mod=fields, renderer_cls=UDFRendererBlending, loss_cls=ColorLoss, fused_adam=False,
                 model_conf=None):
        torch.manual_seed(seed)
        c = dict(DTU_MODEL_CONF)
        if model_conf is not None:
            c.update({k: dict(model_conf[k]) for k in DTU_MODEL_CONF if k in model_conf})
        with contextlib.redirect_stdout(io.StringIO()):
            self.nerf = fields_mod.NeRF(**c["nerf"]).to(device)
            self.udf = fields_mod.UDFNetwork(**c["udf_network"]).to(device)
            self.var = fields_mod.SingleVarianceNetwork(**c["variance_network"]).to(device)
            self.color = fields_mod.ResidualRenderingNetwork(**c["rendering_network"]).to(device)
            self.beta = fields_mod.BetaNetwork(**c["beta_network"]).to(device)
        tc = dict(learning_rate=5e-4, learning_rate_geo=1e-4, igr_weight=0.1, igr_ns_weight=0.0, mask_weight=0.0,
                  sparse_weight=0.0)
        tc.update(train_conf or {})
        self.tc = tc
        geo = list(self.udf.parameters())
        other = list(self.var.parameters()) + list(self.color.parameters()) + list(self.beta.parameters())
        nerf = list(self.nerf.parameters())
        self.param_groups = [geo, other, nerf]
        groups = [{'params': geo, 'lr': tc["learning_rate_geo"]}, {'params': other}, {'params': nerf}]
        if fused_adam:
            from .optim import FusedAdam
            self.optimizer = FusedAdam(groups, lr=tc["learning_rate"])
        else:
            self.optimizer = torch.optim.Adam(groups, lr=tc["learning_rate"])
        self.renderer = renderer_cls(self.nerf, self.udf, self.var, self.color, self.beta, **renderer_conf)
        lc = dict(color_base_weight=0.01, color_weight=1.0, color_pixel_weight=0.0, color_patch_weight=0.0,
                  pixel_loss_type="l1", patch_loss_type="ssim", h_patch_size=3)
        lc.update(color_loss_conf or {})
        self.lc = lc
        with contextlib.redirect_stdout(io.StringIO()):
            self.color_loss = loss_cls(**lc)
        self.data_parallel = data_parallel
        self.status_every = 100
        self._beta_flag = True
        self.fuse_loss = not data_parallel
        self._one = {}
        self.defer_sums_reduce = True
        import os
        self.fuse_blend_loss = os.environ.get("NUDF_FUSE_BLEND_LOSS", "1") != "0"
        if data_parallel:
            self.renderer.data_parallel = True
            self.renderer.defer_loss_sums = True
            self.color_loss.set_data_parallel(True)
            def seg(m):
                e = m.engine() if hasattr(m, "engine") else None
                ps = list(e.params()) if e is not None else list(m.parameters())
                assert {id(p) for p in ps} == {id(p) for p in m.parameters()}
                return ps, e
            self.bucket = nudf_dist.GradBucket([(other_scalars(self.var, self.beta), None), seg(self.color), seg(self.udf),
                                                seg(self.nerf)], device=device)

    def modules(self):
        return dict(nerf=self.nerf, udf=self.udf, var=self.var, color=self.color, beta=self.beta)

    def enable_graph(self, eager_steps=2):
        self.graphed = GraphedStep(self, eager_steps=eager_steps)
        return self.graphed

    def loss_weights(self):
        lw = self.color_loss.weights
        tc = self.tc
        lw.set(igr=tc["igr_weight"], igr_ns=tc["igr_ns_weight"], sparse=tc["sparse_weight"], mask=tc["mask_weight"])
        return lw

    def loss(self, batch, cos_anneal_ratio=1.0, flip_saturation=1.0, blend=None, perturb_overwrite=-1):
        tc, lc = self.tc, self.lc
        w = self.loss_weights().device(batch["rays_o"].device)
        kw = {}
        if blend is not None and lc["color_pixel_weight"] > 0:
            kw = dict(color_maps=blend["color_maps"], w2cs=blend["w2cs"], intrinsics=blend["intrinsics"],
                      query_c2w=blend["query_c2w"],
                      rays_uv=batch["rays_uv"].clone() if lc["color_patch_weight"] > 0 else None)
            if "ref_cam" in blend:
                kw["patch_cams"] = (blend["ref_cam"], blend["src_cam"])
        defer, defer_r = self.renderer.defer_loss_sums, self.renderer.defer_sums_reduce
        if self.fuse_loss:
            self.renderer.defer_loss_sums = True
            self.renderer.defer_sums_reduce = self.defer_sums_reduce
        try:
            out = self.renderer.render(batch["rays_o"], batch["rays_d"], batch["near"], batch["far"],
                                       flip_saturation=flip_saturation, cos_anneal_ratio=cos_anneal_ratio,
                                       perturb_overwrite=perturb_overwrite, **kw)
        finally:
            self.renderer.defer_loss_sums, self.renderer.defer_sums_reduce = defer, defer_r
        weight_sum = out["weight_sum"]
        pixel_mask = batch["mask"] if tc["mask_weight"] > 0 else None
        if (self.fuse_blend_loss and "_loss_sums" in out and not self.data_parallel and tc["mask_weight"] <= 0
                and out["patch_mask"] is not None
                and self.color_loss.blend_fusable(out["color_base"], out["color"], batch["true_rgb"], out["color_pixel"],
                                                  pixel_mask, out["patch_colors"], batch.get("gt_patch_colors"))):
            sums = out.pop("_loss_sums")
            r = self.color_loss.blend_step_loss(out["color_base"], out["color"], batch["true_rgb"], out["color_pixel"],
                                                out["patch_colors"], batch["gt_patch_colors"], out["patch_mask"], weight_sum,
                                                sums, float(weight_sum.shape[0]), w)
            out["gradient_error"], out["gradient_error_near_surface"], out["sparse_error"] = r[6], r[7], r[8]
            return r[0], out
        patch_mask = None
        if out["patch_mask"] is not None:
            patch_mask = (out["patch_mask"].float()[:, None] * (weight_sum > 0.5).float()) > 0.
        cargs = (out["color_base"], out["color"], batch["true_rgb"], out["color_pixel"], pixel_mask, out["patch_colors"],
                 batch.get("gt_patch_colors"), patch_mask)
        bce_sum = None
        if tc["mask_weight"] > 0:
            bce_sum = torch.nn.functional.binary_cross_entropy(weight_sum.clip(1e-3, 1.0 - 1e-3), batch["mask"],
                                                               reduction="sum")
        if "_loss_sums" in out and not self.data_parallel:
            sums = out.pop("_loss_sums")
            if bce_sum is None and self.color_loss.fusable(out["color_base"], out["color"], batch["true_rgb"],
                                                           out["color_pixel"], out["patch_colors"]):
                from .loss.loss import _StepLossFn
                loss, _, _, _, ge, gens, se = _StepLossFn.apply(
                    out["color_base"], out["color"], batch["true_rgb"], pixel_mask, sums, float(weight_sum.shape[0]), w)
                out["gradient_error"], out["gradient_error_near_surface"], out["sparse_error"] = ge, gens, se
                return loss, out
            ge, gens, se = self.renderer.errors_from_sums(sums, weight_sum.shape[0])
            out["gradient_error"], out["gradient_error_near_surface"], out["sparse_error"] = ge, gens, se
            cl = self.color_loss(*cargs)
            mask_loss = bce_sum / float(weight_sum.numel()) if bce_sum is not None else None
        elif "_loss_sums" in out:
            parts = [out.pop("_loss_sums")]
            fused = self.color_loss.fusable(out["color_base"], out["color"], batch["true_rgb"], out["color_pixel"],
                                            out["patch_colors"])
            if fused:
                parts.append(self.color_loss.local_sums(out["color_base"], out["color"], batch["true_rgb"], pixel_mask))
            if bce_sum is not None:
                parts.append(torch.stack([bce_sum, torch.full_like(bce_sum, float(weight_sum.numel()))]))
            packed = nudf_dist.all_reduce_sum(torch.cat([p.reshape(-1) for p in parts]))
            ge, gens, se = self.renderer.errors_from_sums(packed[:5], weight_sum.shape[0])
            out["gradient_error"], out["gradient_error_near_surface"], out["sparse_error"] = ge, gens, se
            k = 5
            if fused:
                cl = self.color_loss.from_global_sums(out["color_base"], out["color"], batch["true_rgb"], pixel_mask,
                                                      packed[k:k + 3])
                k += 3
            else:
                cl = self.color_loss(*cargs)
            mask_loss = packed[k] / packed[k + 1] if bce_sum is not None else None
        else:
            cl = self.color_loss(*cargs)
            mask_loss = bce_sum / float(weight_sum.numel()) if bce_sum is not None else None
        loss = cl["loss"] + out["gradient_error_near_surface"] * w[LW["igr_ns"]] \
            + out["sparse_error"] * w[LW["sparse"]] + out["gradient_error"] * w[LW["igr"]]
        if mask_loss is not None:
            loss = loss + mask_loss * w[LW["mask"]]
        return loss, out

# ... 105 lines not shown
```

Baseline: 19.93 million.

## Fuse Adam update with weight-norm repacking into a single tail kernel

Adds an adam_pack kernel. Each workgroup first applies Adam to the weight rows (and their gain) belonging to one packed panel, then immediately repacks that panel into the weight-norm fragment layout. Adam for the remaining tensors runs on extra blocks in the same launch. Python-side bookkeeping (TailPack, tail tables, prepack before graph capture) marks the packed weights fresh after the step, so the next forward skips a separate pack launch. This removes one kernel launch and a global re-read of the weights per step, at the cost of a lot of host-side freshness tracking that risks stale packs if buffers change.

```diff
diff --git a/include/nudf.h b/include/nudf.h
--- a/include/nudf.h
+++ b/include/nudf.h
@@ -330,8 +330,13 @@
   int32_t pad2_;
   NudfAdamGroup group[NUDF_ADAM_MAX_GROUPS];
   const float* dyn;
+  const struct NudfPackLayer* pack_layer;
+  const int32_t* pack_map;
+  int32_t n_pack_layers, pack_blocks;
+  int32_t pack_pw, pad3_;
 } NudfAdam;
 int nudf_adam_step(const NudfAdam* args, void* stream);
+int nudf_adam_pack(const NudfAdam* args, void* stream);
 int nudf_adam_chunk(void);
 
 enum {
diff --git a/neuraludf_amd/_lib.py b/neuraludf_amd/_lib.py
--- a/neuraludf_amd/_lib.py
+++ b/neuraludf_amd/_lib.py
@@ -132,7 +132,8 @@
 class Adam(C.Structure):
     _fields_ = [("n_tensors", i32), ("pad_", i32), ("t", AdamTensor * ADAM_MAX_TENSORS),
                 ("block_start", i32 * (ADAM_MAX_TENSORS + 1)), ("pad2_", i32), ("group", AdamGroup * ADAM_MAX_GROUPS),
-                ("dyn", c_fp)]
+                ("dyn", c_fp), ("pack_layer", c_fp), ("pack_map", c_fp), ("n_pack_layers", i32), ("pack_blocks", i32),
+                ("pack_pw", i32), ("pad3_", i32)]
 
 
 CH_MAX_STEPS = 20
@@ -337,6 +338,7 @@
     "nudf_patch_metric": (_I, [_I] + [_P, _P, _P, _I, _I, _P, _P, _P, _P]),
     "nudf_adam_step": (_I, [C.POINTER(Adam), _P]),
     "nudf_adam_chunk": (_I, []),
+    "nudf_adam_pack": (_I, [C.POINTER(Adam), _P]),
     "nudf_mlp_chain": (_I, [C.POINTER(Chain), _P]),
     "nudf_mlp_chain_plan": (_I, [C.POINTER(Chain), C.c_char_p, i32, C.POINTER(C.c_int32)]),
     "nudf_set_chain_t16": (_I, [_I]),
diff --git a/neuraludf_amd/csrc/adam_update.h b/neuraludf_amd/csrc/adam_update.h
--- /dev/null
+++ b/neuraludf_amd/csrc/adam_update.h
@@ -0,0 +1,35 @@
+#pragma once
+#include "../../include/nudf.h"
+
+#define ADAM_BLOCK 256
+#define ADAM_PER_THREAD 4
+#define ADAM_CHUNK (ADAM_BLOCK * ADAM_PER_THREAD)
+
+__device__ __forceinline__ NudfAdamTensor adam_tensor(const NudfAdam& a, int ti) {
+  NudfAdamTensor t = a.t[ti];
+  if (a.dyn) {
+    t.neg_step_size = a.dyn[2 * ti];
+    t.bc2_sqrt = a.dyn[2 * ti + 1];
+  }
+  return t;
+}
+
+__device__ __forceinline__ void adam_elem(const NudfAdamTensor& t, const NudfAdamGroup& g, int i) {
+  const float gr = t.g[i];
+  float m = t.m[i], v = t.v[i];
+  m = __fmaf_rn(gr - m, g.one_minus_beta1, m);
+  v = __fmaf_rn(gr, __fmul_rn(g.one_minus_beta2, gr), __fmul_rn(v, g.beta2));
+  const float denom = __fadd_rn(sqrtf(v) / t.bc2_sqrt, g.eps);
+  t.p[i] = __fmaf_rn(t.neg_step_size, m / denom, t.p[i]);
+  t.m[i] = m;
+  t.v[i] = v;
+}
+
+__device__ __forceinline__ int adam_tensor_of_block(const NudfAdam& a, int b) {
+  int lo = 0, hi = a.n_tensors;
+  while (hi - lo > 1) {
+    const int mid = (lo + hi) >> 1;
+    if (a.block_start[mid] <= b) lo = mid; else hi = mid;
+  }
+  return lo;
+}
diff --git a/neuraludf_amd/csrc/optim.hip b/neuraludf_amd/csrc/optim.hip
--- a/neuraludf_amd/csrc/optim.hip
+++ b/neuraludf_amd/csrc/optim.hip
@@ -1,37 +1,18 @@
 #include "nudf_common.h"
 #include "../../include/nudf.h"
 
-#define ADAM_BLOCK 256
-#define ADAM_PER_THREAD 4
-#define ADAM_CHUNK (ADAM_BLOCK * ADAM_PER_THREAD)
+#include "adam_update.h"
 
 __global__ __launch_bounds__(ADAM_BLOCK) void adam_kernel(NudfAdam a) {
-  int lo = 0, hi = a.n_tensors;
   const int b = blockIdx.x;
-  while (hi - lo > 1) {
-    const int mid = (lo + hi) >> 1;
-    if (a.block_start[mid] <= b) lo = mid; else hi = mid;
-  }
-  NudfAdamTensor t = a.t[lo];
+  const int lo = adam_tensor_of_block(a, b);
+  const NudfAdamTensor t = adam_tensor(a, lo);
   const NudfAdamGroup g = a.group[t.group];
-  if (a.dyn) {
-    t.neg_step_size = a.dyn[2 * lo];
-    t.bc2_sqrt = a.dyn[2 * lo + 1];
-  }
   const int base = (b - a.block_start[lo]) * ADAM_CHUNK;
 #pragma unroll
   for (int k = 0; k < ADAM_PER_THREAD; ++k) {
     const int i = base + k * ADAM_BLOCK + threadIdx.x;
-    if (i < t.n) {
-      const float gr = t.g[i];
-      float m = t.m[i], v = t.v[i];
-      m = m + (gr - m) * g.one_minus_beta1;
-      v = v * g.beta2 + g.one_minus_beta2 * gr * gr;
-      const float denom = sqrtf(v) / t.bc2_sqrt + g.eps;
-      t.p[i] = t.p[i] + t.neg_step_size * (m / denom);
-      t.m[i] = m;
-      t.v[i] = v;
-    }
+    if (i < t.n) adam_elem(t, g, i);
   }
 }
 
diff --git a/neuraludf_amd/csrc/rays_embed.hip b/neuraludf_amd/csrc/rays_embed.hip
--- a/neuraludf_amd/csrc/rays_embed.hip
+++ b/neuraludf_amd/csrc/rays_embed.hip
@@ -1,5 +1,6 @@
 #include "nudf_common.h"
 #include "../../include/nudf.h"
+#include "adam_update.h"
 
 static inline int nblocks(long long n, int bs) { return (int)((n + bs - 1) / bs); }
 
@@ -474,16 +475,7 @@
              (unsigned)q[4] | ((unsigned)q[5] << 16), (unsigned)q[6] | ((unsigned)q[7] << 16)};
 }
 
-__global__ __launch_bounds__(WNP_THREADS) void wn_pack_multi_kernel(NudfPackMulti a, int pw) {
-  extern __shared__ float panel[];
-  int li = 0, b = blockIdx.x;
-  for (; li < a.n_layers; ++li) {
-    const int nb = (a.layer[li].out + WNP_ROWS - 1) / WNP_ROWS;
-    if (b < nb) break;
-    b -= nb;
-  }
-  if (li >= a.n_layers) return;
-  const NudfPackLayer& L = a.layer[li];
+__device__ __forceinline__ void wnp_panel(const NudfPackLayer& L, int b, int pw, float* panel) {
   const int row0 = b * WNP_ROWS;
   const int wave = threadIdx.x >> 6, l = threadIdx.x & 63, tid = threadIdx.x;
   for (int e = tid; e < WNP_ROWS * pw; e += WNP_THREADS) panel[e] = 0.0f;
@@ -572,6 +564,78 @@
     }
   }
 }
+
+__global__ __launch_bounds__(WNP_THREADS) void wn_pack_multi_kernel(NudfPackMulti a, int pw) {
+  extern __shared__ float panel[];
+  int li = 0, b = blockIdx.x;
+  for (; li < a.n_layers; ++li) {
+    const int nb = (a.layer[li].out + WNP_ROWS - 1) / WNP_ROWS;
+    if (b < nb) break;
+    b -= nb;
+  }
+  if (li >= a.n_layers) return;
+  wnp_panel(a.layer[li], b, pw, panel);
+}
+
+static_assert(ADAM_CHUNK == WNP_THREADS, "an Adam workgroup of adam_pack_kernel updates one chunk, one element per thread");
+__global__ __launch_bounds__(WNP_THREADS) void adam_pack_kernel(NudfAdam a) {
+  extern __shared__ float panel[];
+  const int tid = threadIdx.x;
+  if ((int)blockIdx.x >= a.pack_blocks) {
+    const int b = blockIdx.x - a.pack_blocks;
+    const int lo = adam_tensor_of_block(a, b);
+    const NudfAdamTensor t = adam_tensor(a, lo);
+    const NudfAdamGroup g = a.group[t.group];
+    const int i = (b - a.block_start[lo]) * ADAM_CHUNK + tid;
+    if (i < t.n) adam_elem(t, g, i);
+    return;
+  }
+  int li = 0, hi = a.n_pack_layers;
+  while (hi - li > 1) {
+    const int mid = (li + hi) >> 1;
+    if (a.pack_map[mid] <= (int)blockIdx.x) li = mid; else hi = mid;
+  }
+  const NudfPackLayer& L = a.pack_layer[li];
+  const int b = blockIdx.x - a.pack_map[li];
+  const int row0 = b * WNP_ROWS;
+  const int nrows = min(WNP_ROWS, L.out - row0);
+  const int tv = a.pack_map[a.n_pack_layers + 1 + 2 * li], tg = a.pack_map[a.n_pack_layers + 2 + 2 * li];
+  if (tv >= 0 && nrows > 0) {
+    const NudfAdamTensor t = adam_tensor(a, tv);
+    const NudfAdamGroup g = a.group[t.group];
+    const int first = row0 * L.in, end = first + nrows * L.in;
+    for (int i = first + tid; i < end; i += WNP_THREADS)
+      if (i < t.n) adam_elem(t, g, i);
+  }
+  if (tg >= 0 && tid < nrows) {
+    const NudfAdamTensor t = adam_tensor(a, tg);
+    const NudfAdamGroup g = a.group[t.group];
+    if (row0 + tid < t.n) adam_elem(t, g, row0 + tid);
+  }
+  __threadfence_block();
+  __syncthreads();
+  wnp_panel(L, b, a.pack_pw, panel);
+}
+extern "C" int nudf_adam_pack(const NudfAdam* args, void* stream) {
+  const NudfAdam& a = *args;
+  if (a.n_tensors < 0 || a.n_tensors > NUDF_ADAM_MAX_TENSORS) {
+    nudf_set_error("nudf_adam_pack: too many tensors in one call", hipErrorInvalidValue);
+    return (int)hipErrorInvalidValue;
+  }
+  if (a.n_pack_layers <= 0) return nudf_adam_step(args, stream);
+  const size_t lds = (size_t)WNP_ROWS * a.pack_pw * sizeof(float);
+  if (!a.pack_layer || !a.pack_map || a.pack_blocks < a.n_pack_layers || a.pack_pw < 36 || (a.pack_pw & 31) != 4 ||
+      lds > 64 * 1024) {
+    nudf_set_error("nudf_adam_pack: pack tables missing, fewer panels than layers, or a panel stride that is not a "
+                   "multiple of 32 plus 4 in [36, 508]", hipErrorInvalidValue);
+    return (int)hipErrorInvalidValue;
+  }
+  const int nblk = a.pack_blocks + (a.n_tensors > 0 ? a.block_start[a.n_tensors] : 0);
+  hipLaunchKernelGGL(adam_pack_kernel, dim3(nblk), dim3(WNP_THREADS), lds, (hipStream_t)stream, a);
+  NUDF_CHECK_LAUNCH("nudf_adam_pack");
+  return 0;
+}
+
 extern "C" int nudf_weightnorm_pack_multi(const NudfPackMulti* args, void* stream) {
   if (args->n_layers <= 0 || args->total_rows <= 0) return 0;
   if (args->n_layers > NUDF_PACK_MAX_LAYERS) {
diff --git a/neuraludf_amd/mlp.py b/neuraludf_amd/mlp.py
--- a/neuraludf_amd/mlp.py
+++ b/neuraludf_amd/mlp.py
@@ -4,6 +4,7 @@
 from typing import List, Optional
 
 import ctypes as C
+import weakref
 
 import torch
 
@@ -583,6 +584,20 @@
     return FUSE_SWEEPS and _shared_split()
 
 
+FUSE_TAIL = int(os.environ.get("NUDF_FUSE_TAIL", "2") or 0)
+FUSE_TAIL_ADAM_PACK = 2
+
+
+def set_fuse_tail(bits):
+    global FUSE_TAIL
+    old, FUSE_TAIL = FUSE_TAIL, int(bits)
+    return old
+
+
+def fuse_adam_pack():
+    return bool(FUSE_TAIL & FUSE_TAIL_ADAM_PACK) and _lib.HOST_FAST
+
+
 def _tn_prec():
     if PRECISION == "fp32":
         return 0
@@ -671,15 +686,8 @@
     memo_key = (len(layers), tuple(kinds) if kinds is not None else None)
     memos = getattr(layers[0], "_group_memo", None) if _lib.HOST_FAST else None
     m = memos.get(memo_key) if memos is not None else None
-    if m is not None:
-        fresh = True
-        for pl, ver_obj, p0, v0, d0, p1, v1, d1 in m:
-            if (pl._ver is not ver_obj or p0._version != v0 or p0.data_ptr() != d0
-                    or (p1 is not None and (p1._version != v1 or p1.data_ptr() != d1))):
-                fresh = False
-                break
-        if fresh:
-            return
+    if m is not None and _memo_fresh(m):
+        return
     kinds = kinds or [()] * len(layers)
     dev = layers[0].params()[0].device
     stale = False
@@ -744,6 +752,14 @@
         layers[0].__dict__.setdefault("_pack_descs", {})[memo_key] = (psig, descs)
 
 
+def _memo_fresh(m):
+    for pl, ver_obj, p0, v0, d0, p1, v1, d1 in m:
+        if (pl._ver is not ver_obj or p0._version != v0 or p0.data_ptr() != d0
+                or (p1 is not None and (p1._version != v1 or p1.data_ptr() != d1))):
+            return False
+    return True
+
+
 def _pack_ptr_signature(layers, kinds, dev):
     sig = []
     for pl, ks in zip(layers, kinds):
@@ -774,6 +790,82 @@
     if memos is None or len(memos) > 8:
         memos = layers[0]._group_memo = {}
     memos[memo_key] = m
+
+
+_TAIL_ENGINES = weakref.WeakSet()
+
+
+class TailPack:
+
+    def __init__(self, layers, kinds_arg, kinds, descs):
+        self.layers, self.kinds_arg, self.kinds, self.descs = list(layers), kinds_arg, kinds, descs
+        self.memo_key = (len(layers), tuple(kinds_arg) if kinds_arg is not None else None)
+        self.bufs = [(pl.W, pl.Wt, pl.inv_norm, pl.perm, dict(pl._frags)) for pl in layers]
+
+    def same_buffers(self, allow_missing=False):
+        for pl, (W, Wt, inv_norm, perm, frags) in zip(self.layers, self.bufs):
+            if pl.W is not W or pl.Wt is not Wt or pl.inv_norm is not inv_norm or pl.perm is not perm:
+                return False
+            if not allow_missing and len(pl._frags) != len(frags):
+                return False
+            for k, f in pl._frags.items():
+                if frags.get(k) is not f:
+                    return False
+        return True
+
+    def fresh(self):
+        memos = getattr(self.layers[0], "_group_memo", None)
+        m = memos.get(self.memo_key) if memos is not None else None
+        return m is not None and _memo_fresh(m)
+
+    def mark_fresh(self):
+        for pl in self.layers:
+            pl._ver = tuple((p.data_ptr(), p._version) for p in pl.params()[:-1])
+        _remember_group(self.layers, self.memo_key)
+
+    def refresh(self):
+        if fuse_adam_pack() and self.same_buffers():
+            self.mark_fresh()
+            return True
+        return False
+
+    def ensure(self):
+        if self.fresh() and self.same_buffers():
+            return False
+        for a in self.descs:
+            call("nudf_weightnorm_pack_multi", a)
+        if self.same_buffers(allow_missing=True):
+            for pl, b in zip(self.layers, self.bufs):
+                pl._frags = dict(b[4])
+            self.mark_fresh()
+        return True
+
+
+def tail_pack_of(engine):
+    la = getattr(engine, "_last_pack", None)
+    if la is None or not fuse_adam_pack():
+        return None
+    layers, kinds_arg = la
+    if kinds_arg is not None and tuple(kinds_arg) != engine._frag_kinds():
+        return None
+    tp = getattr(engine, "_tail_pack", None)
+    rec = getattr(layers[0], "_pack_descs", {}).get((len(layers), tuple(kinds_arg) if kinds_arg is not None else None))
+    if rec is None or layers[0].W is None:
+        return None
+    if tp is None or tp.descs is not rec[1] or tp.kinds_arg is not kinds_arg:
+        kinds = [tuple(dict.fromkeys(ks)) for ks in (kinds_arg or [()] * len(layers))]
+        if _pack_ptr_signature(layers, kinds, layers[0].W.device) != rec[0]:
+            return None
+        if any(k not in ks for pl, ks in zip(layers, kinds) for k in pl._frags):
+            return None
+        tp = engine._tail_pack = TailPack(layers, kinds_arg, kinds, rec[1])
+    if not tp.fresh() or not tp.same_buffers():
+        return None
+    for pl in layers:
+        for p in pl.params()[:-1]:
+            if not p.is_contiguous():
+                return None
+    return tp
 
 
 def claim_grad_slot(engine, layers):
@@ -889,6 +981,16 @@
     def backward(self, st, *adjoints):
         return (self._backward_chain if "chain" in st else self._backward_layers)(st, *adjoints)
 
+    def _pack(self, layers, kinds=None):
+        self._last_pack = (layers, kinds)
+        _TAIL_ENGINES.add(self)
+        pack_group(layers, kinds)
+
+    def prepack(self):
+        la = getattr(self, "_last_pack", None)
+        if la is not None and (la[1] is None or tuple(la[1]) == self._frag_kinds()):
+            pack_group(*la)
+
     def _weight_grads(self, P, first, second=(), f16x2=False, amax_a=None, amax_b=None):
         layers = self._all()
         assign = tn_can_assign()
@@ -987,7 +1089,7 @@
     def _forward_chain(self, x, need_grad_state, feat_ld=0, udf_only=False, feat_buf=None, with_grad=False):
         P, dev, L = x.shape[0], x.device, self.L
         net = self.net
-        pack_group(self.layers, self._frag_kinds())
+        self._pack(self.layers, self._frag_kinds())
         sd = _state_dtype()
         blk = self._blocked(P)
         X = ([_buf(P, self.layers[0].inp, dev, zero=False)] +
@@ -1170,7 +1272,7 @@
         P = x.shape[0]
         dev = x.device
         L = self.L
-        pack_group(self.layers)
+        self._pack(self.layers)
         X = [_buf(P, pl.inp, dev) for pl in self.layers]
         self._embed(x, P, X)
         for l in range(L):
@@ -1334,7 +1436,7 @@
         fused = row_w is not None
         assert not (fused and keep_state)
         H, npe, dout = self.H, self.npe, self.dout
-        pack_group(self.base + self.view, self._frag_kinds())
+        self._pack(self.base + self.view, self._frag_kinds())
         Pp = pad_rows(P)
         VIN = torch.empty(Pp, pad32(H + npe + dout), device=dev) if keep_state else None
         sd = _state_dtype()
@@ -1426,7 +1528,7 @@
     def _forward_layers(self, CIN, rays_d, S, P, keep_state=True):
         dev = CIN.device
         n = self.n
-        pack_group(self.base + self.view)
+        self._pack(self.base + self.view)
         VIN = _zero_cols(torch.empty(P, pad32(self.H + self.npe + self.dout), device=dev), self.H + self.npe + self.dout)
         call("nudf_posenc", ptr(rays_d), 3, S, None, 3, self.net.multires_view, 1.0, P,
              ptr(VIN) + 4 * self.H, VIN.shape[1], 1.0, None, 0, 0.0)
@@ -1484,7 +1586,7 @@
 
     def forward(self, Xin, P, keep_state=True):
         dev, n = Xin.device, len(self.layers)
-        pack_group(self.layers)
+        self._pack(self.layers)
         X = _buf(P, self.layers[0].inp, dev)
         X[:P, :Xin.shape[1]] = Xin
         H = [X]
@@ -1589,7 +1691,7 @@
         net = self.net
         fw = _kind("fwd", "fwd")
         j = self._skip_layer()
-        pack_group(self._all(), self._frag_kinds())
+        self._pack(self._all(), self._frag_kinds())
         Hin = [_buf(P, self.pts[0].inp, dev)]
         if keep_state:
             Hin += [_buf(P, pl.inp, dev) for pl in self.pts[1:]]
@@ -1660,7 +1762,7 @@
 
     def _forward_layers(self, pts4, rays_d, S, P, keep_state=True):
         dev = pts4.device
-        pack_group(self._all())
+        self._pack(self._all())
         Hin = [_buf(P, pl.inp, dev) for pl in self.pts]
         skip_layers = [i + 1 for i in sorted(self.skips) if i + 1 < self.D]
         d2 = Hin[skip_layers[0]] if skip_layers else None
diff --git a/neuraludf_amd/optim.py b/neuraludf_amd/optim.py
--- a/neuraludf_amd/optim.py
+++ b/neuraludf_amd/optim.py
@@ -1,10 +1,13 @@
 from __future__ import annotations
 
+import ctypes as C
 import math
 
 import torch
 
-from ._lib import ADAM_MAX_GROUPS, ADAM_MAX_TENSORS, Adam, call, lib, NudfError
+from ._lib import ADAM_MAX_GROUPS, ADAM_MAX_TENSORS, Adam, PackLayer, call, lib, NudfError
+
+PACK_ROWS = 32
 
 
 class FusedAdam(torch.optim.Optimizer):
@@ -20,6 +23,9 @@
         self._plan = None
         self.plan_hits = 0
         self._order = []
+        self._tail_done = []
+        self._tail_tables = {}
+        self.tail_launches = 0
         self.state_epoch = 0
 
     def load_state_dict(self, state_dict):
@@ -40,6 +46,8 @@
         for p, _ in self._order:
             self.state[p]["step"] += 1
             torch.autograd.graph.increment_version(p)
+        for tp in self._tail_done:
+            tp.refresh()
 
     @torch.no_grad()
     def step(self, closure=None):
@@ -77,12 +85,14 @@
                 self.plan_hits += 1
                 for a in plan["launches"]:
                     self._fill_groups(a)
-                    call("nudf_adam_step", a)
+                self._launch(plan["launches"])
                 self._order = plan["order"]
                 if torch.cuda.is_current_stream_capturing():
                     return loss
                 torch._foreach_add_(plan["steps"], 1.0)
                 torch.autograd.graph.increment_version(plan["params"])
+                for tp in self._tail_done:
+                    tp.refresh()
                 return loss
         a = Adam()
         launches, entries = [], []
@@ -100,7 +110,6 @@
                 a.block_start[nt] = blocks
                 if self.dyn_base is not None:
                     a.dyn = self.dyn_base + 8 * launched
-                call("nudf_adam_step", a)
                 launches.append(a)
             launched += nt
             a = Adam()
@@ -143,6 +152,7 @@
                 order.append((p, gi))
                 entries.append((p, gi, t))
         flush()
+        self._launch(launches)
         self._order = order
         self._plan = None if keep else {
             "epoch": self.state_epoch, "dyn": self.dyn_base, "entries": entries, "launches": launches, "order": order,
@@ -154,7 +164,81 @@
         for p, _ in order:
             self.state[p]["step"] += 1
             torch.autograd.graph.increment_version(p)
+        for tp in self._tail_done:
+            tp.refresh()
         return loss
+
+    def _launch(self, launches):
+        from . import mlp
+        self._tail_done = []
+        fused = [None] * len(launches)
+        if mlp.fuse_adam_pack() and launches:
+            loc = {a.t[i].p: (k, i) for k, a in enumerate(launches) for i in range(a.n_tensors)}
+            per = [([], []) for _ in launches]
+            used, done = set(), []
+            for e in list(mlp._TAIL_ENGINES):
+                tp = mlp.tail_pack_of(e)
+                if tp is None:
+                    continue
+                entries = [d.layer[i] for d in tp.descs for i in range(d.n_layers)]
+                place = []
+                for pl, L in zip(tp.layers, entries):
+                    ps = pl.params()[:-1]
+                    at = [loc.get(p.data_ptr()) for p in ps]
+                    if (None in at or len({k for k, _ in at}) != 1 or any(x in used for x in at) or len(set(at)) != len(at)
+                            or any(launches[k].t[i].n != p.numel() for (k, i), p in zip(at, ps))
+                            or L.v != ps[0].data_ptr() or (L.out, L.in_) != (pl.out, pl.inp)):
+                        place = None
+                        break
+                    used.update(at)
+                    place.append((at[0][0], L, [i for _, i in at] + [-1] * (2 - len(at))))
+                if place is None or len(entries) != len(tp.layers):
+                    continue
+                for k, L, row in place:
+                    per[k][0].append(L)
+                    per[k][1].append(row)
+                done.append(tp)
+            if done:
+                fused = [self._tail_desc(a, ls, tmap, self._chunk) if ls else None for a, (ls, tmap) in zip(launches, per)]
+                if any(f is None and ls for f, (ls, _) in zip(fused, per)):
+                    fused = [None] * len(launches)
+                else:
+                    self._tail_done = done
+        for a, f in zip(launches, fused):
+            if f is None:
+                call("nudf_adam_step", a)
+            else:
+                call("nudf_adam_pack", f)
+                self.tail_launches += 1
+
+    def _tail_desc(self, a, layers, tmap, chunk):
+        starts, blocks = [], 0
+        for L in layers:
+            starts.append(blocks)
+            blocks += (L.out + PACK_ROWS - 1) // PACK_ROWS
+        pmap = starts + [blocks] + [i for r in tmap for i in r]
+        blob = b"".join(bytes(L) for L in layers) + bytes((C.c_int32 * len(pmap))(*pmap))
+        dev_tab = self._tail_tables.get(blob)
+        if dev_tab is None:
+            if torch.cuda.is_current_stream_capturing() or len(self._tail_tables) >= 64:
+                return None
+            dev = torch.device("cuda", torch.cuda.current_device())
+            dev_tab = self._tail_tables[blob] = torch.frombuffer(bytearray(blob), dtype=torch.uint8).to(dev)
+        fa = Adam()
+        C.memmove(C.byref(fa), C.byref(a), C.sizeof(Adam))
+        packed = {i for r in tmap for i in r if i >= 0}
+        nblk = 0
+        for i in range(a.n_tensors):
+            fa.block_start[i] = nblk
+            if i not in packed:
+                nblk += (a.t[i].n + chunk - 1) // chunk
+        fa.block_start[a.n_tensors] = nblk
+        fa.pack_layer = dev_tab.data_ptr()
+        fa.pack_map = dev_tab.data_ptr() + C.sizeof(PackLayer) * len(layers)
+        fa.n_pack_layers, fa.pack_blocks = len(layers), blocks
+        fa.pack_pw = (max(L.in_ for L in layers) + 31) // 32 * 32 + 4
+        fa._keep = dev_tab
+        return fa
 
     def _fill_groups(self, a):
         for gi, group in enumerate(self.param_groups):
diff --git a/neuraludf_amd/train.py b/neuraludf_amd/train.py
--- a/neuraludf_amd/train.py
+++ b/neuraludf_amd/train.py
@@ -138,6 +138,9 @@
                 src = blend[k]
                 if torch.is_tensor(v) and src is not v and src.data_ptr() != v.data_ptr():
                     v.copy_(src)
+        for tp in ent["packs"]:
+            tp.ensure()
+        tr.optimizer._tail_done = ent["tail"]
         tr.optimizer._order = ent["order"]
         ent["scalars"].upload([0.0 if cos_anneal_ratio is None else float(cos_anneal_ratio), float(flip_saturation)],
                               tr.loss_weights().values(), tr.optimizer.dyn_values())
@@ -162,9 +165,13 @@
         ent["batch"] = {k: (v.clone() if torch.is_tensor(v) else v) for k, v in batch.items()}
         ent["blend"] = ({k: (v.clone() if torch.is_tensor(v) else v) for k, v in blend.items()}
                         if blend is not None else None)
-        for m in tr.modules().values():
-            e = getattr(m, "_engine", None)
-            if e is not None and hasattr(e, "mark_stale"):
+        from . import mlp
+        engines = [e for e in (getattr(m, "_engine", None) for m in tr.modules().values()) if e is not None]
+        fuse_tail = mlp.fuse_adam_pack()
+        for e in engines:
+            if fuse_tail and hasattr(e, "prepack"):
+                e.prepack()
+            elif hasattr(e, "mark_stale"):
                 e.mark_stale()
         sc = self.scalars
         tr.renderer.sched_scalars = sc.dev[sc.SCHED:sc.SCHED + 2]
@@ -189,6 +196,15 @@
             tr.optimizer.dyn_base = None
             tr.loss_weights().unbind()
         ent["graph"], ent["loss"], ent["out"], ent["order"] = g, loss, out, list(tr.optimizer._order)
+        ent["tail"] = list(getattr(tr.optimizer, "_tail_done", ()))
+        ent["packs"] = []
+        if fuse_tail:
+            for e in engines:
+                la = getattr(e, "_last_pack", None)
+                rec = la and getattr(la[0][0], "_pack_descs", {}).get((len(la[0]), tuple(la[1]) if la[1] is not None else None))
+                if rec:
+                    kinds = [tuple(dict.fromkeys(ks)) for ks in (la[1] or [()] * len(la[0]))]
+                    ent["packs"].append(mlp.TailPack(la[0], la[1], kinds, rec[1]))
         self.captures += 1
 
 
```

Measured after the change: 19.95 million, median of 2. No clear change (+0.1%).
